# LanceKnight/MolKGNN

Hardware: AMD Instinct MI355X
Metric: molecules/sec fwd+bwd, 3-layer MolKGNN on AID 1798 (higher is better)
Workload: dtype f32; 1 GPU; AID 1798 full set shape (61832 molecules, ~25 atoms / ~53 directed edges each), 3 layers, hidden_dim 32, kernels 10/20/30/50 per degree, batch 4096 molecules per GPU (102584 atoms), 4 resident batches cycled, fwd+bwd+AdamW, one hipGraph per batch; variant=auto, batch_size_per_gpu=4096, parallelism=dp1

## Files before the change

include/molkgnn_hip.h:

```cpp
#ifndef MOLKGNN_HIP_H
#define MOLKGNN_HIP_H

#include <stddef.h>
#include <stdint.h>

#ifdef __cplusplus
extern "C" {
#endif

#define MKGNN_MAX_DEGREE 4
#define MKGNN_ABI_VERSION 8

#define MKGNN_LOSS_BCE_MEAN 0
#define MKGNN_LOSS_SQERR_MEAN 1
#define MKGNN_LOSS_SQERR_SUM 2

typedef struct mkgnn_kernel_bank {
    int32_t num_kernels;
    int32_t reserved;
    const float* x_center;
    const float* x_support;
    const float* edge_attr_support;
    const float* p_support;
    const float* support_attr_sc_weight;
// ... 142 lines not shown
    const int32_t* in_rowptr; const int32_t* in_col;
    const int32_t* out_rowptr; const int32_t* out_col;
    const int32_t* mol_ptr; const int32_t* atom_mol;
    int64_t n_atoms, n_mols, n_loss_mols;
    mkgnn_readout_params readout;
    const float* head_weight;
    const float* head_bias;
    const float* target;
    float dropout_p;
    int64_t* rng_state; int64_t* rng_used;
    float* emb; int64_t emb_stride;
    float* pred; float* loss;
    float* grad_sim; int64_t grad_sim_stride;
    float *grad_lin1_weight, *grad_lin1_bias, *grad_lin2_weight, *grad_lin2_bias, *grad_head_weight, *grad_head_bias;
    int32_t defer_reduce;
    int32_t loss_kind;
} mkgnn_tail_args;
int mkgnn_tail_supported(int32_t K, int32_t H, int32_t G, const int32_t num_kernels[MKGNN_MAX_DEGREE]);
size_t mkgnn_tail_workspace_bytes(int32_t K, int32_t H, int32_t G, int64_t n_atoms, int64_t n_mols);
int mkgnn_tail_fused(const mkgnn_tail_args* args, void* workspace, size_t workspace_bytes, void* stream);
int mkgnn_tail_fused_readout_dropout(const mkgnn_tail_args* args, float readout_dropout_p, void* workspace, size_t workspace_bytes,
                                     void* stream);
int mkgnn_readout_dropout_mask(const int64_t* rng_pair, int64_t n_rows, int32_t H, float p, float* keep, int64_t keep_stride,
                               void* stream);
int mkgnn_tail_flush(void* stream);
int mkgnn_tail_defer_projection(int32_t on);
int mkgnn_debug_tail_projection_launches(int64_t out[3]);
size_t mkgnn_tail_score_workspace_bytes(int32_t K, int32_t H, int32_t G, int64_t n_atoms, int64_t n_mols);
int mkgnn_tail_score(const mkgnn_tail_args* args, void* workspace, size_t workspace_bytes, void* stream);
#define MKGNN_TAIL_MC_MAX_SAMPLES 64
typedef struct mkgnn_tail_mc_out {
    float* samples; int64_t samples_stride;
    float* mean; float* std; float* acq;
    float alpha, beta;
} mkgnn_tail_mc_out;
size_t mkgnn_tail_score_mc_workspace_bytes(int32_t K, int32_t H, int32_t G, int64_t n_atoms, int64_t n_mols);
int mkgnn_tail_score_mc(const mkgnn_tail_args* args, float readout_dropout_p, int32_t n_samples, const int64_t* rng_pair,
                        const mkgnn_tail_mc_out* out, void* workspace, size_t workspace_bytes, void* stream);

#define MKGNN_ATOM_CONTRIB_MAX_TASKS 32
typedef struct mkgnn_atom_contrib_args {
    const float* sim; int64_t sim_stride;
    int32_t num_kernels[MKGNN_MAX_DEGREE];
    const mkgnn_degree_bucket* buckets;
    const int32_t* in_rowptr; const int32_t* in_col;
    int64_t n_atoms;
    mkgnn_readout_params readout;
    const float* head_weight; int64_t head_stride; int32_t T;
    float* contrib; int64_t contrib_stride;
} mkgnn_atom_contrib_args;
size_t mkgnn_atom_contributions_workspace_bytes(int32_t K, int32_t H, int32_t G, int64_t n_atoms);
int mkgnn_atom_contributions(const mkgnn_atom_contrib_args* args, void* workspace, size_t workspace_bytes, void* stream);

#define MKGNN_BN_SPLIT_ROWS 2
size_t mkgnn_batchnorm_workspace_bytes(int32_t C);
int mkgnn_batchnorm_forward(const float* x, int64_t x_stride, int64_t n_rows, int32_t C,
                            const float* weight, const float* bias,
                            float* running_mean, float* running_var, float momentum, float eps,
                            int32_t training, float* out, int64_t out_stride,
                            float* save_mean, float* save_invstd, float* inv_norm, int64_t* num_batches_tracked,
                            const int64_t* n_valid_rows, void* workspace, size_t workspace_bytes, void* stream);
typedef struct mkgnn_bn_stats {
    const float* x; int64_t x_stride; int64_t n_rows; int32_t C;
    float* running_mean; float* running_var;
    float momentum;
    int64_t* num_batches_tracked;
    const int64_t* row_key; const int64_t* key_limit;
} mkgnn_bn_stats;
size_t mkgnn_batchnorm_stats_workspace_bytes(int32_t C);
int mkgnn_batchnorm_update_stats(const mkgnn_bn_stats* stats, void* workspace, size_t workspace_bytes, void* stream);
int mkgnn_batchnorm_forward_with_stats(const float* x, int64_t x_stride, int64_t n_rows, int32_t C,
                            const float* weight, const float* bias,
                            float* running_mean, float* running_var, float momentum, float eps,
                            int32_t training, float* out, int64_t out_stride,
                            float* save_mean, float* save_invstd, float* inv_norm, int64_t* num_batches_tracked,
                            const int64_t* n_valid_rows, void* workspace, size_t workspace_bytes,
                            const mkgnn_bn_stats* companion, void* companion_workspace, size_t companion_workspace_bytes,
                            void* stream);
int mkgnn_batchnorm_backward(const float* grad_out, int64_t grad_out_stride, const float* x, int64_t x_stride,
                             int64_t n_rows, int32_t C, const float* weight,
                             const float* save_mean, const float* save_invstd, int32_t training,
                             float* grad_x, int64_t grad_x_stride, float* grad_weight, float* grad_bias,
                             const int64_t* n_valid_rows, void* workspace, size_t workspace_bytes, void* stream);
int mkgnn_debug_set_bn_merge(int32_t on);

size_t mkgnn_rf_workspace_bytes(int64_t n_atoms);
int mkgnn_rf_count(const int64_t* edge_index, int64_t n_atoms, int64_t n_edges,
                   void* workspace, size_t workspace_bytes, int64_t* counts, void* stream);
int mkgnn_rf_fill(const int64_t* edge_index, const float* p, const float* edge_attr,
                  int64_t n_atoms, int64_t n_edges, int32_t E, const void* workspace,
                  const mkgnn_degree_bucket out[MKGNN_MAX_DEGREE], void* stream);

size_t mkgnn_plan_workspace_bytes(int64_t n_atoms, int64_t n_edges, int64_t n_rows);

size_t mkgnn_index_workspace_bytes(int64_t n_atoms, int64_t n_edges, int64_t n_rows);
int mkgnn_index_build(const int64_t* edge_index, const float* p, const float* edge_attr, int64_t n_atoms, int64_t n_edges,
                      int32_t E, const mkgnn_degree_bucket out[MKGNN_MAX_DEGREE],
                      int32_t* scatter_rowptr, int32_t* scatter_rows, int32_t* in_rowptr, int32_t* in_col,
                      int32_t* in_col_packed, int32_t* out_rowptr, int32_t* out_col, int8_t* deg8, int64_t* counts,
                      void* workspace, size_t workspace_bytes, void* rf_ready_event, void* stream);

int mkgnn_expand_batch(const int32_t* bond_ij, const uint8_t* bond_attr, int64_t n_bonds, int32_t E,
                       const int32_t* mol_ptr, int64_t n_molecules, int64_t n_atoms,
                       int64_t* edge_index, float* edge_attr, int64_t* batch, int32_t* atom_molecule, void* stream);
int mkgnn_plan_build(const mkgnn_degree_bucket buckets[MKGNN_MAX_DEGREE], int64_t n_atoms, const int64_t* edge_index,
                     int64_t n_edges, int32_t* scatter_rowptr, int32_t* scatter_rows, int32_t* in_rowptr, int32_t* in_col,
                     int32_t* in_col_packed, int32_t* out_rowptr, int32_t* out_col, int8_t* deg8, void* workspace,
                     size_t workspace_bytes, void* stream);

int mkgnn_plan_present_blocks(const mkgnn_degree_bucket buckets[MKGNN_MAX_DEGREE], int64_t n_atoms, const int32_t* in_rowptr,
                              const int32_t* in_col_packed, int8_t* present8, int8_t* contrib_present8, void* stream);
int mkgnn_backward_grad_blocks(const int8_t* present8, const int32_t num_kernels[MKGNN_MAX_DEGREE]);
int64_t mkgnn_debug_grad_blocks_launches(void);
int mkgnn_debug_poison_backward(int32_t enable);
int mkgnn_debug_conv_dispatch(const mkgnn_kernel_bank banks[MKGNN_MAX_DEGREE], const mkgnn_degree_bucket buckets[MKGNN_MAX_DEGREE],
                              const float* x, int64_t x_stride, int64_t out_stride, int64_t n_atoms, int32_t F, int32_t E,
                              int32_t fwd_variant, int32_t bwd_variant, int32_t want_grad_x, const float* grad_x,
                              int64_t grad_x_stride, int32_t out[11]);

size_t mkgnn_bce_head_workspace_bytes(int64_t n_rows, int32_t H);
int mkgnn_bce_head_forward(const float* emb, int64_t emb_stride, int64_t n_rows, int32_t H,
                           const float* weight, const float* bias, const float* target,
                           float* pred, float* loss, void* workspace, size_t workspace_bytes, void* stream);
int mkgnn_bce_head_backward(const float* emb, int64_t emb_stride, int64_t n_rows, int32_t H,
                            const float* weight, const float* target, const float* pred, const float* grad_loss,
                            float* grad_emb, int64_t grad_emb_stride, float* grad_weight, float* grad_bias,
                            void* workspace, size_t workspace_bytes, void* stream);

int mkgnn_bce_head_dropout_forward(const float* emb, int64_t emb_stride, int64_t n_rows, int32_t H,
                                   const float* weight, const float* bias, const float* target, float dropout_p,
                                   int64_t* rng_state, int64_t* rng_used, float* pred, float* loss,
                                   void* workspace, size_t workspace_bytes, void* stream);
int mkgnn_bce_head_dropout_backward(const float* emb, int64_t emb_stride, int64_t n_rows, int32_t H,
                                    const float* weight, const float* target, const float* pred,
                                    const float* grad_loss, float dropout_p, const int64_t* rng_used,
                                    float* grad_emb, int64_t grad_emb_stride, float* grad_weight, float* grad_bias,
                                    void* workspace, size_t workspace_bytes, void* stream);

int mkgnn_bce_head_fused(const float* emb, int64_t emb_stride, int64_t n_rows, int32_t H,
                         const float* weight, const float* bias, const float* target, float dropout_p,
                         int64_t* rng_state, int64_t* rng_used, float* pred, float* loss,
                         float* grad_emb, int64_t grad_emb_stride, float* grad_weight, float* grad_bias,
                         void* workspace, size_t workspace_bytes, void* stream);

int mkgnn_head_loss_forward(int32_t loss_kind, const float* emb, int64_t emb_stride, int64_t n_rows, int32_t H,
                            const float* weight, const float* bias, const float* target,
                            float* pred, float* loss, void* workspace, size_t workspace_bytes, void* stream);
int mkgnn_head_loss_backward(int32_t loss_kind, const float* emb, int64_t emb_stride, int64_t n_rows, int32_t H,
                             const float* weight, const float* target, const float* pred, const float* grad_loss,
                             float* grad_emb, int64_t grad_emb_stride, float* grad_weight, float* grad_bias,
                             void* workspace, size_t workspace_bytes, void* stream);
int mkgnn_head_loss_dropout_forward(int32_t loss_kind, const float* emb, int64_t emb_stride, int64_t n_rows, int32_t H,
                                    const float* weight, const float* bias, const float* target, float dropout_p,
                                    int64_t* rng_state, int64_t* rng_used, float* pred, float* loss,
                                    void* workspace, size_t workspace_bytes, void* stream);
int mkgnn_head_loss_dropout_backward(int32_t loss_kind, const float* emb, int64_t emb_stride, int64_t n_rows, int32_t H,
                                     const float* weight, const float* target, const float* pred,
                                     const float* grad_loss, float dropout_p, const int64_t* rng_used,
                                     float* grad_emb, int64_t grad_emb_stride, float* grad_weight, float* grad_bias,
                                     void* workspace, size_t workspace_bytes, void* stream);
int mkgnn_head_loss_fused(int32_t loss_kind, const float* emb, int64_t emb_stride, int64_t n_rows, int32_t H,
                          const float* weight, const float* bias, const float* target, float dropout_p,
                          int64_t* rng_state, int64_t* rng_used, float* pred, float* loss,
                          float* grad_emb, int64_t grad_emb_stride, float* grad_weight, float* grad_bias,
                          void* workspace, size_t workspace_bytes, void* stream);

#define MKGNN_TASK_HEAD_MAX_TASKS 32
size_t mkgnn_task_head_workspace_bytes(int64_t n_rows, int32_t H, int32_t T);
int mkgnn_task_head_forward(int32_t loss_kind, const float* emb, int64_t emb_stride, int64_t n_rows, int32_t H, int32_t T,
                            const float* weight, const float* bias, const float* target, const int32_t* task,
                            const int32_t* row_ids, int64_t n_task, float dropout_p, int64_t* rng_state, int64_t* rng_used,
                            float* pred, float* loss, void* workspace, size_t workspace_bytes, void* stream);
int mkgnn_task_head_backward(int32_t loss_kind, const float* emb, int64_t emb_stride, int64_t n_rows, int32_t H, int32_t T,
                             const float* weight, const float* target, const int32_t* task, const int32_t* row_ids,
                             int64_t n_task, const float* pred, const float* grad_loss, float dropout_p,
                             const int64_t* rng_used, float* grad_emb, int64_t grad_emb_stride, float* grad_weight,
                             float* grad_bias, void* workspace, size_t workspace_bytes, void* stream);
int mkgnn_task_head_fused(int32_t loss_kind, const float* emb, int64_t emb_stride, int64_t n_rows, int32_t H, int32_t T,
                          const float* weight, const float* bias, const float* target, const int32_t* task,
                          const int32_t* row_ids, int64_t n_task, float dropout_p, int64_t* rng_state, int64_t* rng_used,
                          float* pred, float* loss, float* grad_emb, int64_t grad_emb_stride, float* grad_weight,
                          float* grad_bias, void* workspace, size_t workspace_bytes, void* stream);

typedef struct mkgnn_loss_weights {
    const float*   sample_weight;
    const int32_t* weight_ids;
    int64_t        n_sample_weight;
    const float*   pos_weight;
} mkgnn_loss_weights;
int mkgnn_task_head_weighted_forward(int32_t loss_kind, const float* emb, int64_t emb_stride, int64_t n_rows, int32_t H, int32_t T,
                                     const float* weight, const float* bias, const float* target, const int32_t* task,
                                     const int32_t* row_ids, int64_t n_task, float dropout_p, int64_t* rng_state,
                                     int64_t* rng_used, float* pred, float* loss, const mkgnn_loss_weights* weights,
                                     void* workspace, size_t workspace_bytes, void* stream);
int mkgnn_task_head_weighted_backward(int32_t loss_kind, const float* emb, int64_t emb_stride, int64_t n_rows, int32_t H, int32_t T,
// ... 254 lines not shown
```

molkgnn_amd/_lib.py:

```python
from __future__ import annotations

import ctypes as C
import os
from typing import Optional, Sequence

import torch

_HERE = os.path.dirname(os.path.abspath(__file__))
LIB_PATH = os.environ.get("MKGNN_LIB") or os.path.join(_HERE, "libmolkgnn_hip.so")
MAX_DEGREE = 4
ABI_VERSION = 8
LOSS_BCE_MEAN, LOSS_SQERR_MEAN, LOSS_SQERR_SUM = 0, 1, 2
TASK_HEAD_MAX_TASKS, TASK_HEAD_MAX_H = 32, 64
EMBED_COSINE_MAX_QUERIES, EMBED_COSINE_MAX_H = 32, 64
MAX_COSINE_MAX_REFS, MAX_COSINE_MAX_H = 1 << 20, 64
MAX_COSINE_ROWS, MAX_COSINE_TILE, MAX_COSINE_MAX_PARTS, MAX_COSINE_TARGET_BLOCKS = 128, 32, 256, 2048
SELECT_ROWS_PASS = 1024
DIVERSE_MAX_ROWS, DIVERSE_MAX_H = 1 << 20, 64
DIVERSE_COVER_ROWS, DIVERSE_COVER_TILE = 128, 32
MAXMIN_MAX_ROWS, MAXMIN_MAX_PICKS, MAXMIN_MAX_H = 1 << 20, 4096, 64
MAXMIN_TILE, MAXMIN_ROWS = 1024, 256
EXEMPLARS_MAX_K, EXEMPLARS_MAX_COLUMNS = 64, 256
EXEMPLARS_TILE, EXEMPLARS_CHUNK = 128, 64
KNN_MAX_K, KNN_MAX_QUERIES, KNN_MAX_ROWS, KNN_MAX_H = 64, 1 << 20, 1 << 20, 64
# ... 144 lines not shown
Int64x6 = C.c_int64 * 6
Banks4 = KernelBank * MAX_DEGREE
BankGrads4 = KernelBankGrad * MAX_DEGREE
Buckets4 = DegreeBucket * MAX_DEGREE
Saved4 = Saved * MAX_DEGREE
Int32x4 = C.c_int32 * MAX_DEGREE
Int64x4 = C.c_int64 * MAX_DEGREE

MOLECULE_MAX_LAYERS = 4
MOLECULE_MAX_ATOMS = 64
MOLECULE_MAX_MOLS = 16
MOLECULE_HEAD, MOLECULE_BACKWARD, MOLECULE_GRAD_EMB, MOLECULE_SQERR, MOLECULE_SUM = 1, 2, 4, 8, 16
MOLECULE_READOUT_DROPOUT = 32


class MoleculeLayer(C.Structure):
    _fields_ = [("bank", Banks4), ("grad", BankGrads4), ("saved", Saved4), ("F", C.c_int32), ("reserved", C.c_int32),
                ("sim_out", C.c_void_p), ("sim_stride", C.c_int64)]


class BnStats(C.Structure):
    _fields_ = [("x", C.c_void_p), ("x_stride", C.c_int64), ("n_rows", C.c_int64), ("C", C.c_int32),
                ("running_mean", C.c_void_p), ("running_var", C.c_void_p), ("momentum", C.c_float),
                ("num_batches_tracked", C.c_void_p), ("row_key", C.c_void_p), ("key_limit", C.c_void_p)]


class MoleculeNet(C.Structure):
    _fields_ = [("num_layers", C.c_int32), ("E", C.c_int32), ("layer", MoleculeLayer * MOLECULE_MAX_LAYERS),
                ("bn_weight", C.c_void_p), ("bn_bias", C.c_void_p), ("bn_running_mean", C.c_void_p),
                ("bn_running_var", C.c_void_p), ("bn_num_batches_tracked", C.c_void_p),
                ("bn_eps", C.c_float), ("bn_momentum", C.c_float), ("bn_training", C.c_int32), ("reserved", C.c_int32),
                ("grad_bn_weight", C.c_void_p), ("grad_bn_bias", C.c_void_p),
                ("readout", ReadoutParams),
                ("grad_lin1_weight", C.c_void_p), ("grad_lin1_bias", C.c_void_p), ("grad_lin2_weight", C.c_void_p),
                ("grad_lin2_bias", C.c_void_p),
                ("ffn_weight", C.c_void_p), ("ffn_bias", C.c_void_p), ("grad_ffn_weight", C.c_void_p),
                ("grad_ffn_bias", C.c_void_p), ("head_dropout", C.c_float), ("readout_dropout", C.c_float),
                ("rng_state", C.c_void_p), ("rng_used", C.c_void_p), ("edge_stats", C.POINTER(BnStats))]


class MoleculeBatch(C.Structure):
    _fields_ = [("n_atoms", C.c_int64), ("n_mols", C.c_int64), ("n_chunks", C.c_int64), ("max_chunk_atoms", C.c_int64),
                ("chunk_mol_ptr", C.c_void_p), ("mol_atom_ptr", C.c_void_p), ("atom_degree", C.c_void_p),
                ("atom_rank", C.c_void_p), ("buckets", Buckets4), ("x", C.c_void_p), ("x_stride", C.c_int64)]


class LossWeights(C.Structure):
    _fields_ = [("sample_weight", C.c_void_p), ("weight_ids", C.c_void_p), ("n_sample_weight", C.c_int64),
                ("pos_weight", C.c_void_p)]


EXPORTS = ("mkgnn_abi_version", "mkgnn_last_error", "mkgnn_row_inv_norm", "mkgnn_unit_rows8", "mkgnn_workspace_bytes",
           "mkgnn_kernelsetconv_forward", "mkgnn_kernelsetconv_backward", "mkgnn_segment_sum_rows",
           "mkgnn_readout_hidden_stride", "mkgnn_readout_workspace_bytes", "mkgnn_readout_forward",
           "mkgnn_readout_backward", "mkgnn_batchnorm_workspace_bytes", "mkgnn_batchnorm_forward",
           "mkgnn_batchnorm_backward", "mkgnn_bce_head_workspace_bytes", "mkgnn_bce_head_forward",
           "mkgnn_bce_head_backward", "mkgnn_rf_workspace_bytes", "mkgnn_rf_count", "mkgnn_rf_fill", "mkgnn_adamw_step", "mkgnn_adamw_state_floats",
           "mkgnn_adamw_clip_workspace_bytes", "mkgnn_adamw_step_clipped",
           "mkgnn_adamw_average_floats", "mkgnn_adamw_step_averaged", "mkgnn_flat_swap",
           "mkgnn_bce_head_dropout_forward", "mkgnn_bce_head_dropout_backward", "mkgnn_segment_sum_block_rows",
           "mkgnn_plan_workspace_bytes", "mkgnn_plan_build", "mkgnn_plan_present_blocks", "mkgnn_backward_grad_blocks",
           "mkgnn_debug_grad_blocks_launches", "mkgnn_debug_poison_backward", "mkgnn_backward_join", "mkgnn_backward_streams", "mkgnn_bank_prepare", "mkgnn_bank_prepare_deferred", "mkgnn_bank_prepare_flush", "mkgnn_bank_prepare_withdraw", "mkgnn_touch_hint", "mkgnn_expand_batch", "mkgnn_bce_head_fused", "mkgnn_collate_compact", "mkgnn_collate_compact_bytes",
           "mkgnn_readout_blocks_supported", "mkgnn_readout_blocks_forward", "mkgnn_readout_blocks_backward",
           "mkgnn_readout_blocks_workspace_bytes", "mkgnn_molecule_supported", "mkgnn_molecule_workspace_bytes",
           "mkgnn_molecule_step", "mkgnn_batchnorm_stats_workspace_bytes", "mkgnn_batchnorm_update_stats",
           "mkgnn_batchnorm_forward_with_stats", "mkgnn_index_workspace_bytes", "mkgnn_index_build",
           "mkgnn_rows_split_supported", "mkgnn_rows_presplit", "mkgnn_tail_supported", "mkgnn_tail_workspace_bytes", "mkgnn_tail_fused", "mkgnn_tail_flush", "mkgnn_flat_copy",
           "mkgnn_tail_fused_readout_dropout", "mkgnn_readout_dropout_mask", "mkgnn_tail_score", "mkgnn_tail_score_workspace_bytes",
           "mkgnn_head_loss_forward", "mkgnn_head_loss_backward", "mkgnn_head_loss_dropout_forward",
           "mkgnn_head_loss_dropout_backward", "mkgnn_head_loss_fused", "mkgnn_gather_compact",
           "mkgnn_gather_compact_workspace_bytes", "mkgnn_gather_compact_packed", "mkgnn_topk_update", "mkgnn_topk_workspace_bytes",
           "mkgnn_task_head_workspace_bytes", "mkgnn_task_head_forward", "mkgnn_task_head_backward", "mkgnn_task_head_fused",
           "mkgnn_task_head_weighted_forward", "mkgnn_task_head_weighted_backward", "mkgnn_task_head_weighted_fused",
           "mkgnn_tail_fused_weighted",
           "mkgnn_task_scores", "mkgnn_topk_tasks_workspace_bytes", "mkgnn_topk_update_tasks", "mkgnn_embed_cosine",
           "mkgnn_atom_contributions", "mkgnn_atom_contributions_workspace_bytes", "mkgnn_embed_max_cosine",
           "mkgnn_embed_max_cosine_workspace_bytes", "mkgnn_select_rows", "mkgnn_tail_defer_projection",
           "mkgnn_debug_tail_projection_launches", "mkgnn_diverse_pick", "mkgnn_diverse_pick_workspace_bytes",
           "mkgnn_kernel_exemplars_update", "mkgnn_kernel_exemplars_workspace_bytes", "mkgnn_embed_knn_update",
           "mkgnn_embed_knn_workspace_bytes", "mkgnn_embed_count_within", "mkgnn_embed_count_within_workspace_bytes",
           "mkgnn_embed_neighbours_within", "mkgnn_embed_neighbours_within_workspace_bytes", "mkgnn_graph_components",
           "mkgnn_graph_components_workspace_bytes", "mkgnn_maxmin_pick", "mkgnn_maxmin_pick_workspace_bytes",
           "mkgnn_tail_score_mc", "mkgnn_tail_score_mc_workspace_bytes", "mkgnn_debug_set_bn_merge", "mkgnn_debug_conv_dispatch",
           "mkgnn_bootstrap_roc", "mkgnn_bootstrap_roc_workspace_bytes")

_lib: Optional[C.CDLL] = None
TORCH_LIB_PATH = os.path.join(os.path.dirname(LIB_PATH), "libmolkgnn_torch.so")
_torch_ops_loaded = False


def load_torch_ops():
    global _torch_ops_loaded
    import torch
    if not _torch_ops_loaded:
        load()
        if not os.path.exists(TORCH_LIB_PATH):
            raise MolKGNNLibraryError(f"{TORCH_LIB_PATH} is missing: build it with `make -C molkgnn_amd/csrc torch`")
        torch.ops.load_library(TORCH_LIB_PATH)
        if int(torch.ops.molkgnn.abi_version()) != ABI_VERSION:
            raise MolKGNNLibraryError("libmolkgnn_torch.so was built against another ABI version")
        _torch_ops_loaded = True
    return torch.ops.molkgnn


class MolKGNNLibraryError(RuntimeError):
    pass


def load() -> C.CDLL:
    global _lib
    if _lib is not None:
        return _lib
    if not os.path.exists(LIB_PATH):
        raise MolKGNNLibraryError(
            f"{LIB_PATH} is missing: build it with `make -C molkgnn_amd/csrc` "
            "(python -c 'import __graft_entry__ as g; g.build()'). There is no fallback path.")
    lib = C.CDLL(LIB_PATH)
    for name in EXPORTS:
        if not hasattr(lib, name):
            raise MolKGNNLibraryError(f"{LIB_PATH} does not export {name}")
    lib.mkgnn_abi_version.restype = C.c_int
    lib.mkgnn_last_error.restype = C.c_char_p
    lib.mkgnn_row_inv_norm.restype = C.c_int
    lib.mkgnn_row_inv_norm.argtypes = [C.c_void_p, C.c_int64, C.c_int64, C.c_int32, C.c_void_p, C.c_void_p]
    lib.mkgnn_unit_rows8.restype = C.c_int
    lib.mkgnn_unit_rows8.argtypes = [C.c_void_p, C.c_int64, C.c_int32, C.c_void_p, C.c_void_p]
    lib.mkgnn_workspace_bytes.restype = C.c_size_t
    lib.mkgnn_workspace_bytes.argtypes = [Int32x4, C.c_int32, C.c_int32, C.c_int64, C.c_int64]
    lib.mkgnn_kernelsetconv_forward.restype = C.c_int
    lib.mkgnn_kernelsetconv_forward.argtypes = [
        Banks4, Buckets4, C.c_void_p, C.c_int64, C.c_void_p, C.c_int64, C.c_int32, C.c_int32, C.c_int32,
        C.c_void_p, C.c_int64, Saved4, C.c_void_p, C.c_size_t, C.c_int32, C.c_void_p]
    lib.mkgnn_kernelsetconv_backward.restype = C.c_int
    lib.mkgnn_kernelsetconv_backward.argtypes = [
        Banks4, Buckets4, C.c_void_p, C.c_int64, C.c_void_p, C.c_int64, C.c_int32, C.c_int32, C.c_int32,
        C.c_void_p, C.c_int64, Saved4, C.c_void_p, C.c_void_p, C.c_void_p, C.c_int64, BankGrads4,
        C.c_void_p, C.c_size_t, C.c_int32, C.c_int32, C.c_void_p]
    lib.mkgnn_backward_streams.restype = C.c_int
    lib.mkgnn_backward_streams.argtypes = [Banks4, Buckets4, C.c_void_p, C.c_int64, C.c_int64, C.c_int32, C.c_int32]
    lib.mkgnn_debug_conv_dispatch.restype = C.c_int
    lib.mkgnn_debug_conv_dispatch.argtypes = [Banks4, Buckets4, C.c_void_p, C.c_int64, C.c_int64, C.c_int64, C.c_int32, C.c_int32,
                                              C.c_int32, C.c_int32, C.c_int32, C.c_void_p, C.c_int64, C.POINTER(C.c_int32 * 11)]
    lib.mkgnn_tail_supported.restype = C.c_int
    lib.mkgnn_tail_supported.argtypes = [C.c_int32, C.c_int32, C.c_int32, Int32x4]
    lib.mkgnn_tail_workspace_bytes.restype = C.c_size_t
    lib.mkgnn_tail_workspace_bytes.argtypes = [C.c_int32, C.c_int32, C.c_int32, C.c_int64, C.c_int64]
    lib.mkgnn_tail_fused.restype = C.c_int
    lib.mkgnn_tail_fused.argtypes = [C.POINTER(TailArgs), C.c_void_p, C.c_size_t, C.c_void_p]
    lib.mkgnn_tail_score_workspace_bytes.restype = C.c_size_t
    lib.mkgnn_tail_score_workspace_bytes.argtypes = [C.c_int32, C.c_int32, C.c_int32, C.c_int64, C.c_int64]
    lib.mkgnn_tail_score.restype = C.c_int
    lib.mkgnn_tail_score.argtypes = [C.POINTER(TailArgs), C.c_void_p, C.c_size_t, C.c_void_p]
    lib.mkgnn_tail_score_mc_workspace_bytes.restype = C.c_size_t
    lib.mkgnn_tail_score_mc_workspace_bytes.argtypes = [C.c_int32, C.c_int32, C.c_int32, C.c_int64, C.c_int64]
    lib.mkgnn_tail_score_mc.restype = C.c_int
    lib.mkgnn_tail_score_mc.argtypes = [C.POINTER(TailArgs), C.c_float, C.c_int32, C.c_void_p, C.POINTER(TailMcOut), C.c_void_p,
                                        C.c_size_t, C.c_void_p]
    lib.mkgnn_atom_contributions_workspace_bytes.restype = C.c_size_t
    lib.mkgnn_atom_contributions_workspace_bytes.argtypes = [C.c_int32, C.c_int32, C.c_int32, C.c_int64]
    lib.mkgnn_atom_contributions.restype = C.c_int
    lib.mkgnn_atom_contributions.argtypes = [C.POINTER(AtomContribArgs), C.c_void_p, C.c_size_t, C.c_void_p]
    lib.mkgnn_tail_fused_readout_dropout.restype = C.c_int
    lib.mkgnn_tail_fused_readout_dropout.argtypes = [C.POINTER(TailArgs), C.c_float, C.c_void_p, C.c_size_t, C.c_void_p]
    lib.mkgnn_tail_fused_weighted.restype = C.c_int
    lib.mkgnn_tail_fused_weighted.argtypes = [C.POINTER(TailArgs), C.c_float, C.POINTER(LossWeights), C.c_void_p, C.c_size_t,
                                              C.c_void_p]
    lib.mkgnn_readout_dropout_mask.restype = C.c_int
# ... 97 lines not shown
    for name, args in (("mkgnn_head_loss_forward", lib.mkgnn_bce_head_forward.argtypes),
                       ("mkgnn_head_loss_backward", lib.mkgnn_bce_head_backward.argtypes),
                       ("mkgnn_head_loss_dropout_forward", lib.mkgnn_bce_head_dropout_forward.argtypes),
                       ("mkgnn_head_loss_dropout_backward", lib.mkgnn_bce_head_dropout_backward.argtypes),
                       ("mkgnn_head_loss_fused", lib.mkgnn_bce_head_fused.argtypes)):
        getattr(lib, name).restype = C.c_int
        getattr(lib, name).argtypes = [I32] + list(args)
    lib.mkgnn_bce_head_workspace_bytes.restype = C.c_size_t
    lib.mkgnn_bce_head_workspace_bytes.argtypes = [I64, I32]
    lib.mkgnn_task_head_workspace_bytes.restype = C.c_size_t
    lib.mkgnn_task_head_workspace_bytes.argtypes = [I64, I32, I32]
    lib.mkgnn_task_head_forward.restype = C.c_int
    lib.mkgnn_task_head_forward.argtypes = [I32, P, I64, I64, I32, I32, P, P, P, P, P, I64, C.c_float, P, P, P, P, P, C.c_size_t, P]
    lib.mkgnn_task_head_backward.restype = C.c_int
    lib.mkgnn_task_head_backward.argtypes = [I32, P, I64, I64, I32, I32, P, P, P, P, I64, P, P, C.c_float, P, P, I64, P, P, P,
                                             C.c_size_t, P]
    lib.mkgnn_task_head_fused.restype = C.c_int
    lib.mkgnn_task_head_fused.argtypes = [I32, P, I64, I64, I32, I32, P, P, P, P, P, I64, C.c_float, P, P, P, P, P, I64, P, P, P,
                                          C.c_size_t, P]
    for name in ("forward", "backward", "fused"):
        args = list(getattr(lib, "mkgnn_task_head_" + name).argtypes)
        getattr(lib, "mkgnn_task_head_weighted_" + name).restype = C.c_int
        getattr(lib, "mkgnn_task_head_weighted_" + name).argtypes = args[:-3] + [C.POINTER(LossWeights)] + args[-3:]
    lib.mkgnn_task_scores.restype = C.c_int
    lib.mkgnn_task_scores.argtypes = [P, I64, I64, I32, I32, P, P, P, I64, I64, P]
    lib.mkgnn_embed_cosine.restype = C.c_int
    lib.mkgnn_embed_cosine.argtypes = [P, I64, I64, I32, P, I64, I32, P, I64, I64, P]
    lib.mkgnn_embed_max_cosine_workspace_bytes.restype = C.c_size_t
    lib.mkgnn_embed_max_cosine_workspace_bytes.argtypes = [I64, I32]
    lib.mkgnn_embed_max_cosine.restype = C.c_int
    lib.mkgnn_embed_max_cosine.argtypes = [P, I64, I64, I32, P, I64, I32, P, P, P, C.c_size_t, P]
    lib.mkgnn_embed_count_within_workspace_bytes.restype = C.c_size_t
    lib.mkgnn_embed_count_within_workspace_bytes.argtypes = [I64, I32]
    lib.mkgnn_embed_count_within.restype = C.c_int
    lib.mkgnn_embed_count_within.argtypes = [P, I64, I64, I32, P, I64, I32, F32, P, P, C.c_size_t, P]
    lib.mkgnn_embed_neighbours_within_workspace_bytes.restype = C.c_size_t
    lib.mkgnn_embed_neighbours_within_workspace_bytes.argtypes = [I64, I32]
    lib.mkgnn_embed_neighbours_within.restype = C.c_int
    lib.mkgnn_embed_neighbours_within.argtypes = [P, I64, I64, I32, P, I64, I32, F32, P, I64, P, P, P, P, C.c_size_t, P]
    lib.mkgnn_graph_components_workspace_bytes.restype = C.c_size_t
    lib.mkgnn_graph_components_workspace_bytes.argtypes = [I32]
    lib.mkgnn_graph_components.restype = C.c_int
    lib.mkgnn_graph_components.argtypes = [P, P, I32, P, P, I32, P, C.c_size_t, P]
    lib.mkgnn_select_rows.restype = C.c_int
    lib.mkgnn_select_rows.argtypes = [P, P, P, I32, P, P, P, P, P, P]
    lib.mkgnn_diverse_pick_workspace_bytes.restype = C.c_size_t
    lib.mkgnn_diverse_pick_workspace_bytes.argtypes = [I64]
    lib.mkgnn_diverse_pick.restype = C.c_int
    lib.mkgnn_diverse_pick.argtypes = [P, I64, I64, I32, C.c_float, I32, P, P, P, P, P, C.c_size_t, P]
    lib.mkgnn_maxmin_pick_workspace_bytes.restype = C.c_size_t
    lib.mkgnn_maxmin_pick_workspace_bytes.argtypes = [I64]
    lib.mkgnn_maxmin_pick.restype = C.c_int
    lib.mkgnn_maxmin_pick.argtypes = [P, I64, I64, I32, P, C.c_float, I32, P, P, P, P, P, P, C.c_size_t, P]
    lib.mkgnn_bootstrap_roc_workspace_bytes.restype = C.c_size_t
    lib.mkgnn_bootstrap_roc_workspace_bytes.argtypes = [I64, I32]
    lib.mkgnn_bootstrap_roc.restype = C.c_int
    lib.mkgnn_bootstrap_roc.argtypes = [P, P, P, I64, I64, I32, C.c_uint64, C.c_uint64, C.c_double, C.c_double, P, P, P, P, P,
                                        C.c_size_t, P]
    lib.mkgnn_kernel_exemplars_workspace_bytes.restype = C.c_size_t
    lib.mkgnn_kernel_exemplars_workspace_bytes.argtypes = [C.POINTER(Int64x4), C.POINTER(Int32x4), I32, I32]
    lib.mkgnn_kernel_exemplars_update.restype = C.c_int
    lib.mkgnn_kernel_exemplars_update.argtypes = [P, I64, I64, C.POINTER(Buckets4), C.POINTER(Int32x4), C.POINTER(Int32x4), P, P, P,
                                                  I32, P, P, P, I32, I32, P, P, P, P, P, C.c_size_t, P]
    lib.mkgnn_embed_knn_workspace_bytes.restype = C.c_size_t
    lib.mkgnn_embed_knn_workspace_bytes.argtypes = [I64, I32, I32]
    lib.mkgnn_embed_knn_update.restype = C.c_int
    lib.mkgnn_embed_knn_update.argtypes = [P, I64, I64, I32, P, P, P, P, I64, I32, I32, P, P, P, P, C.c_size_t, P]
    lib.mkgnn_rf_workspace_bytes.restype = C.c_size_t
    lib.mkgnn_rf_workspace_bytes.argtypes = [I64]
    lib.mkgnn_rf_count.restype = C.c_int
    lib.mkgnn_rf_count.argtypes = [P, I64, I64, P, C.c_size_t, P, P]
    lib.mkgnn_rf_fill.restype = C.c_int
    lib.mkgnn_rf_fill.argtypes = [P, P, P, I64, I64, I32, P, Buckets4, P]
    lib.mkgnn_segment_sum_block_rows.restype = C.c_int
    lib.mkgnn_segment_sum_block_rows.argtypes = [P, I64, P, P, P, I64, Int32x4, I32, P, I64, P, P]
    lib.mkgnn_plan_workspace_bytes.restype = C.c_size_t
    lib.mkgnn_plan_workspace_bytes.argtypes = [I64, I64, I64]
    lib.mkgnn_plan_build.restype = C.c_int
    lib.mkgnn_plan_build.argtypes = [Buckets4, I64, P, I64, P, P, P, P, P, P, P, P, P, C.c_size_t, P]
    lib.mkgnn_plan_present_blocks.restype = C.c_int
    lib.mkgnn_plan_present_blocks.argtypes = [Buckets4, I64, P, P, P, P, P]
    lib.mkgnn_backward_grad_blocks.restype = C.c_int
    lib.mkgnn_backward_grad_blocks.argtypes = [P, P]
    lib.mkgnn_debug_grad_blocks_launches.restype = C.c_int64
    lib.mkgnn_debug_grad_blocks_launches.argtypes = []
    lib.mkgnn_debug_poison_backward.restype = C.c_int
    lib.mkgnn_debug_poison_backward.argtypes = [I32]
    lib.mkgnn_index_workspace_bytes.restype = C.c_size_t
    lib.mkgnn_index_workspace_bytes.argtypes = [I64, I64, I64]
    lib.mkgnn_index_build.restype = C.c_int
    lib.mkgnn_index_build.argtypes = [P, P, P, I64, I64, I32, Buckets4, P, P, P, P, P, P, P, P, P, P, C.c_size_t, P, P]
    lib.mkgnn_adamw_step.restype = C.c_int
    lib.mkgnn_adamw_state_floats.restype = C.c_int64
    lib.mkgnn_adamw_state_floats.argtypes = [I64]
    lib.mkgnn_adamw_step.argtypes = [P, I32, P, I32, P]
    lib.mkgnn_adamw_clip_workspace_bytes.restype = C.c_size_t
    lib.mkgnn_adamw_clip_workspace_bytes.argtypes = [P, I32]
    lib.mkgnn_adamw_step_clipped.restype = C.c_int
    lib.mkgnn_adamw_step_clipped.argtypes = [P, I32, P, I32, C.c_float, I32, P, C.c_size_t, P, P]
    lib.mkgnn_adamw_average_floats.restype = C.c_int64
    lib.mkgnn_adamw_average_floats.argtypes = [I64]
    lib.mkgnn_adamw_step_averaged.restype = C.c_int
    lib.mkgnn_adamw_step_averaged.argtypes = [P, I32, P, I32, C.POINTER(AdamWAverage), C.c_float, I32, P, C.c_size_t, P, P]
    lib.mkgnn_flat_swap.restype = C.c_int
    lib.mkgnn_flat_swap.argtypes = [P, I32, P]
    lib.mkgnn_molecule_supported.restype = C.c_int
    lib.mkgnn_molecule_supported.argtypes = [C.POINTER(MoleculeNet), I32]
    lib.mkgnn_molecule_workspace_bytes.restype = C.c_size_t
    lib.mkgnn_molecule_workspace_bytes.argtypes = [C.POINTER(MoleculeNet), I32, I64, I64]
    lib.mkgnn_molecule_step.restype = C.c_int
    lib.mkgnn_molecule_step.argtypes = [C.POINTER(MoleculeNet), C.POINTER(MoleculeBatch), I32, P, P, P, P, P, P, C.c_size_t, P]
    if lib.mkgnn_abi_version() != ABI_VERSION:
        raise MolKGNNLibraryError(f"ABI version {lib.mkgnn_abi_version()} != {ABI_VERSION}: rebuild the library")
    _lib = lib
    return lib


def check(rc: int, what: str) -> None:
    if rc != 0:
        msg = load().mkgnn_last_error()
        raise MolKGNNLibraryError(f"{what}: {msg.decode() if msg else 'error'}")


def ptr(t: Optional[torch.Tensor]) -> Optional[int]:
    return None if t is None or t.numel() == 0 else t.data_ptr()


def stream_ptr(device: torch.device) -> int:
    return torch.cuda.current_stream(device).cuda_stream


def require_gpu_tensor(t: torch.Tensor, name: str) -> None:
    if not t.is_cuda:
        raise MolKGNNLibraryError(
            f"{name} is on {t.device}: the kernel convolution runs on an MI355X only (no CPU fallback)")
```

molkgnn_amd/csrc/kgnn_batchnorm.hip:

```cpp
#include <hip/hip_runtime.h>
#include <atomic>
#include <cstdint>
#include <cstdlib>
#include "kgnn_common.h"

#include "kgnn_launch.h"
#include "kgnn_prepare.h"
#include "kgnn_split.h"
#include "../../include/molkgnn_hip.h"

namespace mkgnn {

typedef mkgnn_f32x4 f32x4;

#ifndef MKGNN_BN_BLOCKS
#define MKGNN_BN_BLOCKS 256
#endif
#ifndef MKGNN_BN_AB
#define MKGNN_BN_AB 0
#endif
constexpr int BN_MAIN_BLOCKS = MKGNN_BN_BLOCKS;
constexpr int BN_SIDE_BLOCKS = 1024;
struct BnSide {
    const float* x; int64_t xs; int64_t n; int C, CL, nblk;
    int flat;
    float *running_mean, *running_var; float momentum;
    int64_t* nbt;
    const int64_t* key; const int64_t* key_limit;
    float* part;
    int merge;
};

struct BnArgs {
    const float* x; int64_t xs; int64_t n; int C;
    const float *weight, *bias;
    float *running_mean, *running_var;
    float momentum, eps; int training;
    float* out; int64_t os;
    float *save_mean, *save_invstd;
    float* part1; float* part2;
    float* part3;
    const float* gout; int64_t gos;
    float* gx; int64_t gxs;
    float *gweight, *gbias;
    float* inv_out;
    int split_out;
    int touch_first;
    TouchArgs touch;
    int64_t* nbt;
    const int64_t* nvalid;
    int merge;
    BnSide side;
};

__device__ __forceinline__ int bn_nblk() { return (int)gridDim.x < BN_MAIN_BLOCKS ? (int)gridDim.x : BN_MAIN_BLOCKS; }

__device__ __forceinline__ int64_t bn_valid(const BnArgs& a) {
    if (!a.nvalid) return a.n;
    const int64_t v = *a.nvalid;
    return v < 1 ? 1 : (v < a.n ? v : a.n);
}

__device__ __forceinline__ void bn_rows(const BnArgs& a, int64_t& lo, int64_t& hi) {
    const int64_t per = (a.n + bn_nblk() - 1) / bn_nblk();
    lo = per * blockIdx.x;
    hi = lo + per < a.n ? lo + per : a.n;
    if (lo > hi) lo = hi;
}

constexpr int BN_U = 16;
constexpr int BN_UA = 8;

__device__ __forceinline__ float bn_shfl_xor(float v, int o) { return __shfl_xor(v, o, 64); }
__device__ __forceinline__ f32x4 bn_shfl_xor(f32x4 v, int o) {
    return f32x4{__shfl_xor(v[0], o, 64), __shfl_xor(v[1], o, 64), __shfl_xor(v[2], o, 64), __shfl_xor(v[3], o, 64)};
}
__device__ __forceinline__ void bn_zero(float& v) { v = 0.f; }
__device__ __forceinline__ void bn_zero(f32x4& v) { v = f32x4{0.f, 0.f, 0.f, 0.f}; }

template <typename V> __device__ __forceinline__ V bn_reduce_rows(V v, int LW, V* shv) {
    const int t = threadIdx.x;
    for (int o = 32; o >= LW; o >>= 1) v = v + bn_shfl_xor(v, o);
    __syncthreads();
    int parts;
    if (LW <= 64) {
        if ((t & 63) < LW) shv[(t >> 6) * LW + (t & 63)] = v;
        parts = 4;
    } else {
        shv[t] = v;
        parts = 256 / LW;
    }
    __syncthreads();
    V r;
    bn_zero(r);
    if (t < LW)
        for (int k = 0; k < parts; ++k) r = r + shv[k * LW + t];
    return r;
}

__device__ __forceinline__ void bn_share(int64_t nv, int nblk, int b, int64_t& lo, int64_t& hi) {
    const int64_t per = (nv + nblk - 1) / nblk;
    lo = per * b;
    hi = lo + per < nv ? lo + per : nv;
    if (lo > hi) lo = hi;
}

template <int MODE, int U>
__device__ __forceinline__ void bn_pass_vec(const float* x, int64_t xs, const float* g, int64_t gs, int64_t lo, int64_t hi, int rsub, int RS,
                                            int col, f32x4 mu, f32x4 is, f32x4& s0, f32x4& s1) {
    for (int64_t r0 = lo + rsub; r0 < hi; r0 += (int64_t)U * RS) {
        f32x4 v[U], gg[U];
#pragma unroll
        for (int u = 0; u < U; ++u) {
            const int64_t rr = r0 + (int64_t)u * RS < hi ? r0 + (int64_t)u * RS : hi - 1;
            v[u] = *(const f32x4*)(x + rr * xs + col);
            if (MODE == 2) gg[u] = *(const f32x4*)(g + rr * gs + col);
        }
#pragma unroll
        for (int u = 0; u < U; ++u) {
            if (r0 + (int64_t)u * RS < hi) {
#pragma unroll
                for (int e = 0; e < 4; ++e) {
                    if (MODE == 0) s0[e] += v[u][e];
                    if (MODE == 1) { const float d = v[u][e] - mu[e]; s0[e] = fmaf(d, d, s0[e]); s1[e] += d; }
                    if (MODE == 2) { s0[e] += gg[u][e]; s1[e] = fmaf(gg[u][e], (v[u][e] - mu[e]) * is[e], s1[e]); }
                }
            }
        }
    }
}
template <int MODE>
__device__ __forceinline__ void bn_pass_col(const float* x, int64_t xs, const float* g, int64_t gs, int64_t lo, int64_t hi, int rsub, int RS,
                                            int c, float mu, float is, float& s0, float& s1) {
    for (int64_t r0 = lo + rsub; r0 < hi; r0 += 8 * RS) {
        float v[8], gg[8];
#pragma unroll
        for (int u = 0; u < 8; ++u) {
            const int64_t rr = r0 + u * RS < hi ? r0 + u * RS : hi - 1;
            v[u] = x[rr * xs + c];
            if (MODE == 2) gg[u] = g[rr * gs + c];
        }
#pragma unroll
        for (int u = 0; u < 8; ++u) {
            if (r0 + u * RS < hi) {
                if (MODE == 0) s0 += v[u];
                if (MODE == 1) { const float d = v[u] - mu; s0 = fmaf(d, d, s0); s1 += d; }
                if (MODE == 2) { s0 += gg[u]; s1 = fmaf(gg[u], (v[u] - mu) * is, s1); }
            }
        }
    }
}

static inline bool bn_vec_rows(const void* p, int64_t stride, int C) { return p && C % 4 == 0 && stride % 4 == 0 && ((uintptr_t)p & 15) == 0; }

template <bool VEC>
__device__ __forceinline__ void bn_block_stats(const BnArgs& a, int CL, float* sh) {
    __shared__ float bmean[256];
    const int t = threadIdx.x;
    int64_t lo, hi;
    bn_share(bn_valid(a), bn_nblk(), blockIdx.x, lo, hi);
    const float cnt = (float)(hi - lo);
    float* const p1 = a.part1 + (int64_t)blockIdx.x * a.C;
    float* const p2 = a.part2 + (int64_t)blockIdx.x * a.C;
    float* const p3 = a.part3 + (int64_t)blockIdx.x * a.C;
    if constexpr (VEC) {
        const int LW = CL >= 4 ? CL / 4 : 1, g = t % LW, rsub = t / LW, RS = 256 / LW, col = 4 * g;
        const bool act = col < a.C;
        const int cb = act ? col : 0;
        const f32x4 z = {0.f, 0.f, 0.f, 0.f};
        f32x4 s0 = z, s1 = z;
        bn_pass_vec<0, BN_U>(a.x, a.xs, nullptr, 0, lo, hi, rsub, RS, cb, z, z, s0, s1);
        const f32x4 tot = bn_reduce_rows(s0, LW, (f32x4*)sh);
        if (t < LW && act) {
#pragma unroll
            for (int e = 0; e < 4; ++e) { p1[col + e] = tot[e]; bmean[col + e] = cnt > 0.f ? tot[e] / cnt : 0.f; }
        }
        __syncthreads();
        const f32x4 mu = {bmean[cb], bmean[cb + 1], bmean[cb + 2], bmean[cb + 3]};
        s0 = z;
        if (MKGNN_BN_AB != 3) bn_pass_vec<1, BN_U>(a.x, a.xs, nullptr, 0, lo, hi, rsub, RS, cb, mu, z, s0, s1);
        const f32x4 m2 = bn_reduce_rows(s0, LW, (f32x4*)sh);
        const f32x4 m1 = bn_reduce_rows(s1, LW, (f32x4*)sh);
        if (t < LW && act) {
#pragma unroll
            for (int e = 0; e < 4; ++e) { p2[col + e] = m2[e]; p3[col + e] = m1[e]; }
        }
    } else {
        const int c = t & (CL - 1), rsub = t / CL, RS = 256 / CL;
// ... 733 lines not shown
    const bool split_rows = (training & MKGNN_BN_SPLIT_ROWS) != 0;
    training &= 1;
    if (split_rows && !inv_norm) return api_fail("mkgnn_batchnorm_forward: MKGNN_BN_SPLIT_ROWS needs inv_norm");
    if (companion && !training) return api_fail("mkgnn_batchnorm_forward: a statistics companion needs training mode (nothing moves in eval mode)");
    if (!x || !out || x_stride < C || out_stride < C) return api_fail("mkgnn_batchnorm_forward: bad x/out");
    if (training && (!save_mean || !save_invstd)) return api_fail("mkgnn_batchnorm_forward: save_mean/save_invstd is null");
    if (!training && (!running_mean || !running_var)) return api_fail("mkgnn_batchnorm_forward: eval mode needs running statistics");
    if (training && (!ws || ws_bytes < mkgnn_batchnorm_workspace_bytes(C))) return api_fail("mkgnn_batchnorm_forward: workspace too small");
    hipStream_t st = (hipStream_t)stream;
    BnArgs a{};
    a.x = x; a.xs = x_stride; a.n = n_rows; a.C = C; a.weight = weight; a.bias = bias;
    a.running_mean = running_mean; a.running_var = running_var; a.momentum = momentum; a.eps = eps; a.training = training;
    a.out = out; a.os = out_stride; a.save_mean = save_mean; a.save_invstd = save_invstd;
    if (inv_norm && (C > 32 || C % 4 || x_stride % 4 || out_stride % 4 || ((uintptr_t)x & 15) || ((uintptr_t)out & 15)))
        return api_fail("mkgnn_batchnorm_forward: inv_norm needs C <= 32, a multiple of 4, and 16-byte aligned rows of x and out (C=%d)", C);
    a.inv_out = inv_norm; a.split_out = split_rows ? 1 : 0; a.nbt = num_batches_tracked; a.nvalid = n_valid_rows; a.merge = bn_merge_on();
    a.part1 = (float*)ws; a.part2 = a.part1 ? a.part1 + (size_t)BN_BLOCKS * C : nullptr;
    a.part3 = a.part1 ? a.part1 + (size_t)2 * BN_BLOCKS * C : nullptr;
    static_assert(BN_BLOCKS == BN_MAIN_BLOCKS, "the companion's blocks sit behind the batch norm's own");
    bool side_single = false;
    if (companion) {
        if (int rc = bn_side_setup("mkgnn_batchnorm_forward", companion, companion_ws, companion_ws_bytes, a.side)) return rc;
        if ((int64_t)companion->n_rows * a.side.CL <= 64 * 1024) { a.side.nblk = 1; side_single = true; }
    }
    const bool one_launch = switches().bn_one_launch;
    if (training && one_launch) {
        if (bn_vec_rows(x, x_stride, C)) bn_forward_fused_kernel<true><<<BN_BLOCKS + a.side.nblk, 256, 0, st>>>(a, CL);
        else bn_forward_fused_kernel<false><<<BN_BLOCKS + a.side.nblk, 256, 0, st>>>(a, CL);
    } else {
        if (training) {
            a.touch.count = 0;
            a.touch_first = BN_BLOCKS + a.side.nblk;
            const int extra = take_touch_hint(a.touch) ? TOUCH_BLOCKS : 0;
            PrepManyArgs pm;
            if (take_pending_prepare(pm)) {
                pm.touch.count = 0;
                const int prep_first = a.touch_first + extra;
                if (bn_vec_rows(x, x_stride, C)) bn_stats_prep_kernel<true><<<prep_first + pm.prep_blocks, 256, 0, st>>>(a, CL, pm, prep_first);
                else bn_stats_prep_kernel<false><<<prep_first + pm.prep_blocks, 256, 0, st>>>(a, CL, pm, prep_first);
            } else if (bn_vec_rows(x, x_stride, C)) bn_stats_kernel<true><<<BN_BLOCKS + a.side.nblk + extra, 256, 0, st>>>(a, CL);
            else bn_stats_kernel<false><<<BN_BLOCKS + a.side.nblk + extra, 256, 0, st>>>(a, CL);
            a.touch.count = 0;
        }
        bn_apply_kernel<<<BN_BLOCKS + ((a.side.nblk && !side_single) ? 1 : 0), 256, 0, st>>>(a, CL);
    }
    hipError_t e = hipGetLastError();
    return e == hipSuccess ? 0 : api_hip_fail("mkgnn_batchnorm_forward", e);
}

int mkgnn_batchnorm_backward(const float* grad_out, int64_t grad_out_stride, const float* x, int64_t x_stride,
                             int64_t n_rows, int32_t C, const float* weight, const float* save_mean,
                             const float* save_invstd, int32_t training, float* grad_x, int64_t grad_x_stride, float* grad_weight, float* grad_bias,
                             const int64_t* n_valid_rows, void* ws, size_t ws_bytes, void* stream) {
    int CL;
    if (int rc = bn_common("mkgnn_batchnorm_backward", n_rows, C, CL)) return rc;
    if (!grad_out || !x || grad_out_stride < C || x_stride < C) return api_fail("mkgnn_batchnorm_backward: bad grad_out/x");
    if (!save_mean || !save_invstd) return api_fail("mkgnn_batchnorm_backward: saved statistics are null");
    if (grad_x && grad_x_stride < C) return api_fail("mkgnn_batchnorm_backward: bad grad_x stride");
    if (!ws || ws_bytes < mkgnn_batchnorm_workspace_bytes(C)) return api_fail("mkgnn_batchnorm_backward: workspace too small");
    hipStream_t st = (hipStream_t)stream;
    BnArgs a{};
    a.x = x; a.xs = x_stride; a.n = n_rows; a.C = C; a.weight = weight;
    a.training = training;
    a.save_mean = (float*)save_mean; a.save_invstd = (float*)save_invstd;
    a.part1 = (float*)ws; a.part2 = a.part1 + (size_t)BN_BLOCKS * C;
    a.gout = grad_out; a.gos = grad_out_stride; a.gx = grad_x; a.gxs = grad_x_stride;
    a.gweight = grad_weight; a.gbias = grad_bias; a.nvalid = n_valid_rows; a.merge = bn_merge_on();
    const bool one_launch = switches().bn_one_launch;
    const bool vec = bn_vec_rows(x, x_stride, C) && bn_vec_rows(grad_out, grad_out_stride, C) && (!grad_x || bn_vec_rows(grad_x, grad_x_stride, C));
    if (one_launch && grad_x) {
        if (vec) bn_backward_fused_kernel<true><<<BN_BLOCKS, 256, 0, st>>>(a, CL);
        else bn_backward_fused_kernel<false><<<BN_BLOCKS, 256, 0, st>>>(a, CL);
    } else if (vec) {
        bn_bwd_partial_kernel<true><<<BN_BLOCKS, 256, 0, st>>>(a, CL);
        bn_bwd_final_kernel<true><<<grad_x ? BN_BLOCKS : 1, 256, 0, st>>>(a, CL, BN_BLOCKS);
    } else {
        bn_bwd_partial_kernel<false><<<BN_BLOCKS, 256, 0, st>>>(a, CL);
        bn_bwd_final_kernel<false><<<grad_x ? BN_BLOCKS : 1, 256, 0, st>>>(a, CL, BN_BLOCKS);
    }
    hipError_t e = hipGetLastError();
    return e == hipSuccess ? 0 : api_hip_fail("mkgnn_batchnorm_backward", e);
}

}
```

molkgnn_amd/csrc/kgnn_capi.hip:

```cpp
#include <stdarg.h>
#include <stdio.h>
#include <string.h>

#include <mutex>

#include "kgnn_launch.h"
#include "kgnn_split.h"

using namespace mkgnn;

static thread_local char g_err[512] = "";

namespace mkgnn {
int api_fail(const char* fmt, ...) {
    va_list ap;
    va_start(ap, fmt);
    vsnprintf(g_err, sizeof(g_err), fmt, ap);
    va_end(ap);
    return 1;
}
int api_hip_fail(const char* what, hipError_t e) { return api_fail("%s: %s", what, hipGetErrorString(e)); }
int spans_disjoint(const char* who, const Span* writes, int n_writes, const Span* reads, int n_reads, const char* reads_text,
                   const char* writes_text) {
    auto overlap_start = [](const Span& x, const Span& y) -> const char* {
        const char *xp = (const char*)x.p, *yp = (const char*)y.p;
        return x.n && y.n && xp < yp + y.n && yp < xp + x.n ? (xp > yp ? xp : yp) : nullptr;
    };
    const char *first = nullptr, *text = nullptr;
    for (int i = 0; i < n_writes; ++i) {
        for (int j = 0; j < n_reads; ++j) {
            const char* at = overlap_start(writes[i], reads[j]);
            if (at && (!first || at < first)) { first = at; text = reads_text; }
        }
        for (int j = i + 1; j < n_writes; ++j) {
            const char* at = overlap_start(writes[i], writes[j]);
            if (at && (!first || at < first)) { first = at; text = writes_text; }
        }
    }
    return first ? api_fail("%s: %s", who, text) : 0;
}
}

struct DegreeStreams {
    hipStream_t aux[3];
    hipEvent_t fork;
    hipEvent_t join[3];
    bool ready;
    bool deferred;
    std::once_flag once;
};
static DegreeStreams g_streams[16];

static DegreeStreams* degree_streams() {
    if (switches().serial) return nullptr;
    int dev = 0;
    if (hipGetDevice(&dev) != hipSuccess || dev < 0 || dev >= 16) return nullptr;
    DegreeStreams& p = g_streams[dev];
    std::call_once(p.once, [&p]() {
        bool ok = true;
        int least = 0, greatest = 0;
        const char env_prio = switches().helper_priority;
        const bool ranged = env_prio && hipDeviceGetStreamPriorityRange(&least, &greatest) == hipSuccess;
        const int prio = (ranged && env_prio == 'l') ? least : ((ranged && env_prio == 'h') ? greatest : 0);
        for (int i = 0; i < 3 && ok; ++i) {
            ok = ((ranged && prio != 0) ? hipStreamCreateWithPriority(&p.aux[i], hipStreamNonBlocking, prio)
                                        : hipStreamCreateWithFlags(&p.aux[i], hipStreamNonBlocking)) == hipSuccess &&
                 hipEventCreateWithFlags(&p.join[i], hipEventDisableTiming) == hipSuccess;
        }
        ok = ok && hipEventCreateWithFlags(&p.fork, hipEventDisableTiming) == hipSuccess;
        p.ready = ok;
    });
    return p.ready ? &p : nullptr;
}

struct ForkJoin {
    DegreeStreams* p;
    hipStream_t main;
    bool used[3];
    bool two_way = false;
    hipError_t begin(hipStream_t st, bool enable) {
        hipStreamCaptureStatus cap = hipStreamCaptureStatusNone;
        const bool fork_in_graph = switches().fork_in_graph;
        const bool capturing = hipStreamIsCapturing(st, &cap) == hipSuccess && cap != hipStreamCaptureStatusNone;
        if (enable && capturing && switches().fork_mode && !fork_in_graph) two_way = true;
        else if (enable && !fork_in_graph && capturing) enable = false;
        main = st; p = enable ? degree_streams() : nullptr;
        used[0] = used[1] = used[2] = false;
        if (!p) return hipSuccess;
        return two_way ? hipSuccess : hipEventRecord(p->fork, main);
// ... 254 lines not shown
    if (n_rows < 0 || E < 1 || E > 8) return api_fail("mkgnn_unit_rows8: %lld rows of width %d (1..8)", (long long)n_rows, E);
    if (n_rows && (!in || !out)) return api_fail("mkgnn_unit_rows8: null pointer");
    hipError_t e = launch_unit_rows8(in, n_rows, E, out, (hipStream_t)stream);
    return e == hipSuccess ? 0 : api_hip_fail("mkgnn_unit_rows8", e);
}

size_t mkgnn_workspace_bytes(const int32_t num_kernels[MKGNN_MAX_DEGREE], int32_t F, int32_t E, int64_t n_atoms,
                             int64_t n_edges) {
    return make_layout(num_kernels, F, E, n_atoms, n_edges).total;
}

static int check_common(const char* who, const mkgnn_kernel_bank banks[4], const mkgnn_degree_bucket buckets[4],
                        const float* x, int64_t x_stride, const float* inv_norm, int64_t n_atoms, int32_t F, int32_t E,
                        int32_t need_coordinates, int64_t* n_edges_out) {
    if (!banks || !buckets) return api_fail("%s: banks/buckets is null", who);
    if (F <= 0 || F > 256) return api_fail("%s: node attribute width F=%d outside 1..256", who, F);
    if (E <= 0 || E > 64) return api_fail("%s: edge attribute width E=%d outside 1..64", who, E);
    if (n_atoms < 0 || x_stride < F) return api_fail("%s: bad x shape", who);
    if (n_atoms && (!x || !inv_norm)) return api_fail("%s: x/inv_norm is null", who);
    int64_t n_edges = 0, n_focal = 0;
    for (int i = 0; i < 4; ++i) {
        const mkgnn_kernel_bank& b = banks[i];
        const mkgnn_degree_bucket& k = buckets[i];
        if (b.num_kernels < 0 || b.num_kernels > 4096) return api_fail("%s: degree %d has %d kernels", who, i + 1, b.num_kernels);
        if (k.count < 0) return api_fail("%s: degree %d bucket count %lld", who, i + 1, (long long)k.count);
        if (k.count > 0) {
            if (!k.selected_index || !k.nei_index || !k.nei_edge_attr)
                return api_fail("%s: degree %d bucket has null index/edge tensors", who, i + 1);
            if (i == 3 && need_coordinates && (!k.p_focal || !k.nei_p || !b.p_support))
                return api_fail("%s: degree-4 coordinates are required in the last layer (chirality)", who);
        }
        if (b.num_kernels > 0 && (!b.x_center || !b.x_support || !b.edge_attr_support || !b.support_attr_sc_weight ||
                                  !b.center_attr_sc_weight || !b.edge_attr_support_sc_weight))
            return api_fail("%s: degree %d bank has null parameters", who, i + 1);
        n_edges += k.count * (i + 1);
        n_focal += k.count;
    }
    if (n_focal > n_atoms) return api_fail("%s: buckets hold %lld atoms, batch has %lld", who, (long long)n_focal, (long long)n_atoms);
    *n_edges_out = n_edges;
    return 0;
}

static thread_local TouchArgs g_touch_hint;
extern "C++" {
namespace mkgnn {
bool take_touch_hint(TouchArgs& out) {
    if (g_touch_hint.count <= 0) return false;
    out = g_touch_hint;
    g_touch_hint.count = 0;
    return true;
}
}
}

static thread_local GradBlocks g_grad_blocks_hint;
static std::atomic<int> g_poison_bwd{0};
extern "C++" {
namespace mkgnn {
std::atomic<long long> g_grad_blocks_launches;
bool take_grad_blocks_hint(GradBlocks& out) {
    out = g_grad_blocks_hint;
    g_grad_blocks_hint = GradBlocks{};
    return out.present8 != nullptr;
}
}
}

int mkgnn_backward_grad_blocks(const int8_t* present8, const int32_t num_kernels[MKGNN_MAX_DEGREE]) {
    g_grad_blocks_hint = GradBlocks{};
    if (!present8) return 0;
    if (!num_kernels) return api_fail("mkgnn_backward_grad_blocks: null pointer");
    GradBlocks gb{present8, 0, 0};
    int off = 0;
    for (int d = 1; d <= 4; ++d) {
        const int L = num_kernels[d - 1];
        if (L < 1 || off + L > 255) return 0;
        gb.blk_off |= (uint64_t)off << (8 * d);
        gb.blk_len |= (uint64_t)L << (8 * d);
        off += L;
    }
    g_grad_blocks_hint = gb;
    return 0;
}

int64_t mkgnn_debug_grad_blocks_launches(void) { return g_grad_blocks_launches.load(); }
int mkgnn_debug_poison_backward(int32_t enable) { g_poison_bwd.store(enable ? 1 : 0); return 0; }

int mkgnn_touch_hint(const void* const* arrays, const size_t* bytes, int32_t count) {
    if (count <= 0 || !arrays || !bytes) {
        const int had = g_touch_hint.count > 0 ? 1 : 0;
        g_touch_hint.count = 0;
        return had;
    }
    TouchArgs ta{};
    for (int k = 0; k < count && ta.count < TOUCH_MAX; ++k) {
        if (!arrays[k] || bytes[k] < 32) continue;
        const uintptr_t lo = ((uintptr_t)arrays[k] + 15) & ~(uintptr_t)15, hi = ((uintptr_t)arrays[k] + bytes[k]) & ~(uintptr_t)15;
        if (hi <= lo) continue;
        const size_t n = hi - lo;
        ta.ptr[ta.count] = (const char*)lo;
        ta.bytes[ta.count] = (uint32_t)(n > 0xfffffff0u ? 0xfffffff0u : n);
        ++ta.count;
    }
    g_touch_hint = ta;
    return 0;
}

struct PendingPrepare { PrepManyArgs m; bool armed; };
static PendingPrepare g_pending_prepare[16];
static std::mutex g_pending_prepare_mutex;
static PendingPrepare* pending_prepare_slot() {
    int dev = 0;
    if (hipGetDevice(&dev) != hipSuccess || dev < 0 || dev >= 16) dev = 0;
    return &g_pending_prepare[dev];
}
extern "C++" {
namespace mkgnn {
bool take_pending_prepare(PrepManyArgs& out) {
    std::lock_guard<std::mutex> lock(g_pending_prepare_mutex);
    PendingPrepare* p = pending_prepare_slot();
    if (!p->armed) return false;
    out = p->m;
    p->armed = false;
    return true;
}
}
}

static int bank_prepare_impl(const char* who, int32_t count, const mkgnn_kernel_bank* banks, const int32_t* F, int32_t E,
                             void* const* workspaces, const size_t* workspace_bytes, bool defer, void* stream);

int mkgnn_bank_prepare_deferred(int32_t count, const mkgnn_kernel_bank* banks, const int32_t* F, int32_t E, void* const* workspaces,
                                const size_t* workspace_bytes) {
    return bank_prepare_impl("mkgnn_bank_prepare_deferred", count, banks, F, E, workspaces, workspace_bytes, true, nullptr);
}

int mkgnn_bank_prepare_flush(void* stream) {
    PrepManyArgs m;
    if (!take_pending_prepare(m)) return 0;
    (void)take_touch_hint(m.touch);
    hipError_t e = launch_bank_prepare_args(m, (hipStream_t)stream);
    return e == hipSuccess ? 0 : api_hip_fail("mkgnn_bank_prepare_flush", e);
}

int mkgnn_bank_prepare_withdraw(void) {
    PrepManyArgs m;
    return take_pending_prepare(m) ? 1 : 0;
}

int mkgnn_bank_prepare(int32_t count, const mkgnn_kernel_bank* banks, const int32_t* F, int32_t E, void* const* workspaces,
                       const size_t* workspace_bytes, void* stream) {
    if (int rc = mkgnn_bank_prepare_flush(stream)) return rc;
    return bank_prepare_impl("mkgnn_bank_prepare", count, banks, F, E, workspaces, workspace_bytes, false, stream);
}

static int bank_prepare_impl(const char* who, int32_t count, const mkgnn_kernel_bank* banks, const int32_t* F, int32_t E,
                             void* const* workspaces, const size_t* workspace_bytes, bool defer, void* stream) {
    if (count < 0 || count > PREP_MANY_MAX) return api_fail("%s: %d calls (0..%d per launch)", who, count, PREP_MANY_MAX);
    TouchArgs ta{};
    if (!defer) (void)take_touch_hint(ta);
    if (count == 0 && ta.count == 0) return 0;
    if (count > 0 && (!banks || !F || !workspaces || !workspace_bytes || E <= 0)) return api_fail("%s: bad arguments", who);
    WorkspaceLayout w[PREP_MANY_MAX];
    char* ws[PREP_MANY_MAX];
    int Fs[PREP_MANY_MAX];
    for (int k = 0; k < count; ++k) {
// ... 42 lines not shown
    for (int i = 0; i < 4; ++i) { L[i] = banks[i].num_kernels; K += L[i]; }
    if (out_stride < K || (n_atoms && !out)) return api_fail("%s: bad out (stride %lld, K %d)", who, (long long)out_stride, K);
    WorkspaceLayout w = make_layout(L, F, E, n_atoms, n_edges);
    if (workspace_bytes < w.fwd_end || !workspace)
        return api_fail("%s: workspace of %zu bytes, need %zu", who, workspace_bytes, w.fwd_end);
    const bool block_rows_only = (variant & MKGNN_VARIANT_BLOCK_ROWS) != 0;
    const bool bank_prepared = (variant & MKGNN_VARIANT_BANK_PREPARED) != 0;
    const bool rows_split = (variant & MKGNN_VARIANT_ROWS_SPLIT) != 0;
    variant &= ~(MKGNN_VARIANT_BLOCK_ROWS | MKGNN_VARIANT_BANK_PREPARED | MKGNN_VARIANT_ROWS_SPLIT);
    if (variant < 0 || variant > 3) return api_fail("%s: variant %d", who, variant);
    const ConvShape shape = conv_shape(banks, buckets, F, E, n_atoms, x, x_stride, out_stride);
    const FwdDispatch plan = plan_conv_forward(shape, variant);
    if (rows_split && (variant == 1 || variant == 3 || !rows_split_covered(shape, plan)))
        return api_fail("%s: MKGNN_VARIANT_ROWS_SPLIT needs the streamed kernels with split-fp16 products for every degree "
                        "(mkgnn_rows_split_supported(..) tells)", who);
    if (const int g = plan.overflow_groups)
        return api_fail("%s: the banks need %d column groups, the %s launch holds %d", who, g, plan.overflow_launch, FUSED_MAX_GROUPS);
    if (const int d = plan.refused_degree)
        return api_fail("%s: MFMA variant does not cover degree %d with F=%d E=%d L=%d stride=%lld", who, d, F, E, L[d - 1], (long long)x_stride);
    hipStream_t st = (hipStream_t)stream; char* ws = (char*)workspace;
    hipError_t e = bank_prepared ? hipSuccess : launch_bank_prepare(banks, w, ws, F, E, st);
    if (e != hipSuccess) return api_hip_fail("bank_prepare", e);
    if (n_atoms > 0 && K > 0 && !block_rows_only) {
        const int64_t K4 = (K + 3) / 4 * 4;
        if (K4 == out_stride) e = hipMemsetAsync(out, 0, (size_t)n_atoms * out_stride * 4, st);
        else e = hipMemset2DAsync(out, (size_t)out_stride * 4, 0, (size_t)(K4 <= out_stride ? K4 : K) * 4, (size_t)n_atoms, st);
        if (e != hipSuccess) return api_hip_fail("output memset", e);
    }
    FusedFwdArgs fa; memset(&fa, 0, sizeof(fa));
    fa.x = x; fa.xs = x_stride; fa.inv = inv_norm; fa.out = out; fa.os = out_stride;
    fa.K = K; fa.F = F; fa.E = E; fa.last = is_last_layer ? 1 : 0; fa.n_atoms = n_atoms;
    fa.bf16 = variant == 3 ? 1 : 0;
    fa.x_split = rows_split ? 1 : 0;
    bool use_stream[4], use_bank[4], any_fused = false;
    int off = 0;
    for (int i = 0; i < 4; ++i) {
        const int d = i + 1; FwdArgs a;
        a.x = x; a.xs = x_stride; a.inv = inv_norm;
        a.sel = buckets[i].selected_index; a.nei = buckets[i].nei_index; a.e_nei = buckets[i].nei_edge_attr;
        a.p_focal = buckets[i].p_focal; a.p_nei = buckets[i].nei_p;
        a.n = buckets[i].count; a.F = F; a.E = E; a.L = L[i]; a.last = is_last_layer ? 1 : 0;
        a.cen = (const float*)(ws + w.bank[i].cen); a.sup = (const float*)(ws + w.bank[i].sup);
        a.edg = (const float*)(ws + w.bank[i].edg); a.chir = (const int8_t*)(ws + w.bank[i].chir);
        a.mix = (const float*)(ws + w.bank[i].mix);
        a.padded = (const float*)(ws + w.bank[i].padded); a.edge_padded = (const float*)(ws + w.bank[i].edge_padded);
        a.n_atoms = n_atoms;
        a.out = out; a.os = out_stride; a.off = off; a.K = K;
        a.pair = saved ? saved[i].pair_state : nullptr;
        a.chir_out = (saved && d == 4 && is_last_layer) ? saved[i].chirality : nullptr;
        off += L[i];
        use_stream[i] = plan.deg[i] == FWD_STREAMED; use_bank[i] = plan.deg[i] == FWD_LDS_BANK;
        if (use_stream[i] || use_bank[i]) {
            FusedDeg& g = fa.deg[i];
            g.sel = a.sel; g.nei = a.nei; g.e_nei = a.e_nei; g.e_unit = buckets[i].nei_edge_unit; g.p_focal = a.p_focal; g.p_nei = a.p_nei;
            g.padded = a.padded; g.edge_padded = a.edge_padded; g.chir = a.chir; g.mix = a.mix;
            g.eqflag = (const int8_t*)(ws + w.eqflag);
            g.signflag = (const int8_t*)(ws + w.signflag);
            g.pair = a.pair; g.chir_out = a.chir_out;
            g.n = a.n; g.L = a.L; g.off = a.off;
            any_fused = true;
        } else if (plan.deg[i] == FWD_GENERIC) {
            e = launch_forward_generic(d, a, st);
            if (e != hipSuccess) return api_hip_fail("kernelconv forward launch", e);
        }
    }
    if (any_fused) {
        e = launch_forward_fused(fa, use_stream, use_bank, st);
        if (e != hipSuccess) return api_hip_fail("fused kernelconv forward launch", e);
    }
    return 0;
}

int mkgnn_kernelsetconv_backward(const mkgnn_kernel_bank banks[MKGNN_MAX_DEGREE],
                                 const mkgnn_degree_bucket buckets[MKGNN_MAX_DEGREE], const float* x, int64_t x_stride,
                                 const float* inv_norm, int64_t n_atoms, int32_t F, int32_t E, int32_t is_last_layer,
                                 const float* grad_out, int64_t grad_out_stride,
                                 const mkgnn_saved saved[MKGNN_MAX_DEGREE], const int32_t* scatter_rowptr,
                                 const int32_t* scatter_rows, float* grad_x, int64_t grad_x_stride,
                                 const mkgnn_kernel_bank_grad grads[MKGNN_MAX_DEGREE], void* workspace,
                                 size_t workspace_bytes, int32_t workspace_from_forward, int32_t variant, void* stream) {
    const char* who = "mkgnn_kernelsetconv_backward";
    GradBlocks gb;
    const bool gb_hint = take_grad_blocks_hint(gb);
    const bool defer_bank = (variant & MKGNN_BACKWARD_DEFER_BANK) != 0;
    const bool through_nei = (variant & MKGNN_BACKWARD_THROUGH_NEIGHBOURS) != 0;
    const bool rows_split = (variant & MKGNN_BACKWARD_ROWS_SPLIT) != 0;
    variant &= ~(MKGNN_BACKWARD_DEFER_BANK | MKGNN_BACKWARD_THROUGH_NEIGHBOURS | MKGNN_BACKWARD_ROWS_SPLIT);
    if (variant < 0 || variant > 2) return api_fail("%s: variant %d (0 = automatic, 1 = generic kernels, 2 = fast kernels)", who, variant);
    int64_t n_edges = 0;
    if (int rc = check_common(who, banks, buckets, x, x_stride, inv_norm, n_atoms, F, E, 0, &n_edges)) return rc;
    if (!saved || !grads) return api_fail("%s: saved/grads is null", who);
    int32_t L[4], K = 0;
    for (int i = 0; i < 4; ++i) { L[i] = banks[i].num_kernels; K += L[i]; }
    if (grad_out_stride < K || (n_atoms && !grad_out)) return api_fail("%s: bad grad_out", who);
    if (grad_x && grad_x_stride < F) return api_fail("%s: bad grad_x stride", who);
    if (grad_x && n_atoms && n_edges > 0 && (!scatter_rowptr || !scatter_rows)) return api_fail("%s: scatter CSR is null", who);
    WorkspaceLayout w = make_layout(L, F, E, n_atoms, n_edges);
    if (workspace_bytes < w.total || !workspace) return api_fail("%s: workspace of %zu bytes, need %zu", who, workspace_bytes, w.total);
    for (int i = 0; i < 4; ++i) {
        if (buckets[i].count > 0 && L[i] > 0 && !saved[i].pair_state) return api_fail("%s: degree %d has no saved forward state", who, i + 1);
        if (i == 3 && is_last_layer && buckets[i].count > 0 && !saved[i].chirality)
            return api_fail("%s: degree-4 chirality signs were not saved", who);
    }
    const BwdDispatch plan = plan_conv_backward(conv_shape(banks, buckets, F, E, n_atoms, x, x_stride, 0, grad_x, grad_x_stride), variant);
    if (const int d = plan.refused_degree)
        return api_fail("%s: the fast kernels do not cover degree %d with F=%d E=%d L=%d stride=%lld", who, d, F, E, L[d - 1], (long long)x_stride);
    if (through_nei && !plan.through_nei_ok)
        return api_fail("%s: MKGNN_BACKWARD_THROUGH_NEIGHBOURS needs the streamed kernels for every degree "
                        "(mkgnn_backward_streams(..) tells)", who);
    if (rows_split && !plan.rows_split_ok)
        return api_fail("%s: MKGNN_BACKWARD_ROWS_SPLIT needs the streamed kernels with split-fp16 products for every degree "
                        "(mkgnn_rows_split_supported(..) tells)", who);
    const bool fuse_bank = plan.bank_fused, rows_streamed = plan.rows_streamed, streamed = plan.bank_streamed;
    bool gb_gather = gb_hint && switches().grad_blocks && variant != 1 && grad_x && n_edges > 0 && F <= 255 &&
                     backward_gather_aligned_supported((const float*)((char*)workspace + w.contrib), (F + 3) / 4 * 4, scatter_rows, x, x_stride,
                                                       n_atoms, F, grad_x, grad_x_stride);
    if (gb_gather) {
        int width = 0;
        for (int d = 1; d <= 4; ++d) width += (int)((gb.blk_len >> (8 * d)) & 0xFF);
        gb_gather = width == F;
    }
    hipStream_t st = (hipStream_t)stream; char* ws = (char*)workspace;
    BwdArgs bank_a[4];
    BankReduceArgs reduce[4];
    bool bank_use[4];
    const float* e_unit4[4]; float* coefq4[4];
    int off = 0; int64_t base = 0;
    size_t coef_off = w.coefq_off[0];
    for (int i = 0; i < 4; ++i) {
        BwdArgs& a = bank_a[i];
        a.x = x; a.xs = x_stride; a.inv = inv_norm;
        a.sel = buckets[i].selected_index; a.nei = buckets[i].nei_index; a.e_nei = buckets[i].nei_edge_attr;
        a.n = buckets[i].count; a.F = F; a.E = E; a.L = L[i];
        a.cen = (const float*)(ws + w.bank[i].cen); a.sup = (const float*)(ws + w.bank[i].sup);
        a.edg = (const float*)(ws + w.bank[i].edg); a.mix = (const float*)(ws + w.bank[i].mix);
        a.gout = grad_out; a.gs = grad_out_stride; a.off = off;
        a.pair = saved[i].pair_state;
        a.chir = (i == 3 && is_last_layer) ? saved[i].chirality : nullptr;
        a.contrib = (float*)(ws + w.contrib); a.contrib_base = base; a.CS = (F + 3) / 4 * 4;
        a.slab = (float*)(ws + w.slab_off[i]);
        a.padded = (const float*)(ws + w.bank[i].padded);
        a.nchunk = (int)(a.n < BWD_BANK_BLOCKS ? (a.n > 0 ? a.n : 1) : BWD_BANK_BLOCKS);
        a.theta_slab = (float*)(ws + w.theta_off[i]);
        BankReduceArgs& r = reduce[i];
        r.slab = a.slab; r.F = F; r.E = E; r.L = L[i];
        r.cen = a.cen; r.sup = a.sup; r.edg = a.edg;
        r.icen = (const float*)(ws + w.bank[i].icen); r.isup = (const float*)(ws + w.bank[i].isup);
        r.iedg = (const float*)(ws + w.bank[i].iedg);
        r.g = grads[i];
        off += L[i]; base += buckets[i].count * (i + 2);
        bank_use[i] = fuse_bank && plan.deg[i] >= BWD_MFMA_LDS;
        e_unit4[i] = buckets[i].nei_edge_unit; coefq4[i] = nullptr;
        if (!bank_use[i]) continue;
        coefq4[i] = (float*)(ws + coef_off);
        coef_off += (size_t)((buckets[i].count + 15) / 16) * ((L[i] + 15) / 16) * 512 * 4;
    }
    const bool any_bank = bank_use[0] || bank_use[1] || bank_use[2] || bank_use[3];
    hipError_t e = hipSuccess;
    if (g_poison_bwd.load() && grad_x && n_atoms) {
        int64_t rows_all = 0;
        for (int i = 0; i < 4; ++i) rows_all += buckets[i].count * (i + 2);
        e = hipMemsetAsync(ws + w.contrib, 0xFF, (size_t)rows_all * ((F + 3) / 4 * 4) * sizeof(float), st);
        if (e == hipSuccess)
            e = hipMemset2DAsync(grad_x, (size_t)grad_x_stride * sizeof(float), 0xFF, (size_t)F * sizeof(float), (size_t)n_atoms, st);
        if (e != hipSuccess) return api_hip_fail("poison", e);
    }
    if (!workspace_from_forward) {
        e = launch_bank_prepare(banks, w, ws, F, E, st);
        if (e != hipSuccess) return api_hip_fail("bank_prepare", e);
    }
    int slot_of[4];
    degree_slots(banks, buckets, slot_of);
    ForkJoin fj;
    e = fj.begin(st, !g_time_bwd.load());
    if (e != hipSuccess) return api_hip_fail("stream fork", e);
    TailProjection tp;
    bool project = false;
    if (pending_tail_projection(&tp)) {
        project = grad_out == tp.dsim && grad_out_stride == tp.dss && streamed && rows_streamed && !through_nei && defer_bank && fj.p != nullptr &&
                  any_bank && K == tp.K;
        for (int i = 0; i < 4 && project; ++i) {
            const bool same = L[i] == tp.L[i] && bank_a[i].off == tp.off[i] && buckets[i].count == tp.cnt[i] &&
                              (tp.cnt[i] == 0 || buckets[i].selected_index == tp.sel[i]);
            const bool wanted = tp.cnt[i] > 0 && tp.L[i] > 0;
            project = same && (!wanted || bank_use[i]) && bank_stream_projection_supported(tp.H, tp.HP, L[i]);
        }
        if (!project) {
            e = launch_pending_tail_projection(st, true);
            if (e != hipSuccess) return api_hip_fail("deferred tail projection launch", e);
            e = fj.fork_here();
            if (e != hipSuccess) return api_hip_fail("stream fork", e);
        }
    }
    bool bank_on_main = false;
    for (int i = 0; i < 4; ++i) {
        const int d = i + 1;
        const BwdArgs& a = bank_a[i];
        hipStream_t dst = fj.stream(fj.two_way ? 0 : slot_of[i], &e);
        if (e != hipSuccess) return api_hip_fail("stream fork", e);
        int nchunk = a.n > 0 ? a.nchunk : 0;
        int ntheta = -1;
        if (plan.deg[i] == BWD_ZERO_FILL) {
            e = hipMemsetAsync(a.contrib + (size_t)a.contrib_base * a.CS, 0, (size_t)a.n * (d + 1) * a.CS * sizeof(float), dst);
// ... 13 lines not shown
                }
            }
            if (rows_mfma && !rows_streamed && (grad_x || !fuse_bank)) {
                e = launch_backward_rows_mfma(d, a, &ntheta, st_rows);
                if (e != hipSuccess) return api_hip_fail("kernelconv backward launch", e);
            }
            if (!fuse_bank) e = launch_backward_lds(d, a, &nchunk, &ntheta, !rows_mfma, st_bank);
        }
        if (e != hipSuccess) return api_hip_fail("kernelconv backward launch", e);
        BankReduceArgs& r = reduce[i];
        r.nchunk = nchunk;
        if (ntheta >= 0) { r.theta_src = a.theta_slab; r.theta_stride = 4; r.theta_count = ntheta; }
        else {
            r.theta_src = a.slab + (size_t)L[i] * F + (size_t)L[i] * d * F + (size_t)L[i] * d * E;
            r.theta_stride = bank_floats(d, L[i], F, E); r.theta_count = nchunk;
        }
    }
    BankStreamLaunch bsl;
    int nchunk4[4] = {0, 0, 0, 0}, ntheta4[4] = {0, 0, 0, 0};
    if (streamed) {
        plan_backward_bank_stream(bank_a, bank_use, e_unit4, coefq4, nchunk4, ntheta4, through_nei, &bsl);
        bsl.x_split = rows_split ? 1 : 0;
        if (project) { bsl.a.proj_dz = tp.dz; bsl.a.proj_w1 = tp.w1; bsl.a.proj_H = tp.H; bsl.a.proj_HP = tp.HP; bsl.a.proj_K = tp.K; }
        if (project && switches().tail_project_in_prepass >= 2) {
            e = fj.refork(1);
            if (e != hipSuccess) return api_hip_fail("stream fork", e);
            e = launch_pending_tail_projection(fj.p->aux[0], false);
            if (e != hipSuccess) return api_hip_fail("deferred tail projection launch", e);
        }
        { BwdTimer t(st, 0); e = launch_coef_prepare(bsl, st); }
        if (e != hipSuccess) return api_hip_fail("coefficient pre-pass launch", e);
        e = fj.refork(1);
        if (e != hipSuccess) return api_hip_fail("stream fork", e);
    }
    if (rows_streamed && any_bank && grad_x) {
        BwdTimer t(st, 1);
        e = launch_backward_rows_stream(bank_a, bank_use, streamed ? coefq4 : nullptr, st);
        if (e != hipSuccess) return api_hip_fail("streamed rows launch", e);
    }
    if (any_bank) {
        hipStream_t st_bank = fj.stream(1, &e);
        if (e != hipSuccess) return api_hip_fail("stream fork", e);
        if (project) {
            e = launch_pending_tail_projection(st_bank, false);
            if (e != hipSuccess) return api_hip_fail("deferred tail projection launch", e);
        }
        if (st_bank != st) {
            e = launch_pending_tail_reduce(st_bank);
            if (e != hipSuccess) return api_hip_fail("deferred tail reduction launch", e);
        }
        {
            BwdTimer t(st_bank, 2);
            if (streamed) e = launch_backward_bank_stream(bsl, st_bank);
            else e = launch_backward_bank_fused(bank_a, bank_use, nchunk4, ntheta4, st_bank);
        }
        if (e != hipSuccess) return api_hip_fail("fused bank gradient launch", e);
        for (int i = 0; i < 4; ++i)
            if (bank_use[i]) {
                reduce[i].nchunk = nchunk4[i];
                reduce[i].theta_src = bank_a[i].theta_slab; reduce[i].theta_stride = 4; reduce[i].theta_count = ntheta4[i];
            }
    }
    const bool split = fj.two_way && !bank_on_main && fj.used[0];
    if (!split) {
        e = fj.end();
        if (e != hipSuccess) return api_hip_fail("stream join", e);
    }
    hipStream_t st_reduce = st;
    if (split) {
        st_reduce = fj.stream(1, &e);
        if (e != hipSuccess) return api_hip_fail("stream fork", e);
    }
    { BwdTimer t(st_reduce, 3); e = launch_bank_reduce_all(reduce, st_reduce); }
    if (e != hipSuccess) return api_hip_fail("bank gradient reduce launch", e);
    if (grad_x && n_edges == 0) {
        if (n_atoms) e = hipMemset2DAsync(grad_x, (size_t)grad_x_stride * sizeof(float), 0, (size_t)F * sizeof(float), (size_t)n_atoms, st);
        if (e != hipSuccess) return api_hip_fail("zero input gradient", e);
    } else if (grad_x) {
        BwdTimer t(st, 4);
        if (gb_gather) {
            e = launch_backward_gather_grad_blocks((const float*)(ws + w.contrib), (F + 3) / 4 * 4, scatter_rowptr, scatter_rows, x, x_stride,
                                                   inv_norm, n_atoms, F, grad_x, grad_x_stride, st, rows_split, gb);
            if (e == hipSuccess) g_grad_blocks_launches.fetch_add(1);
        } else
        e = launch_backward_gather((const float*)(ws + w.contrib), (F + 3) / 4 * 4, base, scatter_rowptr, scatter_rows, x,
                                   x_stride, inv_norm, n_atoms, F, grad_x, grad_x_stride, variant != 1, st, rows_split);
        if (e != hipSuccess) return api_hip_fail("backward gather launch", e);
    }
    if (split && defer_bank && fj.used[0] && !fj.used[1] && !fj.used[2]) {
        fj.p->deferred = true;
    } else if (split) {
        e = fj.end();
        if (e != hipSuccess) return api_hip_fail("stream join", e);
    }
    return 0;
}

int mkgnn_backward_streams(const mkgnn_kernel_bank banks[MKGNN_MAX_DEGREE], const mkgnn_degree_bucket buckets[MKGNN_MAX_DEGREE],
                           const float* x, int64_t x_stride, int64_t n_atoms, int32_t F, int32_t E) {
    if (!banks || !buckets) return 0;
    return plan_conv_backward(conv_shape(banks, buckets, F, E, n_atoms, x, x_stride, 0), 0).covers ? 1 : 0;
}

int mkgnn_rows_split_supported(const mkgnn_kernel_bank banks[MKGNN_MAX_DEGREE], const mkgnn_degree_bucket buckets[MKGNN_MAX_DEGREE],
                               int64_t x_stride, int64_t out_stride, int64_t n_atoms, int32_t F, int32_t E) {
    if (!banks || !buckets || F < 1 || E < 1) return 0;
    const ConvShape s = conv_shape(banks, buckets, F, E, n_atoms, nullptr, x_stride, out_stride);
    return rows_split_covered(s, plan_conv_forward(s, 0)) ? 1 : 0;
}

int mkgnn_debug_conv_dispatch(const mkgnn_kernel_bank banks[MKGNN_MAX_DEGREE], const mkgnn_degree_bucket buckets[MKGNN_MAX_DEGREE],
                              const float* x, int64_t x_stride, int64_t out_stride, int64_t n_atoms, int32_t F, int32_t E,
                              int32_t fwd_variant, int32_t bwd_variant, int32_t want_grad_x, const float* grad_x, int64_t grad_x_stride,
                              int32_t out[11]) {
    const char* who = "mkgnn_debug_conv_dispatch";
    if (!banks || !buckets || !out) return api_fail("%s: null pointer", who);
    fwd_variant &= ~(MKGNN_VARIANT_BLOCK_ROWS | MKGNN_VARIANT_BANK_PREPARED | MKGNN_VARIANT_ROWS_SPLIT);
    bwd_variant &= ~(MKGNN_BACKWARD_DEFER_BANK | MKGNN_BACKWARD_THROUGH_NEIGHBOURS | MKGNN_BACKWARD_ROWS_SPLIT);
    if (fwd_variant < 0 || fwd_variant > 3 || bwd_variant < 0 || bwd_variant > 2)
        return api_fail("%s: variants %d / %d", who, fwd_variant, bwd_variant);
    const FwdDispatch fwd = plan_conv_forward(conv_shape(banks, buckets, F, E, n_atoms, x, x_stride, out_stride), fwd_variant);
    const BwdDispatch bwd = plan_conv_backward(conv_shape(banks, buckets, F, E, n_atoms, x, x_stride, 0, want_grad_x ? grad_x : nullptr,
                                                          grad_x_stride), bwd_variant);
    for (int i = 0; i < 4; ++i) { out[i] = fwd.deg[i]; out[4 + i] = bwd.deg[i]; }
    out[8] = bwd.bank_fused; out[9] = bwd.rows_streamed; out[10] = bwd.bank_streamed;
    return 0;
}

int mkgnn_backward_join(void* stream) {
    DegreeStreams* p = degree_streams();
    if (!p || !p->deferred) return 0;
    p->deferred = false;
    hipError_t e = hipEventRecord(p->join[0], p->aux[0]);
    if (e == hipSuccess) e = hipStreamWaitEvent((hipStream_t)stream, p->join[0], 0);
    return e == hipSuccess ? 0 : api_hip_fail("mkgnn_backward_join", e);
}

int mkgnn_segment_sum_rows(const float* in, int64_t in_stride, const int32_t* rowptr, const int32_t* col, int64_t n_rows,
                           int32_t width, float* out, int64_t out_stride, float* inv_norm, void* stream) {
    if (n_rows < 0 || width <= 0 || width > 16384 || in_stride < width || out_stride < width)
        return api_fail("mkgnn_segment_sum_rows: bad shape");
    if (n_rows && (!in || !rowptr || !out)) return api_fail("mkgnn_segment_sum_rows: null pointer");
    hipError_t e = launch_segment_sum(in, in_stride, rowptr, col, n_rows, width, out, out_stride, inv_norm, (hipStream_t)stream);
    return e == hipSuccess ? 0 : api_hip_fail("mkgnn_segment_sum_rows", e);
}

int mkgnn_segment_sum_block_rows(const float* in, int64_t in_stride, const int32_t* rowptr, const int32_t* col,
                                 const int8_t* degree, int64_t n_rows, const int32_t num_kernels[MKGNN_MAX_DEGREE],
                                 int32_t mode, float* out, int64_t out_stride, float* inv_norm, void* stream) {
    const char* who = "mkgnn_segment_sum_block_rows";
    if (mode < 1 || mode > 3) return api_fail("%s: mode %d (1 = block-row sources, 2 = block-row destinations, 3 = 1 with pre-split output)", who, mode);
    if (mode == 3 && !inv_norm) return api_fail("%s: mode 3 (pre-split rows) needs inv_norm", who);
    if (!num_kernels) return api_fail("%s: num_kernels is null", who);
    int width = 0;
    for (int i = 0; i < MKGNN_MAX_DEGREE; ++i) {
        if (num_kernels[i] < 0 || num_kernels[i] > 255) return api_fail("%s: num_kernels[%d] = %d outside 0..255", who, i, num_kernels[i]);
        width += num_kernels[i];
    }
    if (n_rows < 0 || width <= 0 || in_stride < width || out_stride < width) return api_fail("%s: bad shape", who);
    if (n_rows == 0) return 0;
    if (!in || !rowptr || !col || !out || (mode == 2 && !degree)) return api_fail("%s: null pointer", who);
    if (!segment_sum_blocks_supported(in, in_stride, n_rows, width, out, out_stride))
        return api_fail("%s: needs 16-byte aligned rows (strides multiples of 4 floats), at most 255 columns and fewer than 2^28 rows", who);
    hipError_t e = launch_segment_sum_blocks(in, in_stride, rowptr, col, degree, n_rows, width, num_kernels, mode, out, out_stride,
                                             inv_norm, (hipStream_t)stream);
    return e == hipSuccess ? 0 : api_hip_fail(who, e);
// ... 4 lines not shown
```

molkgnn_amd/csrc/kgnn_csr.hip:

```cpp
#include <hip/hip_runtime.h>
#include <cstdint>
#include <cstdlib>
#include "kgnn_common.h"
#include "kgnn_launch.h"
#include "kgnn_split.h"

#include <atomic>
#include <type_traits>

namespace mkgnn {

typedef mkgnn_f32x4 f32x4;

struct CsrArgs {
    const float* src; int64_t ss;
    const int32_t* rowptr; const int32_t* idx;
    int64_t n; int width;
    float* out; int64_t os;
    float* inv_out;
    const float* x; int64_t xs; const float* inv;
    const int8_t* deg8;
    uint64_t blk_off, blk_len;
    int fixed4;
    int split_out;
    int x_split;
    const int8_t* present8;
};

template <int LPR>
__device__ __forceinline__ float group_sum(float v) {
#pragma unroll
    for (int o = LPR / 2; o > 0; o >>= 1) v += __shfl_xor(v, o, 64);
    return v;
}

__device__ __forceinline__ f32x4 keep_if(f32x4 v, bool keep) {
    const uint32_t m = keep ? 0xFFFFFFFFu : 0u;
#pragma unroll
    for (int c = 0; c < 4; ++c) v[c] = __uint_as_float(__float_as_uint(v[c]) & m);
    return v;
}

__device__ __forceinline__ f32x4 mask_cols(f32x4 v, int col, int width) {
#pragma unroll
    for (int c = 0; c < 4; ++c) v[c] = (col + c < width) ? v[c] : 0.f;
    return v;
}

template <int LPR, bool GATHER, int BLK = 0, int CPL = 1, bool PM = false>
__global__ void __launch_bounds__(256) csr_rows_kernel(CsrArgs a) {
    static_assert(!(GATHER && BLK), "block rows: segment sums only");
    static_assert(!PM || GATHER, "present blocks: the gather only");
    static_assert(CPL == 1 || CPL == 2, "one or two chunks per lane");
    constexpr int RPW = 64 / LPR, SEG = 4;
    static_assert(LPR >= SEG, "one index per lane of a row group");
    const int lane = threadIdx.x & 63;
    const int sub = lane / LPR, l = lane % LPR;
    int col[CPL], colc[CPL];
    bool active[CPL];
#pragma unroll
    for (int q = 0; q < CPL; ++q) {
        col[q] = 4 * (l + q * LPR);
        active[q] = col[q] < a.width;
        colc[q] = active[q] ? col[q] : 0;
    }
    const int n = (int)a.n;
    const int wave0 = (int)((blockIdx.x * blockDim.x + threadIdx.x) >> 6);
    const int nwaves = (int)((gridDim.x * blockDim.x) >> 6);
    const int ngroups = (n + RPW - 1) / RPW;
    int last = a.rowptr[n] - 1;
    const int32_t* idxp = last >= 0 ? a.idx : a.rowptr;
    last = last >= 0 ? last : 0;

    auto segment = [&](int g, int& lo, int& hi, int& dg) -> int {
        const int j = g * RPW + sub;
        const int jc = (j < n && g < ngroups) ? j : n - 1;
        lo = a.rowptr[(uint32_t)jc];
        hi = a.rowptr[(uint32_t)jc + 1];
        if constexpr (BLK == 2) dg = a.deg8[(uint32_t)jc];
        if constexpr (PM) dg = a.present8[(uint32_t)jc];
        if (j >= n || g >= ngroups) hi = lo;
        return jc;
    };
    auto block_of = [&](int d, int& b0, int& b1) {
        b0 = (int)((a.blk_off >> (8 * (d & 7))) & 0xFF);
        b1 = b0 + (int)((a.blk_len >> (8 * (d & 7))) & 0xFF);
    };
    uint32_t keep_tab[CPL], col_tab[CPL];
#pragma unroll
    for (int q = 0; q < CPL; ++q) keep_tab[q] = col_tab[q] = 0;
    if constexpr (BLK == 1) {
#pragma unroll
        for (int d = 1; d <= 4; ++d) {
            int b0, b1;
            block_of(d, b0, b1);
            const int lo4 = b0 & ~3, hi4 = (b1 - 1) & ~3;
#pragma unroll
            for (int q = 0; q < CPL; ++q) {
                const int lo = min(max(b0 - col[q], 0), 4), hi = min(max(b1 - col[q], 0), 4);
                const uint32_t m = hi > lo ? (1u << hi) - (1u << lo) : 0u;
                int cc = colc[q] < lo4 ? lo4 : (colc[q] > hi4 ? hi4 : colc[q]);
                if (b1 <= b0) cc = 0;
                keep_tab[q] |= m << (4 * d);
                col_tab[q] |= (uint32_t)(cc >> 2) << (6 * d);
            }
        }
    }
    uint32_t pm_blocks[CPL], pm_first = 0;
    int pm_c[CPL];
    bool pm_keep[CPL];
#pragma unroll
    for (int q = 0; q < CPL; ++q) { pm_blocks[q] = 0; pm_c[q] = colc[q]; pm_keep[q] = true; }
    if constexpr (PM) {
#pragma unroll
        for (int q = 0; q < CPL; ++q) pm_blocks[q] = active[q] ? grad_blocks_of_chunk(a.blk_off, a.blk_len, col[q]) : 0u;
#pragma unroll
        for (int d = 1; d <= 4; ++d) {
            int b0, b1;
            block_of(d, b0, b1);
            pm_first |= (uint32_t)(b0 >> 2) << (8 * (d - 1));
        }
    }
    auto present_of = [&](int mask8) {
        if constexpr (PM) {
            const uint32_t m = (uint32_t)mask8 & 15u;
            const uint32_t first = (pm_first >> ((8 * (uint32_t)__builtin_ctz(m | 16u)) & 31u)) & 0xFFu;
#pragma unroll
            for (int q = 0; q < CPL; ++q) {
                pm_keep[q] = m == 0 || (m & pm_blocks[q]) != 0;
                pm_c[q] = pm_keep[q] ? colc[q] : (int)(first << 2);
            }
        }
    };
    auto row_load = [&](int rid_raw, int dst_b0, int dst_b1, f32x4 (&v)[CPL]) {
        int row = rid_raw, c[CPL];
#pragma unroll
        for (int q = 0; q < CPL; ++q) c[q] = PM ? pm_c[q] : colc[q];
        if constexpr (BLK == 1) {
            const uint32_t d6 = 6 * ((uint32_t)rid_raw >> 28);
            row = rid_raw & 0x0FFFFFFF;
#pragma unroll
            for (int q = 0; q < CPL; ++q) c[q] = (int)((col_tab[q] >> d6) & 63) << 2;
        } else if constexpr (BLK == 2) {
            const int lo4 = dst_b0 & ~3, hi4 = (dst_b1 - 1) & ~3;
#pragma unroll
            for (int q = 0; q < CPL; ++q) {
                c[q] = c[q] < lo4 ? lo4 : (c[q] > hi4 ? hi4 : c[q]);
                if (dst_b1 <= dst_b0) c[q] = 0;
            }
        }
        const float* base = a.src + (uint64_t)(uint32_t)row * (uint32_t)a.ss;
#pragma unroll
        for (int q = 0; q < CPL; ++q) {
#ifdef MKGNN_CSR_NT_LOAD
            if constexpr (GATHER) { v[q] = __builtin_nontemporal_load((const f32x4*)(base + (uint32_t)c[q])); continue; }
#endif
            v[q] = *(const f32x4*)(base + (uint32_t)c[q]);
        }
    };
    auto row_keep = [&](const f32x4 (&v)[CPL], int rid_raw, bool valid, f32x4 (&acc)[CPL], bool first) {
        if constexpr (BLK == 1) {
            const uint32_t d4 = valid ? 4 * ((uint32_t)rid_raw >> 28) : 0;
#pragma unroll
            for (int q = 0; q < CPL; ++q) {
                const int m = (int)(keep_tab[q] >> d4);
                f32x4 w = v[q];
#pragma unroll
                for (int c = 0; c < 4; ++c)
                    w[c] = __uint_as_float(__float_as_uint(w[c]) & (uint32_t)__builtin_amdgcn_sbfe(m, c, 1));
                acc[q] = first ? w : acc[q] + w;
            }
        } else {
#pragma unroll
            for (int q = 0; q < CPL; ++q) {
                const f32x4 w = keep_if(v[q], PM ? (valid && pm_keep[q]) : valid);
                acc[q] = first ? w : acc[q] + w;
            }
        }
    };
    auto idx_issue = [&](int lo, int hi, int k0) -> int {
        const int u_mine = l & (SEG - 1);
        int k = k0 + u_mine < hi ? k0 + u_mine : lo;
        k = k < last ? k : last;
        return idxp[(uint32_t)k];
    };
    auto idx_bcast = [&](int mine, int (&rid)[SEG]) {
#pragma unroll
        for (int u = 0; u < SEG; ++u) rid[u] = __shfl(mine, sub * LPR + u, 64);
    };

    int lo_c, hi_c, lo_n, hi_n, dg_c = 0, dg_n = 0;
    int g = wave0;
    int j_c = segment(g, lo_c, hi_c, dg_c);
    int mine_c = idx_issue(lo_c, hi_c, lo_c);
    int j_n = segment(g + nwaves, lo_n, hi_n, dg_n);
    int mine_n, lo_nn, hi_nn, dg_nn, j_nn;
    auto body = [&](auto kc) {
        constexpr int K = decltype(kc)::value;
        dg_nn = 0;
        int d0 = 0, d1 = 0;
        if constexpr (BLK == 2) block_of(dg_c, d0, d1);
        present_of(dg_c);
        int rid_c[SEG];
        idx_bcast(mine_c, rid_c);
        f32x4 v[SEG][CPL];
#pragma unroll
        for (int u = 0; u < K; ++u) row_load(rid_c[u], d0, d1, v[u]);
        f32x4 xv[CPL];
        float iv = 0.f;
        if constexpr (GATHER) {
            const float* xrow = a.x + (uint64_t)(uint32_t)j_c * (uint32_t)a.xs;
#pragma unroll
            for (int q = 0; q < CPL; ++q) xv[q] = *(const f32x4*)(xrow + (PM ? pm_c[q] : colc[q]));
            iv = a.inv[j_c];
        }
        mine_n = idx_issue(lo_n, hi_n, lo_n);
        j_nn = segment(g + 2 * nwaves, lo_nn, hi_nn, dg_nn);
        f32x4 acc[CPL];
        row_keep(v[0], rid_c[0], lo_c < hi_c, acc, true);
#pragma unroll
        for (int u = 1; u < K; ++u) row_keep(v[u], rid_c[u], lo_c + u < hi_c, acc, false);
        if (K == SEG && __any(hi_c - lo_c > SEG)) {
            for (int k0 = lo_c + SEG; __any(k0 < hi_c); k0 += SEG) {
                int rid[SEG];
                idx_bcast(idx_issue(lo_c, hi_c, k0), rid);
                f32x4 w[SEG][CPL];
#pragma unroll
                for (int u = 0; u < SEG; ++u) row_load(rid[u], d0, d1, w[u]);
#pragma unroll
                for (int u = 0; u < SEG; ++u) row_keep(w[u], rid[u], k0 + u < hi_c, acc, false);
            }
        }
#pragma unroll
        for (int q = 0; q < CPL; ++q) acc[q] = mask_cols(acc[q], active[q] ? col[q] : a.width, a.width);
        const bool row_ok = g * RPW + sub < n;
        if constexpr (GATHER) {
            const float xscale = a.x_split ? split_row_inv(iv) : iv;
            f32x4 xh[CPL];
            float dotp = 0.f;
#pragma unroll
            for (int q = 0; q < CPL; ++q) {
                if (a.x_split) { xv[q] = split_row_value(xv[q]); }
                xh[q] = mask_cols(xv[q], active[q] ? col[q] : a.width, a.width) * xscale;
                if constexpr (PM) xh[q] = keep_if(xh[q], pm_keep[q]);
                float dq = acc[q][0] * xh[q][0];
                dq = fmaf(acc[q][1], xh[q][1], dq); dq = fmaf(acc[q][2], xh[q][2], dq); dq = fmaf(acc[q][3], xh[q][3], dq);
                dotp = q == 0 ? dq : dotp + dq;
            }
            dotp = group_sum<LPR>(dotp);
            const bool clamped = iv >= (1.f / MKGNN_EPS);
            float* dst = a.out + (uint64_t)(uint32_t)j_c * (uint32_t)a.os;
#pragma unroll
            for (int q = 0; q < CPL; ++q) {
                f32x4 r;
#pragma unroll
                for (int c = 0; c < 4; ++c) r[c] = clamped ? acc[q][c] * iv : (acc[q][c] - dotp * xh[q][c]) * iv;
                if (row_ok && active[q] && (!PM || pm_keep[q])) *(f32x4*)(dst + col[q]) = r;
            }
        } else if constexpr (BLK == 2) {
            float* drow = a.out + (uint64_t)(uint32_t)j_c * (uint32_t)a.os;
#pragma unroll
            for (int q = 0; q < CPL; ++q) {
                if (row_ok && active[q] && col[q] + 3 >= d0 && col[q] < d1) {
                    float* dst = drow + col[q];
                    if (col[q] >= d0 && col[q] + 3 < d1) *(f32x4*)dst = acc[q];
                    else {
#pragma unroll
                        for (int c = 0; c < 4; ++c)
                            if (col[q] + c >= d0 && col[q] + c < d1) dst[c] = acc[q][c];
                    }
                }
            }
        } else {
            f32x4 stored[CPL];
#pragma unroll
            for (int q = 0; q < CPL; ++q) stored[q] = acc[q];
            if (a.inv_out) {
                float ss = 0.f;
#pragma unroll
                for (int q = 0; q < CPL; ++q) {
                    float sq = acc[q][0] * acc[q][0];
                    sq = fmaf(acc[q][1], acc[q][1], sq); sq = fmaf(acc[q][2], acc[q][2], sq); sq = fmaf(acc[q][3], acc[q][3], sq);
                    ss = q == 0 ? sq : ss + sq;
                }
                ss = group_sum<LPR>(ss);
                const float inv = 1.f / fmaxf(sqrtf(ss), MKGNN_EPS);
                if (row_ok && l == 0) a.inv_out[j_c] = inv;
                if (a.split_out) {
#pragma unroll
                    for (int q = 0; q < CPL; ++q) stored[q] = split_row_store(acc[q], inv);
                }
            }
            float* dst = a.out + (uint64_t)(uint32_t)j_c * (uint32_t)a.os;
#pragma unroll
            for (int q = 0; q < CPL; ++q)
                if (row_ok && active[q]) *(f32x4*)(dst + col[q]) = stored[q];
        }
    };
    for (; g < ngroups; g += nwaves) {
        const int len = hi_c - lo_c;
        const int need = a.fixed4 ? SEG : 1 + (int)__any(len >= 2) + (int)__any(len >= 3) + (int)__any(len >= 4);
        switch (need) {
            case 1: body(std::integral_constant<int, 1>{}); break;
            case 2: body(std::integral_constant<int, 2>{}); break;
            case 3: body(std::integral_constant<int, 3>{}); break;
            default: body(std::integral_constant<int, SEG>{}); break;
        }
        lo_c = lo_n; hi_c = hi_n; j_c = j_n; dg_c = dg_n; mine_c = mine_n;
        lo_n = lo_nn; hi_n = hi_nn; j_n = j_nn; dg_n = dg_nn;
    }
}

template <int LPR>
__global__ void __launch_bounds__(256) row_inv_norm_aligned_kernel(const float* __restrict__ x, int64_t xs, int64_t n, int width,
                                                                   float* __restrict__ inv) {
    constexpr int RPW = 64 / LPR;
    const int lane = threadIdx.x & 63;
    const int sub = lane / LPR, l = lane % LPR, col = 4 * l;
    const bool active = col < width;
    const int64_t wave0 = ((int64_t)blockIdx.x * blockDim.x + threadIdx.x) >> 6;
    const int64_t nwaves = ((int64_t)gridDim.x * blockDim.x) >> 6;
    const int64_t ngroups = (n + RPW - 1) / RPW;
    for (int64_t g = wave0; g < ngroups; g += 2 * nwaves) {
        f32x4 v[2];
        int64_t j[2];
#pragma unroll
        for (int u = 0; u < 2; ++u) {
            j[u] = (g + u * nwaves) * RPW + sub;
            const int64_t jc = j[u] < n ? j[u] : n - 1;
            v[u] = *(const f32x4*)(x + jc * xs + (active ? col : 0));
        }
#pragma unroll
        for (int u = 0; u < 2; ++u) {
            const f32x4 m = mask_cols(v[u], active ? col : width, width);
            float ss = m[0] * m[0];
            ss = fmaf(m[1], m[1], ss); ss = fmaf(m[2], m[2], ss); ss = fmaf(m[3], m[3], ss);
            ss = group_sum<LPR>(ss);
            if (j[u] < n && l == 0) inv[j[u]] = 1.f / fmaxf(sqrtf(ss), MKGNN_EPS);
        }
    }
}

template <int LPR>
__global__ void __launch_bounds__(256) row_presplit_kernel(const float* __restrict__ x, int64_t xs, int64_t n, int width,
                                                           float* __restrict__ inv, float* __restrict__ out, int64_t os) {
    constexpr int RPW = 64 / LPR;
    const int lane = threadIdx.x & 63;
    const int sub = lane / LPR, l = lane % LPR, col = 4 * l;
    const bool active = col < width;
    const int64_t wave0 = ((int64_t)blockIdx.x * blockDim.x + threadIdx.x) >> 6;
    const int64_t nwaves = ((int64_t)gridDim.x * blockDim.x) >> 6;
    const int64_t ngroups = (n + RPW - 1) / RPW;
    for (int64_t g = wave0; g < ngroups; g += nwaves) {
        const int64_t j = g * RPW + sub;
        const int64_t jc = j < n ? j : n - 1;
        const f32x4 m = mask_cols(*(const f32x4*)(x + jc * xs + (active ? col : 0)), active ? col : width, width);
        float ss = m[0] * m[0];
        ss = fmaf(m[1], m[1], ss); ss = fmaf(m[2], m[2], ss); ss = fmaf(m[3], m[3], ss);
        ss = group_sum<LPR>(ss);
        const float iv = 1.f / fmaxf(sqrtf(ss), MKGNN_EPS);
        if (j < n && l == 0) inv[j] = iv;
        if (j < n && active) *(f32x4*)(out + j * os + col) = split_row_store(m, iv);
    }
}

static inline int csr_grid(int64_t n, int rpw) {
    int64_t groups = (n + rpw - 1) / rpw;
    int64_t blocks = (groups + 3) / 4;
    if (blocks < 1) blocks = 1;
    const int64_t cap = switches().csr_blocks;
    if (blocks > cap) blocks = cap;
    return (int)blocks;
}

static inline int lanes_per_row(int width) { return width <= 32 ? 8 : width <= 64 ? 16 : width <= 128 ? 32 : 64; }

bool aligned_rows(const void* p, int64_t stride, int width) {
    return ((uintptr_t)p & 15) == 0 && stride % 4 == 0 && stride >= (width + 3) / 4 * 4;
}

bool try_rows_presplit(const float* x, int64_t xs, int64_t n, int width, float* inv, float* out, int64_t os, hipStream_t st, hipError_t* err) {
    if (n == 0 || width > 256 || !aligned_rows(x, xs, width) || !aligned_rows(out, os, width)) return false;
    const int lpr = lanes_per_row(width);
    const int64_t groups = (n + 64 / lpr - 1) / (64 / lpr);
    int64_t blocks = (groups + 3) / 4;
    if (blocks < 1) blocks = 1;
    if (blocks > 256 * 16) blocks = 256 * 16;
    switch (lpr) {
        case 8: row_presplit_kernel<8><<<(int)blocks, 256, 0, st>>>(x, xs, n, width, inv, out, os); break;
        case 16: row_presplit_kernel<16><<<(int)blocks, 256, 0, st>>>(x, xs, n, width, inv, out, os); break;
        case 32: row_presplit_kernel<32><<<(int)blocks, 256, 0, st>>>(x, xs, n, width, inv, out, os); break;
        default: row_presplit_kernel<64><<<(int)blocks, 256, 0, st>>>(x, xs, n, width, inv, out, os); break;
// ... 32 lines not shown
    a.fixed4 = switches().csr_fixed4;
    const int lpr = lanes_per_row(a.width);
    if (csr_chunks<GATHER, BLK>() == 2) {
        switch (lpr) {
            case 8: csr_rows_kernel<4, GATHER, BLK, 2, PM><<<csr_grid(a.n, 16), 256, 0, st>>>(a); break;
            case 16: csr_rows_kernel<8, GATHER, BLK, 2, PM><<<csr_grid(a.n, 8), 256, 0, st>>>(a); break;
            case 32: csr_rows_kernel<16, GATHER, BLK, 2, PM><<<csr_grid(a.n, 4), 256, 0, st>>>(a); break;
            default: csr_rows_kernel<32, GATHER, BLK, 2, PM><<<csr_grid(a.n, 2), 256, 0, st>>>(a); break;
        }
    } else {
        switch (lpr) {
            case 8: csr_rows_kernel<8, GATHER, BLK, 1, PM><<<csr_grid(a.n, 8), 256, 0, st>>>(a); break;
            case 16: csr_rows_kernel<16, GATHER, BLK, 1, PM><<<csr_grid(a.n, 4), 256, 0, st>>>(a); break;
            case 32: csr_rows_kernel<32, GATHER, BLK, 1, PM><<<csr_grid(a.n, 2), 256, 0, st>>>(a); break;
            default: csr_rows_kernel<64, GATHER, BLK, 1, PM><<<csr_grid(a.n, 1), 256, 0, st>>>(a); break;
        }
    }
    return hipGetLastError();
}

template <bool GATHER>
static hipError_t launch_csr(const CsrArgs& a, hipStream_t st) { return launch_csr_rows<GATHER, 0>(a, st); }

template <int BLK>
static hipError_t launch_csr_blocks(const CsrArgs& a, hipStream_t st) { return launch_csr_rows<false, BLK>(a, st); }

bool segment_sum_blocks_supported(const float* in, int64_t is, int64_t n, int width, const float* out, int64_t os) {
    return n > 0 && n < (1 << 28) && width <= 255 && aligned_rows(in, is, width) && aligned_rows(out, os, width);
}

hipError_t launch_segment_sum_blocks(const float* in, int64_t is, const int32_t* rowptr, const int32_t* col, const int8_t* deg8,
                                     int64_t n, int width, const int32_t L[4], int mode, float* out, int64_t os,
                                     float* inv_norm, hipStream_t st) {
    CsrArgs a{};
    a.src = in; a.ss = is; a.rowptr = rowptr; a.idx = col; a.n = n; a.width = width; a.out = out; a.os = os;
    a.inv_out = (mode == 1 || mode == 3) ? inv_norm : nullptr;
    a.split_out = mode == 3 ? 1 : 0;
    a.deg8 = deg8;
    int off = 0;
    for (int d = 1; d <= 4; ++d) {
        a.blk_off |= (uint64_t)off << (8 * d);
        a.blk_len |= (uint64_t)L[d - 1] << (8 * d);
        off += L[d - 1];
    }
    return mode != 2 ? launch_csr_blocks<1>(a, st) : launch_csr_blocks<2>(a, st);
}

bool try_segment_sum_aligned(const float* in, int64_t is, const int32_t* rowptr, const int32_t* col, int64_t n, int width,
                             float* out, int64_t os, float* inv_norm, hipStream_t st, hipError_t* err) {
    if (n == 0 || n >= (1 << 30) || !col || width > 256 || !aligned_rows(in, is, width) || !aligned_rows(out, os, width)) return false;
    CsrArgs a{};
    a.src = in; a.ss = is; a.rowptr = rowptr; a.idx = col; a.n = n; a.width = width; a.out = out; a.os = os;
    a.inv_out = inv_norm;
    *err = launch_csr<false>(a, st);
    return true;
}

bool backward_gather_aligned_supported(const float* contrib, int64_t cs, const int32_t* rows, const float* x, int64_t xs, int64_t n, int F,
                                       const float* gx, int64_t gxs) {
    return n > 0 && n < (1 << 30) && rows && F <= 256 && aligned_rows(contrib, cs, F) && aligned_rows(x, xs, F) && aligned_rows(gx, gxs, F);
}

bool try_backward_gather_aligned(const float* contrib, int64_t cs, const int32_t* rowptr, const int32_t* rows, const float* x,
                                 int64_t xs, const float* inv, int64_t n, int F, float* gx, int64_t gxs, hipStream_t st,
                                 hipError_t* err, bool x_split) {
    if (!backward_gather_aligned_supported(contrib, cs, rows, x, xs, n, F, gx, gxs)) return false;
    CsrArgs a{};
    a.src = contrib; a.ss = cs; a.rowptr = rowptr; a.idx = rows; a.n = n; a.width = F; a.out = gx; a.os = gxs;
    a.x = x; a.xs = xs; a.inv = inv; a.x_split = x_split ? 1 : 0;
    *err = launch_csr<true>(a, st);
    return true;
}

hipError_t launch_backward_gather_grad_blocks(const float* contrib, int64_t cs, const int32_t* rowptr, const int32_t* rows,
                                              const float* x, int64_t xs, const float* inv, int64_t n, int F, float* gx, int64_t gxs,
                                              hipStream_t st, bool x_split, const GradBlocks& gb) {
    CsrArgs a{};
    a.src = contrib; a.ss = cs; a.rowptr = rowptr; a.idx = rows; a.n = n; a.width = F; a.out = gx; a.os = gxs;
    a.x = x; a.xs = xs; a.inv = inv; a.x_split = x_split ? 1 : 0;
    a.present8 = gb.present8; a.blk_off = gb.blk_off; a.blk_len = gb.blk_len;
    return launch_csr_rows<true, 0, true>(a, st);
}

extern "C" int mkgnn_debug_backward_gather(const float* contrib, int64_t cs, const int32_t* rowptr, const int32_t* rows, const float* x,
                                           int64_t xs, const float* inv, int64_t n, int32_t F, float* gx, int64_t gxs, int32_t x_split,
                                           void* stream) {
    hipError_t e = hipSuccess;
    if (!try_backward_gather_aligned(contrib, cs, rowptr, rows, x, xs, inv, n, F, gx, gxs, (hipStream_t)stream, &e, x_split != 0)) return -1;
    return e == hipSuccess ? 0 : 1;
}

bool try_row_inv_norm_aligned(const float* x, int64_t xs, int64_t n, int width, float* inv, hipStream_t st, hipError_t* err) {
    if (n == 0 || width > 256 || !aligned_rows(x, xs, width)) return false;
    const int lpr = lanes_per_row(width);
    const int64_t groups = (n + 64 / lpr - 1) / (64 / lpr);
    int64_t blocks = (groups + 7) / 8;
    if (blocks < 1) blocks = 1;
    if (blocks > 256 * 16) blocks = 256 * 16;
    switch (lpr) {
        case 8: row_inv_norm_aligned_kernel<8><<<(int)blocks, 256, 0, st>>>(x, xs, n, width, inv); break;
        case 16: row_inv_norm_aligned_kernel<16><<<(int)blocks, 256, 0, st>>>(x, xs, n, width, inv); break;
        case 32: row_inv_norm_aligned_kernel<32><<<(int)blocks, 256, 0, st>>>(x, xs, n, width, inv); break;
        default: row_inv_norm_aligned_kernel<64><<<(int)blocks, 256, 0, st>>>(x, xs, n, width, inv); break;
    }
    *err = hipGetLastError();
    return true;
}

}
```

molkgnn_amd/csrc/kgnn_launch.h:

```cpp
#pragma once
#include "kgnn_common.h"
#include "kgnn_switches.h"

#include <atomic>

namespace mkgnn {

struct PrepArgs {
    mkgnn_kernel_bank bank[MKGNN_MAX_DEGREE];
    float* cen[MKGNN_MAX_DEGREE];
    float* sup[MKGNN_MAX_DEGREE];
    float* edg[MKGNN_MAX_DEGREE];
    float* icen[MKGNN_MAX_DEGREE];
    float* isup[MKGNN_MAX_DEGREE];
    float* iedg[MKGNN_MAX_DEGREE];
    int8_t* chir[MKGNN_MAX_DEGREE];
    float* mix[MKGNN_MAX_DEGREE];
    float* padded[MKGNN_MAX_DEGREE];
    float* edge_padded[MKGNN_MAX_DEGREE];
    int row_start[MKGNN_MAX_DEGREE + 1];
    int F, E;
};

struct FwdArgs {
// ... 156 lines not shown
    const int32_t *rin, *cin, *rout, *cout;
    const int32_t *mol_ptr, *atom_mol;
    int64_t n_atoms, n_mols, n_loss;
    const float *b1, *w2, *b2, *wh, *bh, *y;
    int H, G;
    float drop_p; const int64_t* rng;
    float* emb; int64_t es;
    float* pred;
    float* slab; int slab_stride;
    int mg;
    float rdrop_p;
    const float* sw; const int32_t* wids; int64_t n_sw;
    const float* pw;
};
constexpr int TAIL_MAX_BLOCKS = 768;
constexpr int TAIL_B1 = 0, TAIL_W2 = 32, TAIL_B2 = 32 + 1024, TAIL_WH = TAIL_B2 + 32, TAIL_BH = TAIL_WH + 32, TAIL_LOSS = TAIL_BH + 1,
              TAIL_SLAB = (TAIL_LOSS + 1 + 3) / 4 * 4;
hipError_t launch_pending_tail_reduce(hipStream_t st, bool* launched = nullptr);
struct TailProjection {
    const float* dsim; int64_t dss;
    const float* dz; const float* w1;
    int H, HP, K;
    int off[MKGNN_MAX_DEGREE], L[MKGNN_MAX_DEGREE];
    const int64_t* sel[MKGNN_MAX_DEGREE]; int64_t cnt[MKGNN_MAX_DEGREE];
};
bool pending_tail_projection(TailProjection* out);
hipError_t launch_pending_tail_projection(hipStream_t st, bool full);
extern std::atomic<long long> g_tail_projection_launches[3];
int tail_group_size(int64_t n_loss_mols);
int tail_middle_blocks(int64_t n_loss_mols);
hipError_t launch_tail_middle(const TailMidArgs& a, int nb, int loss_kind, hipStream_t st);
hipError_t launch_tail_score(const TailMidArgs& a, int nb, hipStream_t st);
struct TailMcArgs {
    TailMidArgs m;
    int S;
    float* samples; int64_t ss;
    float *mean, *std, *acq;
    float alpha, beta;
};
hipError_t launch_tail_score_mc(const TailMcArgs& a, int nb, hipStream_t st);

struct AtomContribArgs {
    const float* z;
    const int32_t *rin, *cin; int64_t n;
    const float *b1, *w2, *b2;
    const float* wh; int64_t wh_stride;
    int H, G, T;
    float* out; int64_t os;
};
constexpr int ATOM_CONTRIB_MAX_BLOCKS = 1024;
hipError_t launch_atom_contrib(const AtomContribArgs& a, hipStream_t st);

struct BankStreamLaunch { BankStreamArgs a; int nb, prep_blocks, KC; size_t lds_bytes; int x_split; };
void plan_backward_bank_stream(const BwdArgs a4[4], const bool use[4], const float* const e_unit[4], float* const coefq[4],
                               int nchunk_out[4], int ntheta_out[4], bool through_nei, BankStreamLaunch* out);
hipError_t launch_coef_prepare(const BankStreamLaunch& p, hipStream_t st);
hipError_t launch_backward_bank_stream(const BankStreamLaunch& p, hipStream_t st);
struct GradBlocks { const int8_t* present8; uint64_t blk_off, blk_len; };
bool take_grad_blocks_hint(GradBlocks& out);
extern std::atomic<long long> g_grad_blocks_launches;
#ifdef __HIPCC__
__host__ __device__ __forceinline__ uint32_t grad_blocks_of_chunk(uint64_t blk_off, uint64_t blk_len, int col) {
    uint32_t m = 0;
#pragma unroll
    for (int d = 1; d <= 4; ++d) {
        const int b0 = (int)((blk_off >> (8 * d)) & 0xFF), b1 = b0 + (int)((blk_len >> (8 * d)) & 0xFF);
        if (b1 > b0 && col + 3 >= b0 && col < b1) m |= 1u << (d - 1);
    }
    return m;
}
#endif
bool rows_stream_supported(int d, int F, int E, int L);
hipError_t launch_backward_rows_stream(const BwdArgs a4[4], const bool use[4], float* const coefq[4], hipStream_t st);
bool mfma_backward_supported(int d, int F, int E, int L, int64_t xs, bool x_aligned, int64_t n_atoms);
hipError_t launch_backward_rows_mfma(int d, const BwdArgs& a, int* ntheta_out, hipStream_t st);
hipError_t launch_backward_gather(const float* contrib, int64_t cs, int64_t n_contrib_rows, const int32_t* rowptr,
                                  const int32_t* rows, const float* x, int64_t xs, const float* inv, int64_t n, int F,
                                  float* gx, int64_t gxs, bool allow_fast, hipStream_t st, bool x_split = false);
bool backward_gather_aligned_supported(const float* contrib, int64_t cs, const int32_t* rows, const float* x, int64_t xs, int64_t n, int F,
                                       const float* gx, int64_t gxs);
hipError_t launch_backward_gather_grad_blocks(const float* contrib, int64_t cs, const int32_t* rowptr, const int32_t* rows,
                                              const float* x, int64_t xs, const float* inv, int64_t n, int F, float* gx, int64_t gxs,
                                              hipStream_t st, bool x_split, const GradBlocks& gb);
bool segment_sum_blocks_supported(const float* in, int64_t is, int64_t n, int width, const float* out, int64_t os);
hipError_t launch_segment_sum_blocks(const float* in, int64_t is, const int32_t* rowptr, const int32_t* col, const int8_t* deg8,
                                     int64_t n, int width, const int32_t L[4], int mode, float* out, int64_t os,
                                     float* inv_norm, hipStream_t st);
bool try_segment_sum_aligned(const float* in, int64_t is, const int32_t* rowptr, const int32_t* col, int64_t n, int width,
                             float* out, int64_t os, float* inv_norm, hipStream_t st, hipError_t* err);
bool try_backward_gather_aligned(const float* contrib, int64_t cs, const int32_t* rowptr, const int32_t* rows, const float* x,
                                 int64_t xs, const float* inv, int64_t n, int F, float* gx, int64_t gxs, hipStream_t st,
                                 hipError_t* err, bool x_split = false);
bool try_rows_presplit(const float* x, int64_t xs, int64_t n, int width, float* inv, float* out, int64_t os, hipStream_t st, hipError_t* err);
bool try_row_inv_norm_aligned(const float* x, int64_t xs, int64_t n, int width, float* inv, hipStream_t st, hipError_t* err);
hipError_t launch_segment_sum(const float* in, int64_t is, const int32_t* rowptr, const int32_t* col, int64_t n,
                              int width, float* out, int64_t os, float* inv_norm, hipStream_t st);

struct PerDeviceOnce {
    std::atomic<bool> done[16];
    PerDeviceOnce() { for (auto& d : done) d.store(false); }
    int pending() {
        int dev = 0;
        if (hipGetDevice(&dev) != hipSuccess || dev < 0 || dev >= 16) return 0;
        return done[dev].load(std::memory_order_acquire) ? -1 : dev;
    }
    void set(int dev) { if (dev >= 0 && dev < 16) done[dev].store(true, std::memory_order_release); }
};

struct GridCaps { std::atomic<int> fwd{0}, rows{0}, bank{0}; };
extern GridCaps g_grid_caps;
struct PlanInfo { std::atomic<int> blocks{0}, min_iters{0}, max_iters{0}, launches{0}; };
extern PlanInfo g_last_plan[3];
inline int grid_cap(const std::atomic<int>& cap, int dflt) {
    const int c = cap.load(std::memory_order_relaxed);
    return (c >= 8 && c <= FUSED_MAX_BLOCKS) ? c : dflt;
}
inline void note_plan(int which, int blocks, int ng, const int64_t* tiles_of, const int* count, const int* nstream_of) {
    int lo = 1 << 30, hi = 0;
    for (int g = 0; g < ng; ++g) {
        const int64_t streams = (int64_t)count[g] * nstream_of[g];
        const int it = (int)((tiles_of[g] + streams - 1) / streams);
        if (it < lo) lo = it;
        if (it > hi) hi = it;
    }
    g_last_plan[which].blocks.store(blocks); g_last_plan[which].min_iters.store(ng ? lo : 0); g_last_plan[which].max_iters.store(hi);
}

int api_fail(const char* fmt, ...);
int api_hip_fail(const char* what, hipError_t e);
struct Span { const void* p; size_t n; };
int spans_disjoint(const char* who, const Span* writes, int n_writes, const Span* reads, int n_reads, const char* reads_text,
                   const char* writes_text);

int bwd_split_mode();

}
```

molkgnn_amd/csrc/kgnn_switches.h:

```cpp
#pragma once
#include <stdio.h>
#include <stdlib.h>

#ifndef MKGNN_FWD_PP_DEFAULT
#define MKGNN_FWD_PP_DEFAULT 0
#endif
#ifndef MKGNN_FWD_PAIR_DEFAULT
#define MKGNN_FWD_PAIR_DEFAULT 0
#endif
#ifndef MKGNN_FWD_SPLIT_DEFAULT
#define MKGNN_FWD_SPLIT_DEFAULT 1
#endif
#ifndef MKGNN_BWD_SPLIT_DEFAULT
#define MKGNN_BWD_SPLIT_DEFAULT 1
#endif

namespace mkgnn {

struct Switches {
    bool serial;
    bool fork_in_graph;
    bool no_mfma_bwd;
    bool fork_mode;
    bool bank_fused;
    bool rows_stream;
    bool bank_stream;
    bool fwd_stream;
    bool bf16_stream;
    bool rows_split;
    bool grad_blocks;
    int tail_project_in_prepass;
    bool bn_one_launch;
    bool bn_merge;
    char helper_priority;
    int fwd_pp;
    bool fwd_pp_env;
    int fwd_split;
    int bwd_split;
    int fwd_pair;
    int rows_stream_blocks;
    int bank_stream_blocks;
    int bank_blocks;
    int csr_blocks;
    int csr_fixed4;
    int csr_cpl;
    bool stream_cost_set;
    double stream_cost[4];
};

inline const Switches& switches() {
    static const Switches table = [] {
        auto is_set = [](const char* name) { return getenv(name) != nullptr; };
        auto not_0 = [](const char* name) { const char* e = getenv(name); return !(e && e[0] == '0'); };
        auto number = [](const char* name, int unset) { const char* e = getenv(name); return e ? atoi(e) : unset; };
        Switches s{};
        s.serial = is_set("MKGNN_SERIAL"); s.fork_in_graph = is_set("MKGNN_FORK_IN_GRAPH"); s.no_mfma_bwd = is_set("MKGNN_NO_MFMA_BWD");
        s.fork_mode = not_0("MKGNN_FORK_MODE"); s.bank_fused = not_0("MKGNN_BANK_FUSED"); s.rows_stream = not_0("MKGNN_ROWS_STREAM");
        s.bank_stream = not_0("MKGNN_BANK_STREAM"); s.fwd_stream = not_0("MKGNN_FWD_STREAM"); s.bf16_stream = not_0("MKGNN_BF16_STREAM");
        s.rows_split = not_0("MKGNN_ROWS_SPLIT"); s.grad_blocks = not_0("MKGNN_GRAD_BLOCKS"); s.tail_project_in_prepass = number("MKGNN_TAIL_PROJECT_IN_PREPASS", 2);
        if (const char* e = getenv("MKGNN_BN_ONE_LAUNCH")) s.bn_one_launch = e[0] == '1';
        s.bn_merge = not_0("MKGNN_BN_MERGE");
        if (const char* e = getenv("MKGNN_HELPER_PRIORITY")) s.helper_priority = e[0];
        s.fwd_pp = number("MKGNN_FWD_PP", MKGNN_FWD_PP_DEFAULT); s.fwd_pp_env = number("MKGNN_FWD_PP", 0) != 0;
        s.fwd_split = number("MKGNN_FWD_SPLIT", MKGNN_FWD_SPLIT_DEFAULT); s.bwd_split = number("MKGNN_BWD_SPLIT", MKGNN_BWD_SPLIT_DEFAULT);
        s.fwd_pair = number("MKGNN_FWD_PAIR", MKGNN_FWD_PAIR_DEFAULT); s.bank_blocks = number("MKGNN_BANK_BLOCKS", 0);
        s.rows_stream_blocks = number("MKGNN_ROWS_STREAM_BLOCKS", 0); s.bank_stream_blocks = number("MKGNN_BANK_STREAM_BLOCKS", 0);
        s.csr_blocks = number("MKGNN_CSR_BLOCKS", 256 * 16); s.csr_fixed4 = number("MKGNN_CSR_FIXED4", 0);
        s.csr_cpl = number("MKGNN_CSR_CPL", 0);
        if (const char* e = getenv("MKGNN_STREAM_COST"))
            s.stream_cost_set = sscanf(e, "%lf,%lf,%lf,%lf", &s.stream_cost[0], &s.stream_cost[1], &s.stream_cost[2], &s.stream_cost[3]) == 4;
        return s;
    }();
    return table;
}

}
```

molkgnn_amd/functional.py:

```python
from __future__ import annotations

import threading
from typing import List, Optional, Sequence, Tuple

import os

import torch

from . import _lib
from .plan import BatchPlan

PARAMS_PER_DEGREE = 7
VARIANTS = {"auto": 0, "generic": 1, "mfma": 2, "bf16": 3}
BACKWARD_VARIANTS = {"auto": 0, "generic": 1, "fast": 2}


def _f32c(t: torch.Tensor) -> torch.Tensor:
    if t.dtype != torch.float32:
        raise TypeError(f"expected float32, got {t.dtype}")
    return t if t.is_contiguous() else t.contiguous()


def _row_major(x: torch.Tensor) -> torch.Tensor:
    if x.dim() != 2 or x.dtype != torch.float32:
        raise TypeError(f"expected a 2-D float32 tensor, got {tuple(x.shape)} {x.dtype}")
    if x.shape[0] > 1 and x.stride(1) != 1:
        return x.contiguous()
    if x.shape[0] <= 1 and x.stride(-1) != 1:
        return x.contiguous()
    return x


def _aligned_rows(x: torch.Tensor) -> torch.Tensor:
    x = _row_major(x)
    if x.shape[0] == 0 or (_stride0(x) % 4 == 0 and x.data_ptr() % 16 == 0):
        return x
    n, f = x.shape
    store = torch.zeros((n, f + (-f) % 4), dtype=x.dtype, device=x.device)
    store[:, :f] = x
    return store[:, :f]


def _stride0(x: torch.Tensor) -> int:
    return x.stride(0) if x.shape[0] > 1 else max(x.stride(0), x.shape[1])


def _banks(params: Sequence[torch.Tensor], F: int, E: int):
    banks = _lib.Banks4()
    Ls = []
    keep = []
    for i in range(4):
        xc, xs, es, ps, ts, tc, te = params[i * PARAMS_PER_DEGREE:(i + 1) * PARAMS_PER_DEGREE]
        d = i + 1
        L = int(xc.shape[0])
        if L and (tuple(xs.shape) != (L, d, F) or tuple(xc.shape) != (L, F) or tuple(es.shape) != (L, d, E)):
            raise ValueError(f"degree {d}: kernel shapes {tuple(xc.shape)} {tuple(xs.shape)} {tuple(es.shape)} "
                             f"do not match F={F}, E={E}")
        xc, xs, es, ps = _f32c(xc), _f32c(xs), _f32c(es), _f32c(ps)
        keep += [xc, xs, es, ps]
        b = banks[i]
        b.num_kernels = L
        b.x_center, b.x_support, b.edge_attr_support = _lib.ptr(xc), _lib.ptr(xs), _lib.ptr(es)
        b.p_support = _lib.ptr(ps) if ps.shape[-1] == 3 else None
        b.support_attr_sc_weight, b.center_attr_sc_weight, b.edge_attr_support_sc_weight = \
            ts.data_ptr(), tc.data_ptr(), te.data_ptr()
        Ls.append(L)
    return banks, Ls, keep


def _buckets(plan: BatchPlan, E: int, need_p: bool):
    bk = _lib.Buckets4()
    for i, b in enumerate(plan.buckets):
        k = bk[i]
        k.count = b.count
        if b.count:
            if b.e_nei.numel() != b.count * b.degree * E:
                raise ValueError(f"nei_edge_attr_deg{b.degree} has {b.e_nei.numel()} values, expected "
                                 f"{b.count}x{b.degree}x{E}")
            k.selected_index, k.nei_index, k.nei_edge_attr = b.sel.data_ptr(), b.nei.data_ptr(), b.e_nei.data_ptr()
            k.nei_edge_unit = _lib.ptr(b.e_unit(E))
            if need_p and b.degree == 4:
                if b.p_focal is None or b.p_focal.shape[-1] != 3:
                    raise ValueError("chirality (degree 4, last layer) needs 3-D coordinates")
                k.p_focal, k.nei_p = b.p_focal.data_ptr(), b.nei_p.data_ptr()
    return bk


def workspace_bytes(Ls: Sequence[int], F: int, E: int, n_atoms: int, n_slots: int) -> int:
    return int(_lib.load().mkgnn_workspace_bytes(_lib.Int32x4(*Ls), F, E, n_atoms, n_slots))


def row_inv_norm(x: torch.Tensor) -> torch.Tensor:
    _lib.require_gpu_tensor(x, "x")
    x = _row_major(x)
    inv = torch.empty(x.shape[0], dtype=torch.float32, device=x.device)
    with torch.cuda.device(x.device):
        _lib.check(_lib.load().mkgnn_row_inv_norm(x.data_ptr(), _stride0(x), x.shape[0], x.shape[1],
                                                  inv.data_ptr(), _lib.stream_ptr(x.device)), "mkgnn_row_inv_norm")
    return inv


BANK_PREPARED = 0x200
ROWS_SPLIT = 0x400
_SPLIT_ATTR = "_mkgnn_rows_split"


_PRODUCTS_EPOCH = 0


def debug_set_products(forward: int = -1, backward: int = -1) -> None:
    global _PRODUCTS_EPOCH
    lib = _lib.load()
    _lib.check(lib.mkgnn_debug_set_forward_products(int(forward)), "mkgnn_debug_set_forward_products")
    _lib.check(lib.mkgnn_debug_set_backward_products(int(backward)), "mkgnn_debug_set_backward_products")
    _PRODUCTS_EPOCH += 1


def is_rows_split(x: torch.Tensor) -> bool:
    tag = getattr(x, _SPLIT_ATTR, None)
    return tag is not None and tag == x._version


def mark_rows_split(x: torch.Tensor) -> torch.Tensor:
    setattr(x, _SPLIT_ATTR, x._version)
    return x


_GRAD_BLOCKS_ATTR = "_mkgnn_grad_blocks"
GRAD_BLOCKS = os.environ.get("MKGNN_GRAD_BLOCKS", "1")[:1] != "0"


def mark_grad_blocks(h: torch.Tensor, plan: BatchPlan, blocks) -> torch.Tensor:
    if GRAD_BLOCKS and h.is_cuda and plan.edge_index is not None:
        setattr(h, _GRAD_BLOCKS_ATTR, (h._version, plan, tuple(int(v) for v in blocks)))
    return h


def grad_blocks_of(x: torch.Tensor, plan: BatchPlan):
    tag = getattr(x, _GRAD_BLOCKS_ATTR, None)
    if tag is None or not GRAD_BLOCKS:
        return None
    version, tag_plan, blocks = tag
    if version != x._version or tag_plan is not plan or sum(blocks) != x.shape[1]:
        return None
    if getattr(x, "_backward_hooks", None) or x.retains_grad or torch.is_anomaly_enabled():
        return None
    return blocks


def debug_grad_blocks_launches() -> int:
    return int(_lib.load().mkgnn_debug_grad_blocks_launches())


def debug_poison_backward(on: bool) -> None:
    _lib.check(_lib.load().mkgnn_debug_poison_backward(int(bool(on))), "mkgnn_debug_poison_backward")


def presplit_rows(x: torch.Tensor) -> torch.Tensor:
    _lib.require_gpu_tensor(x, "x")
    x = _aligned_rows(x)
    n, F = x.shape
    F4 = F + (-F) % 4
    out = torch.zeros((n, F4), dtype=torch.float32, device=x.device)[:, :F]
    inv = torch.empty(n, dtype=torch.float32, device=x.device)
    with torch.cuda.device(x.device):
        _lib.check(_lib.load().mkgnn_rows_presplit(x.data_ptr(), _stride0(x), n, F, inv.data_ptr(), out.data_ptr(), F4,
                                                   _lib.stream_ptr(x.device)), "mkgnn_rows_presplit")
    setattr(out, _INV_ATTR, (inv, out._version))
    return mark_rows_split(out)


def rows_split_supported(plan: BatchPlan, params: Sequence[torch.Tensor], F: int, E: int, n_atoms: int) -> bool:
    banks, Ls, keep = _banks([p.detach() for p in params], F, E)
    buckets = _buckets(plan, E, False)
    F4, K4 = F + (-F) % 4, sum(Ls) + (-sum(Ls)) % 4
    return bool(_lib.load().mkgnn_rows_split_supported(banks, buckets, F4, K4, n_atoms, F, E))


class PreparedBank:
    __slots__ = ("ws", "key")

    def __init__(self, ws, key):
        self.ws, self.key = ws, key


def _prepared_key(params, F, E, n_atoms, n_slots):
    return (F, E, n_atoms, n_slots) + tuple((p.data_ptr(), p._version) for p in params)


TOUCH = os.environ.get("MKGNN_TOUCH", "1") != "0"


def plan_touch_list(plan: BatchPlan) -> List[torch.Tensor]:
    out = []
    for bk in plan.buckets:
        if bk.count:
            out += [bk.nei, bk.sel]
            if bk._e_unit is not None:
                out.append(bk._e_unit)
    if plan._csr_in_packed is not None:
        out += [t for t in plan._csr_in_packed if t is not None]
    if plan._present8 is not None:
        out.append(plan._present8)
    return [t for t in out if t.is_cuda and t.numel() * t.element_size() >= 4096][:16]


class touch_hint:

    def __init__(self, tensors):
        self.tensors = [t for t in (tensors or []) if t.is_cuda][:16] if TOUCH else []
        self.taken = False

    def __enter__(self):
        if self.tensors:
            import ctypes as C
            n = len(self.tensors)
            ptrs = (C.c_void_p * n)(*[t.data_ptr() for t in self.tensors])
            nbytes = (C.c_size_t * n)(*[t.numel() * t.element_size() for t in self.tensors])
            _lib.load().mkgnn_touch_hint(C.cast(ptrs, C.c_void_p), C.cast(nbytes, C.c_void_p), n)
        return self

    def __exit__(self, *exc):
        if self.tensors:
            self.taken = _lib.load().mkgnn_touch_hint(None, None, 0) == 0
        return False


def prepare_banks(params_per_call: Sequence[Sequence[torch.Tensor]], Fs: Sequence[int], E: int, n_atoms: int, n_slots: int,
                  side: Optional["torch.cuda.Stream"] = None, defer: bool = False):
    if defer and len(params_per_call) > 4:
# ... 128 lines not shown
    _USE_TORCH_OPS = bool(on)


def _op_lists(plan: BatchPlan, params, E: int, need_p: bool, saved_t, dev):
    none = torch.empty(0, dtype=torch.float32, device=dev)
    ps = []
    for i in range(4):
        xc, xs, es, p3, ts, tc, te = params[i * PARAMS_PER_DEGREE:(i + 1) * PARAMS_PER_DEGREE]
        ps += [_f32c(xc), _f32c(xs), _f32c(es), _f32c(p3), ts.detach(), tc.detach(), te.detach()]
    bk, counts = [], []
    for b in plan.buckets:
        counts.append(int(b.count))
        if not b.count:
            bk += [none] * 6
            continue
        if b.e_nei.numel() != b.count * b.degree * E:
            raise ValueError(f"nei_edge_attr_deg{b.degree} has {b.e_nei.numel()} values, expected {b.count}x{b.degree}x{E}")
        eu = b.e_unit(E)
        withp = need_p and b.degree == 4
        if withp and (b.p_focal is None or b.p_focal.shape[-1] != 3):
            raise ValueError("chirality (degree 4, last layer) needs 3-D coordinates")
        bk += [b.sel, b.nei, b.e_nei, b.p_focal if withp else none, b.nei_p if withp else none, eu if eu is not None else none]
    sv = []
    for pr, ch in saved_t:
        sv += [pr if pr is not None else none, ch if ch is not None else none]
    return ps, bk, counts, sv


def kernelsetconv_details(x, plan: BatchPlan, is_last_layer: bool, params, edge_attr_dim: int, variant: str = "auto",
                          raw: bool = False):
    with torch.no_grad():
        _, out, _, saved_t, _, _, _ = _forward_impl(x, plan, is_last_layer, VARIANTS[variant], 0, edge_attr_dim,
                                                 [p.detach() for p in params], True, _handed_inv_norm(x))
    if raw:
        return out, saved_t

    def unpack(pr, ch):
        if pr is None:
            return None, None, None
        best = pr[..., 3].contiguous().view(torch.int32).to(torch.uint8).t()
        return best, pr[..., :3].permute(2, 1, 0), (None if ch is None else ch.t())
    return out, [unpack(pr, ch) for pr, ch in saved_t]


DEFER_BANK = 0x100
THROUGH_NEIGHBOURS = 0x200


class _Deferred:
    active = False
    held: list = []
    seen: set = set()


class deferred_bank_gradients:

    def __enter__(self):
        if _Deferred.active:
            raise RuntimeError("deferred_bank_gradients regions do not nest")
        _Deferred.active, _Deferred.held, _Deferred.seen = True, [], set()
        return self

    def __exit__(self, *exc):
        _Deferred.active = False
        try:
            if _Deferred.held and torch.cuda.is_available():
                _lib.check(_lib.load().mkgnn_backward_join(_lib.stream_ptr(_Deferred.held[0][0].device)), "mkgnn_backward_join")
        finally:
            _Deferred.held, _Deferred.seen = [], set()
        return False


_CALL = threading.local()


class _KernelSetConvFn(torch.autograd.Function):

    @staticmethod
    def forward(ctx, x, plan: BatchPlan, is_last_layer: bool, variant: int, out_pad: int, E: int, inv, bwd_variant: int,
                propagate, prepared, *params):
        need_grad = any(ctx.needs_input_grad) and getattr(_CALL, "grad_enabled", True)
        ctx.bwd_variant = int(bwd_variant)
        ctx.grad_blocks = grad_blocks_of(x, plan) if (need_grad and bwd_variant != BACKWARD_VARIANTS["generic"]) else None
        x, out_full, inv, saved_t, Ls, ws, x_split = _forward_impl(x, plan, is_last_layer, variant, out_pad, E, params, need_grad,
                                                                   inv, prepared)
        ctx.x_split = x_split
        ctx.plan, ctx.is_last, ctx.E, ctx.Ls = plan, bool(is_last_layer), E, Ls
        ctx.ws = ws if need_grad else None
        ctx.param_versions = [p._version for p in params]
        ctx.saved_t = saved_t
        ctx.save_for_backward(x, inv, *params)
        ctx.propagate = bool(propagate)
        K = sum(Ls)
        sim_sc = out_full[:, :K] if out_full.shape[1] != K else out_full
        if not propagate:
            return sim_sc
        inv_h = torch.empty(x.shape[0], dtype=torch.float32, device=x.device)
        h = _segment_sum_blocks(sim_sc, plan.csr_in_packed, None, tuple(Ls), 3 if propagate == "split" else 1, (-K) % 4, inv_h)
        ctx.mark_non_differentiable(inv_h)
        ctx.set_materialize_grads(False)
        return h, inv_h

    @staticmethod
    def backward(ctx, grad_out, _grad_inv=None):
        lib = _lib.load()
        x, inv, *params = ctx.saved_tensors
        plan, E, Ls = ctx.plan, ctx.E, ctx.Ls
        n, F = x.shape
        dev = x.device
        if grad_out is None:
            return (None,) * (10 + len(params))
        g = _row_major(grad_out if grad_out.dtype == torch.float32 else grad_out.float())
        banks, _, keep = _banks(params, F, E)
        buckets = _buckets(plan, E, False)
        through = 0
        if ctx.propagate:
            with torch.cuda.device(dev):
                streams = ctx.bwd_variant != BACKWARD_VARIANTS["generic"] and \
                    lib.mkgnn_backward_streams(banks, buckets, x.data_ptr(), _stride0(x), n, F, E) == 1
            if streams and not os.environ.get("MKGNN_NO_THROUGH_NEIGHBOURS"):
                through = THROUGH_NEIGHBOURS
            else:
                K = sum(Ls)
                if _stride0(g) % 4 or g.data_ptr() % 16:
                    g = _aligned_rows(g)
                g = _segment_sum_blocks(g, plan.csr_out, plan.deg8, tuple(Ls), 2, (-K) % 4, None)
        saved = _lib.Saved4()
        for i, (pr, ch) in enumerate(ctx.saved_t):
            saved[i].pair_state = _lib.ptr(pr)
            saved[i].chirality = _lib.ptr(ch)
        grads = _lib.BankGrads4()
        gparams: List[Optional[torch.Tensor]] = []
        alive = []
        for i in range(4):
            xc, xs, es, ps, ts, tc, te = params[i * PARAMS_PER_DEGREE:(i + 1) * PARAMS_PER_DEGREE]
            gxc, gxs, ges = torch.empty_like(xc), torch.empty_like(xs), torch.empty_like(es)
            idle = plan.buckets[i].count == 0 or Ls[i] == 0
            gth = torch.zeros(3, dtype=torch.float32, device=dev) if idle else torch.empty(3, dtype=torch.float32, device=dev)
            alive += [gxc, gxs, ges, gth]
            gr = grads[i]
            gr.x_center, gr.x_support, gr.edge_attr_support = _lib.ptr(gxc), _lib.ptr(gxs), _lib.ptr(ges)
            gr.support_attr_sc_weight = gth.data_ptr()
            gr.center_attr_sc_weight = gth.data_ptr() + 4
            gr.edge_attr_support_sc_weight = gth.data_ptr() + 8
            if idle:
                gparams += [None] * PARAMS_PER_DEGREE
            else:
                gparams += [gxc, gxs, ges, None, gth[0].reshape(ts.shape), gth[1].reshape(tc.shape),
                            gth[2].reshape(te.shape)]
        rowptr, rows = plan.scatter
        with torch.cuda.device(dev):
            F4 = F + (-F) % 4
            gx = torch.empty((n, F4), dtype=torch.float32, device=dev)[:, :F] if ctx.needs_input_grad[0] else None
            ws_bytes = workspace_bytes(Ls, F, E, n, plan.n_slots)
            ws, ctx.ws = ctx.ws, None
            reuse = ws is not None and ws.numel() >= ws_bytes and \
                all(p._version == v for p, v in zip(params, ctx.param_versions))
            if not reuse:
                ws = torch.empty(ws_bytes, dtype=torch.uint8, device=dev)
            bwd_variant = ctx.bwd_variant | through | (ROWS_SPLIT if ctx.x_split else 0)
            live = [p for p in params if p.requires_grad]
            defer = _Deferred.active and all(p.grad is None and id(p) not in _Deferred.seen for p in live)
            if defer:
                bwd_variant |= DEFER_BANK
                _Deferred.seen.update(id(p) for p in live)
                _Deferred.held.append((x, inv, g, ws, ctx.saved_t, plan, params, [t for t in alive if t is not None and
                                                                                 all(t is not q for q in gparams)]))
            hinted = ctx.grad_blocks is not None and gx is not None
            present = plan.present8 if hinted else None
            if _USE_TORCH_OPS:
                ps, bkl, counts, sv = _op_lists(plan, params, E, False, ctx.saved_t, dev)
            try:
                if hinted:
                    _lib.check(lib.mkgnn_backward_grad_blocks(present.data_ptr(), _lib.Int32x4(*ctx.grad_blocks)),
                               "mkgnn_backward_grad_blocks")
                if _USE_TORCH_OPS:
                    _lib.load_torch_ops().kernelsetconv_backward(x, inv, ps, bkl, counts, E, bool(ctx.is_last), g, sv, rowptr, rows, gx,
                                                                 list(alive), ws, bool(reuse), bwd_variant)
                else:
                    _lib.check(lib.mkgnn_kernelsetconv_backward(
                        banks, buckets, x.data_ptr(), _stride0(x), inv.data_ptr(), n, F, E, int(ctx.is_last),
                        g.data_ptr(), _stride0(g), saved, rowptr.data_ptr(), rows.data_ptr(),
                        _lib.ptr(gx), F4, grads, ws.data_ptr(), ws_bytes, int(reuse), bwd_variant, _lib.stream_ptr(dev)),
                        "mkgnn_kernelsetconv_backward")
            finally:
                if hinted:
                    lib.mkgnn_backward_grad_blocks(None, None)
        del alive
        return (gx, None, None, None, None, None, None, None, None, None, *gparams)


BLOCK_ROWS = 0x100
_BLOCKS_ATTR = "_mkgnn_block_rows"


def kernelsetconv(x: torch.Tensor, plan: BatchPlan, is_last_layer: bool, params: Sequence[torch.Tensor],
                  edge_attr_dim: int, variant: str = "auto", out_pad: Optional[int] = None,
                  block_rows: bool = False, backward_variant: Optional[str] = None, propagate: bool = False,
                  prepared: Optional[PreparedBank] = None, grad_blocks: bool = False) -> torch.Tensor:
    if block_rows and out_pad not in (None, (-sum(int(p.shape[0]) for p in params[0::7])) % 4):
        raise ValueError("block_rows needs the default padded storage")
    if backward_variant is None:
        backward_variant = "generic" if variant == "generic" else "auto"
    _CALL.grad_enabled = torch.is_grad_enabled()
    if propagate:
        if not block_rows:
            raise ValueError("propagate=True continues on block rows: block_rows=True is required")
        if propagate not in (True, "split"):
            raise ValueError('propagate: False, True, or "split" (h written pre-split for the next kernelsetconv)')
        h, inv_h = _KernelSetConvFn.apply(x, plan, is_last_layer, VARIANTS[variant] | BLOCK_ROWS, out_pad, edge_attr_dim,
                                          _handed_inv_norm(x), BACKWARD_VARIANTS[backward_variant], propagate, prepared, *params)
        setattr(h, _INV_ATTR, (inv_h, h._version))
        if propagate == "split":
            mark_rows_split(h)
        if grad_blocks:
            mark_grad_blocks(h, plan, [int(p.shape[0]) for p in params[0::7]])
        return h
    out = _KernelSetConvFn.apply(x, plan, is_last_layer, VARIANTS[variant] | (BLOCK_ROWS if block_rows else 0), out_pad,
                                 edge_attr_dim, _handed_inv_norm(x), BACKWARD_VARIANTS[backward_variant], False, prepared,
                                 *params)
    if block_rows:
        setattr(out, _BLOCKS_ATTR, tuple(int(p.shape[0]) for p in params[0::7]))
    return out


FORWARD_FAMILIES = ("skip", "generic", "lds_bank", "streamed")
BACKWARD_FAMILIES = ("skip", "zero_fill", "generic", "lds_pair", "mfma_lds", "streamed")


def debug_conv_dispatch(x: torch.Tensor, plan: BatchPlan, params: Sequence[torch.Tensor], E: int, variant: str = "auto",
                        backward_variant: Optional[str] = None):
    if backward_variant is None:
        backward_variant = "generic" if variant == "generic" else "auto"
    x = _row_major(x) if variant == "generic" else _aligned_rows(x)
    n, F = x.shape
    banks, Ls, keep = _banks([p.detach() for p in params], F, E)
    buckets = _buckets(plan, E, False)
    K, F4 = sum(Ls), F + (-F) % 4
    out = (_lib.C.c_int32 * 11)()
    _lib.check(_lib.load().mkgnn_debug_conv_dispatch(banks, buckets, x.data_ptr(), _stride0(x), K + (-K) % 4, n, F, E, VARIANTS[variant],
                                                     BACKWARD_VARIANTS[backward_variant], 1, 16, F4, out), "mkgnn_debug_conv_dispatch")
    return ([FORWARD_FAMILIES[v] for v in out[0:4]], [BACKWARD_FAMILIES[v] for v in out[4:8]], tuple(int(v) for v in out[8:11]))


_INV_ATTR = "_mkgnn_inv_norm"


def _handed_inv_norm(x: torch.Tensor):
    tag = getattr(x, _INV_ATTR, None)
    if tag is None:
        return None
    inv, version = tag
    if version != x._version or inv.shape[0] != x.shape[0] or inv.device != x.device:
        return None
    return inv


class _SegmentSumFn(torch.autograd.Function):

    @staticmethod
    def forward(ctx, v, plan: BatchPlan, out_pad: int, blocks):
        _lib.require_gpu_tensor(v, "sim_sc")
        v = _row_major(v)
        ctx.plan = plan
        ctx.width = v.shape[1]
        ctx.blocks = blocks
        inv = torch.empty(v.shape[0], dtype=torch.float32, device=v.device)
        if blocks is not None:
            out = _segment_sum_blocks(v, plan.csr_in_packed, None, blocks, 1, out_pad, inv)
        else:
# ... 53 lines not shown
```

molkgnn_amd/readout.py:

```python
from __future__ import annotations

import ctypes

import weakref
from typing import Optional, Tuple

import os

import torch

from . import _lib
from .functional import _aligned_rows, _row_major, _stride0

_SEG_CACHE: dict = {}
_SEG_CACHE_MAX = 32


class MoleculeSegments:

    @classmethod
    def from_tensors(cls, mol_ptr: torch.Tensor, atom_mol: torch.Tensor, max_atoms: Optional[int] = None,
                     max_edges: Optional[int] = None) -> "MoleculeSegments":
        if mol_ptr.dtype != torch.int32 or atom_mol.dtype != torch.int32:
            raise TypeError("mol_ptr and atom_mol must be int32")
# ... 147 lines not shown
        return out

    @staticmethod
    def backward(ctx, grad_out):
        lib = _lib.load()
        sim, w1, b1, w2, b2, gate, gsum, pooled = ctx.saved_tensors
        seg, plan, blocks = ctx.seg, ctx.plan, ctx.blocks
        n, K = sim.shape
        H, G = w1.shape[0], w2.shape[0]
        dev = sim.device
        g = _row_major(grad_out if grad_out.dtype == torch.float32 else grad_out.float())
        hs = gate.shape[1]
        dz = torch.empty((n, hs), dtype=torch.float32, device=dev)
        K4 = K + (-K) % 4
        gsim = torch.empty((n, K4), dtype=torch.float32, device=dev)[:, :K] if ctx.needs_input_grad[0] else None
        gw1, gw2 = torch.empty_like(w1), torch.empty_like(w2)
        gb1 = torch.empty_like(b1) if b1 is not None else None
        gb2 = torch.empty_like(b2) if b2 is not None else None
        p = _params(w1, b1, w2, b2)
        bk = _sel_buckets(plan)
        rowptr, col = plan.csr_out
        with torch.cuda.device(dev):
            ws_bytes = int(lib.mkgnn_readout_blocks_workspace_bytes(K, H, G, seg.size))
            ws = torch.empty(ws_bytes, dtype=torch.uint8, device=dev)
            _lib.check(lib.mkgnn_readout_blocks_backward(
                p, sim.data_ptr(), _stride0(sim), _lib.Int32x4(*blocks), bk, n, rowptr.data_ptr(), col.data_ptr(),
                seg.mol_ptr.data_ptr(), seg.atom_mol.data_ptr(), seg.size, gate.data_ptr(), gsum.data_ptr(), pooled.data_ptr(),
                g.data_ptr(), _stride0(g), dz.data_ptr(), _lib.ptr(gsim), K4, gw1.data_ptr(), _lib.ptr(gb1),
                gw2.data_ptr(), _lib.ptr(gb2), ws.data_ptr(), ws_bytes, _lib.stream_ptr(dev)), "mkgnn_readout_blocks_backward")
        return gsim, gw1, gb1, gw2, gb2, None, None, None, None


def readout_blocks_supported(K: int, H: int, G: int, blocks) -> bool:
    return bool(_lib.load().mkgnn_readout_blocks_supported(int(K), int(H), int(G), _lib.Int32x4(*[int(b) for b in blocks])))


def readout_blocks(sim: torch.Tensor, plan, blocks, lin1: torch.nn.Linear, lin2: torch.nn.Linear,
                   dropout: Optional[torch.nn.Dropout], seg: "MoleculeSegments") -> torch.Tensor:
    H = lin1.weight.shape[0]
    p_drop = dropout.p if (dropout is not None and dropout.training) else 0.0
    keep = None
    if p_drop > 0.0:
        keep = torch.empty((sim.shape[0], H), dtype=torch.float32, device=sim.device)
        if p_drop >= 1.0:
            keep.zero_()
        else:
            keep.bernoulli_(1.0 - p_drop).mul_(1.0 / (1.0 - p_drop))
    return _ReadoutBlocksFn.apply(sim, lin1.weight, lin1.bias, lin2.weight, lin2.bias, keep, seg, plan, tuple(blocks))


_TORCH_READOUT_OK = os.environ.get("MKGNN_TORCH_READOUT", "") == "1"


def readout(h: torch.Tensor, lin1: torch.nn.Linear, lin2: torch.nn.Linear, dropout: Optional[torch.nn.Dropout],
            batch: torch.Tensor, size: Optional[int] = None, segments: Optional["MoleculeSegments"] = None) -> torch.Tensor:
    _lib.require_gpu_tensor(h, "node_representation")
    seg = segments if segments is not None else molecule_segments(batch, size)
    H, F = lin1.weight.shape
    G = lin2.weight.shape[0]
    p_drop = dropout.p if (dropout is not None and dropout.training) else 0.0
    if not readout_supported(F, H, G) and not _TORCH_READOUT_OK:
        raise _lib.MolKGNNLibraryError(
            f"readout: lin1 {F} -> {H}, lin2 -> {G} is outside the HIP readout kernels (F <= 128, H <= 64, G <= 64; inside "
            "MolKGNNNet the block-row readout takes up to 255 kernel columns); set MKGNN_TORCH_READOUT=1 to run this shape "
            "through PyTorch operators on the GPU instead")
    if not (seg.sorted and readout_supported(F, H, G) and h.shape[0] > 0 and seg.size > 0):
        z = swish(lin1(h))
        if dropout is not None:
            z = dropout(z)
        z = lin2(z)
        return torch.zeros(seg.size, G, dtype=z.dtype, device=z.device).index_add_(0, batch, z)
    keep = None
    if p_drop > 0.0:
        keep = torch.empty((h.shape[0], H), dtype=torch.float32, device=h.device)
        if p_drop >= 1.0:
            keep.zero_()
        else:
            keep.bernoulli_(1.0 - p_drop).mul_(1.0 / (1.0 - p_drop))
    return _ReadoutFn.apply(h, lin1.weight, lin1.bias, lin2.weight, lin2.bias, keep, seg)


class _BatchNormFn(torch.autograd.Function):
    @staticmethod
    def forward(ctx, x, weight, bias, bn: torch.nn.BatchNorm1d, use_batch_stats: bool, n_valid=None, companion=None, split_out=False):
        lib = _lib.load()
        ctx.n_valid = n_valid
        x = _row_major(x if x.dtype == torch.float32 else x.float())
        n, C = x.shape
        dev = x.device
        out = torch.empty((n, C), dtype=torch.float32, device=dev)
        save_mean = torch.empty(C, dtype=torch.float32, device=dev)
        save_invstd = torch.empty(C, dtype=torch.float32, device=dev)
        update = bn.training and bn.track_running_stats and bn.running_mean is not None
        rm = bn.running_mean if (update or not use_batch_stats) else None
        rv = bn.running_var if (update or not use_batch_stats) else None
        nbt = bn.num_batches_tracked if (update and bn.num_batches_tracked is not None) else None
        if nbt is not None and (nbt.dtype != torch.int64 or nbt.device != dev):
            raise _lib.MolKGNNLibraryError("num_batches_tracked must be an int64 tensor on the input's device")
        inv = torch.empty(n, dtype=torch.float32, device=dev) \
            if (C <= 32 and C % 4 == 0 and _stride0(x) % 4 == 0 and x.data_ptr() % 16 == 0) else None
        with torch.cuda.device(dev):
            ws_bytes = int(lib.mkgnn_batchnorm_workspace_bytes(C))
            ws = torch.empty(ws_bytes, dtype=torch.uint8, device=dev)
            st, keep, cws, cws_bytes = None, None, None, 0
            if companion is not None and use_batch_stats and bn.training:
                st, keep = _bn_stats_struct(*companion)
                cws_bytes = int(lib.mkgnn_batchnorm_stats_workspace_bytes(st.C))
                cws = torch.empty(cws_bytes, dtype=torch.uint8, device=dev)
            _lib.check(lib.mkgnn_batchnorm_forward_with_stats(
                x.data_ptr(), _stride0(x), n, C, _lib.ptr(weight), _lib.ptr(bias), _lib.ptr(rm), _lib.ptr(rv),
                float(bn.momentum if bn.momentum is not None else 0.0), float(bn.eps),
                int(use_batch_stats) | (2 if (split_out and inv is not None) else 0),
                out.data_ptr(), C, save_mean.data_ptr(), save_invstd.data_ptr(), _lib.ptr(inv), _lib.ptr(nbt),
                _lib.ptr(n_valid), ws.data_ptr(), ws_bytes, None if st is None else ctypes.byref(st), _lib.ptr(cws), cws_bytes,
                _lib.stream_ptr(dev)), "mkgnn_batchnorm_forward_with_stats")
            del keep
        ctx.use_batch_stats = use_batch_stats
        ctx.save_for_backward(x, weight, save_mean, save_invstd)
        ctx.wrote_split = bool(split_out and inv is not None)
        if inv is None:
            inv = torch.empty(0, dtype=torch.float32, device=dev)
        ctx.mark_non_differentiable(inv)
        ctx.set_materialize_grads(False)
        return out, inv

    @staticmethod
    def backward(ctx, grad_out, _g_inv=None):
        lib = _lib.load()
        if grad_out is None:
            return None, None, None, None, None, None, None, None
        x, weight, save_mean, save_invstd = ctx.saved_tensors
        n, C = x.shape
        dev = x.device
        g = _row_major(grad_out if grad_out.dtype == torch.float32 else grad_out.float())
        gx = torch.empty((n, C), dtype=torch.float32, device=dev) if ctx.needs_input_grad[0] else None
        gw = torch.empty(C, dtype=torch.float32, device=dev) if (weight is not None and ctx.needs_input_grad[1]) else None
        gb = torch.empty(C, dtype=torch.float32, device=dev) if ctx.needs_input_grad[2] else None
        with torch.cuda.device(dev):
            ws_bytes = int(lib.mkgnn_batchnorm_workspace_bytes(C))
            ws = torch.empty(ws_bytes, dtype=torch.uint8, device=dev)
            _lib.check(lib.mkgnn_batchnorm_backward(
                g.data_ptr(), _stride0(g), x.data_ptr(), _stride0(x), n, C, _lib.ptr(weight), save_mean.data_ptr(),
                save_invstd.data_ptr(), int(ctx.use_batch_stats), _lib.ptr(gx), C, _lib.ptr(gw), _lib.ptr(gb),
                _lib.ptr(ctx.n_valid), ws.data_ptr(), ws_bytes, _lib.stream_ptr(dev)), "mkgnn_batchnorm_backward")
        return gx, gw, gb, None, None, None, None, None


def _stats_supported(x: torch.Tensor, bn: torch.nn.BatchNorm1d) -> bool:
    return (x.is_cuda and x.dim() == 2 and 1 <= x.shape[1] <= 256 and x.shape[0] >= 1 and x.shape[1] == bn.num_features
            and bn.momentum is not None and bn.running_mean is not None and bn.running_mean.is_cuda)


def _bn_stats_struct(x: torch.Tensor, bn: torch.nn.BatchNorm1d, key: Optional[torch.Tensor], key_limit: Optional[torch.Tensor]):
    x = _row_major(x if x.dtype == torch.float32 else x.float())
    if (key is None) != (key_limit is None):
        raise ValueError("key and key_limit come together")
    if key is not None:
        if not (key.is_cuda and key.dtype == torch.int64 and key.is_contiguous() and key.numel() == x.shape[0]):
            raise ValueError("key must be a contiguous int64 GPU tensor with one entry per row")
        if not (key_limit.is_cuda and key_limit.dtype == torch.int64 and key_limit.numel() == 1):
            raise ValueError("key_limit must be a one-element int64 tensor on the GPU")
    nbt = bn.num_batches_tracked
    if nbt is not None and (nbt.dtype != torch.int64 or nbt.device != x.device):
        raise _lib.MolKGNNLibraryError("num_batches_tracked must be an int64 tensor on the input's device")
    st = _lib.BnStats(x.data_ptr(), _stride0(x), x.shape[0], x.shape[1], _lib.ptr(bn.running_mean), _lib.ptr(bn.running_var),
                      float(bn.momentum), _lib.ptr(nbt), _lib.ptr(key), _lib.ptr(key_limit))
    return st, (x, key, key_limit)


def update_running_stats(x: torch.Tensor, bn: torch.nn.BatchNorm1d, key: Optional[torch.Tensor] = None,
                         key_limit: Optional[torch.Tensor] = None) -> None:
    if not (bn.training and bn.track_running_stats and bn.running_mean is not None):
        return
    _lib.require_gpu_tensor(x, "x")
    if not _stats_supported(x, bn):
        if key is not None:
            if torch.cuda.is_current_stream_capturing():
                raise _lib.MolKGNNLibraryError("update_running_stats: a keyed batch outside the HIP kernels' limits (> 256 channels, "
                                               "momentum None, statistics off the GPU) cannot run inside a hipGraph capture")
            x = x[key < key_limit]
        bn(x)
        return
    lib = _lib.load()
    dev = x.device
    st, keep = _bn_stats_struct(x, bn, key, key_limit)
    with torch.cuda.device(dev):
        ws_bytes = int(lib.mkgnn_batchnorm_stats_workspace_bytes(st.C))
        ws = torch.empty(ws_bytes, dtype=torch.uint8, device=dev)
        _lib.check(lib.mkgnn_batchnorm_update_stats(ctypes.byref(st), ws.data_ptr(), ws_bytes, _lib.stream_ptr(dev)),
                   "mkgnn_batchnorm_update_stats")
    del keep


def batch_norm(x: torch.Tensor, bn: torch.nn.BatchNorm1d, n_valid: Optional[torch.Tensor] = None,
               companion=None, split_out: bool = False) -> torch.Tensor:
    _lib.require_gpu_tensor(x, "x")
    if n_valid is not None and not (n_valid.is_cuda and n_valid.dtype == torch.int64 and n_valid.numel() == 1):
        raise ValueError("n_valid must be a one-element int64 tensor on the GPU")
    if x.dim() != 2 or x.shape[1] != bn.num_features:
        raise ValueError(f"expected a [N, {bn.num_features}] input, got {tuple(x.shape)}")
    use_batch_stats = bn.training or bn.running_mean is None
    if companion is not None:
        x2, bn2 = companion[0], companion[1]
        if not (bn2.training and bn2.track_running_stats and bn2.running_mean is not None):
            companion = None
        elif not (_stats_supported(x2, bn2) and bn.training and use_batch_stats):
            update_running_stats(*companion)
            companion = None
    if x.shape[1] > 256 or x.shape[0] == 0 or (bn.training and bn.track_running_stats and bn.momentum is None):
        if n_valid is not None:
            raise ValueError("n_valid needs the HIP batch norm (<= 256 channels, momentum set)")
        if companion is not None:
            update_running_stats(*companion)
        return bn(x)
    if use_batch_stats and bn.training and x.shape[0] == 1:
        raise ValueError(f"Expected more than 1 value per channel when training, got input size {tuple(x.shape)}")
    out, inv = _BatchNormFn.apply(x, bn.weight, bn.bias, bn, use_batch_stats, n_valid, companion, split_out)
    if inv.numel():
        from .functional import _INV_ATTR, mark_rows_split
        setattr(out, _INV_ATTR, (inv, out._version))
        if split_out:
            mark_rows_split(out)
    return out


_HEAD_WS: dict = {}


def _head_workspace(dev, nbytes: int) -> torch.Tensor:
    held = _HEAD_WS.setdefault(str(dev), [])
    if not held or held[-1].numel() < nbytes:
        held.append(torch.empty(max(nbytes, 1 << 16), dtype=torch.uint8, device=dev))
    return held[-1]


_HEAD_RNG: dict = {}
_SPLIT_HEAD = os.environ.get("MKGNN_SPLIT_HEAD") == "1"


def head_rng_state(dev) -> torch.Tensor:
    st = _HEAD_RNG.get(str(dev))
    if st is None:
        seed = int(torch.randint(0, 2 ** 62, (1,), dtype=torch.int64).item())
        st = torch.tensor([seed, 0], dtype=torch.int64, device=dev)
        _HEAD_RNG[str(dev)] = st
    return st


def reset_head_rng(dev=None, seed=None) -> None:
    for k in ([str(dev)] if dev is not None else list(_HEAD_RNG)):
        _HEAD_RNG.pop(k, None)
        if seed is not None:
            _HEAD_RNG[k] = torch.tensor([int(seed), 0], dtype=torch.int64, device=torch.device(k))


_UNIT_SEEDS: list = []


def register_unit_gradient(one: torch.Tensor) -> None:
    if not any(t is one for t, _ in _UNIT_SEEDS):
        _UNIT_SEEDS.append((one, one._version))


def _is_unit_seed(grad: torch.Tensor) -> bool:
    for t, version in _UNIT_SEEDS:
        if t._version == version and t.device == grad.device and (grad is t or (
                grad.data_ptr() == t.data_ptr() and grad.numel() == 1 and grad.dtype == t.dtype)):
            return True
    return False


LOSS_KINDS = {"bce": _lib.LOSS_BCE_MEAN, "mse": _lib.LOSS_SQERR_MEAN, "mse_sum": _lib.LOSS_SQERR_SUM}


def loss_kind(loss: str) -> int:
    if loss not in LOSS_KINDS:
        raise ValueError(f"unknown loss {loss!r}: one of {sorted(LOSS_KINDS)}")
    return LOSS_KINDS[loss]


def _head_call(lib, name: str, kind: Optional[int], *args) -> None:
    if kind is None:
        _lib.check(getattr(lib, "mkgnn_bce_head_" + name)(*args), "mkgnn_bce_head_" + name)
    else:
        _lib.check(getattr(lib, "mkgnn_head_loss_" + name)(int(kind), *args), "mkgnn_head_loss_" + name)


class _BceHeadFn(torch.autograd.Function):
    @staticmethod
    def forward(ctx, emb, weight, bias, target, p_drop, n_rows, kind=None):
        lib = _lib.load()
        ctx.kind = kind
        emb = _row_major(emb if emb.dtype == torch.float32 else emb.float())
        ctx.rows_total = emb.shape[0]
        B, H = int(n_rows), emb.shape[1]
        dev = emb.device
        w = weight.reshape(-1).contiguous()
        y = target.reshape(-1).float().contiguous()
        pred = torch.empty(B, dtype=torch.float32, device=dev)
        loss = torch.empty((), dtype=torch.float32, device=dev)
        rng = head_rng_state(dev) if p_drop > 0.0 else None
        used = torch.empty(2, dtype=torch.int64, device=dev) if p_drop > 0.0 else None
        ctx.unit = None
        if any(ctx.needs_input_grad[:3]) and not _SPLIT_HEAD:
            gemb = None
# ... 1638 lines not shown
```

Before: 6.356 million molecules/s.

## Fuse batchnorm backward column sums into the conv backward gather kernel

When the first layer's input comes from a batchnorm whose input needs no gradient, the conv backward gather now accumulates the per-column sums BN needs for grad_weight and grad_bias. It does this directly from the gradient rows it computes and writes per-block partials, so grad_x is never materialised. The BN backward then only runs a small final reduction over those partials. This removes the grad_x write and the separate full read pass of BN backward, at the cost of ticket plumbing, thread-local hints and a per-call workspace allocation.

Result: slower. 6.260 million molecules/s (-1.5%).

```diff
diff --git a/include/molkgnn_hip.h b/include/molkgnn_hip.h
--- a/include/molkgnn_hip.h
+++ b/include/molkgnn_hip.h
@@ -248,6 +248,8 @@
                              const float* save_mean, const float* save_invstd, int32_t training,
                              float* grad_x, int64_t grad_x_stride, float* grad_weight, float* grad_bias,
                              const int64_t* n_valid_rows, void* workspace, size_t workspace_bytes, void* stream);
+int mkgnn_batchnorm_backward_from_partials(int32_t C, float* grad_weight, float* grad_bias, const void* workspace,
+                                           size_t workspace_bytes, void* stream);
 int mkgnn_debug_set_bn_merge(int32_t on);
 
 size_t mkgnn_rf_workspace_bytes(int64_t n_atoms);
@@ -277,6 +279,10 @@
 int mkgnn_plan_present_blocks(const mkgnn_degree_bucket buckets[MKGNN_MAX_DEGREE], int64_t n_atoms, const int32_t* in_rowptr,
                               const int32_t* in_col_packed, int8_t* present8, int8_t* contrib_present8, void* stream);
 int mkgnn_backward_grad_blocks(const int8_t* present8, const int32_t num_kernels[MKGNN_MAX_DEGREE]);
+int mkgnn_backward_bn_sums(const float* x_raw, int64_t x_raw_stride, const float* save_mean, const float* save_invstd,
+                           const int64_t* n_valid_rows, void* workspace, size_t workspace_bytes);
+int mkgnn_backward_bn_sums_taken(void);
+int64_t mkgnn_debug_bn_sums_launches(void);
 int64_t mkgnn_debug_grad_blocks_launches(void);
 int mkgnn_debug_poison_backward(int32_t enable);
 int mkgnn_debug_conv_dispatch(const mkgnn_kernel_bank banks[MKGNN_MAX_DEGREE], const mkgnn_degree_bucket buckets[MKGNN_MAX_DEGREE],
diff --git a/molkgnn_amd/_lib.py b/molkgnn_amd/_lib.py
--- a/molkgnn_amd/_lib.py
+++ b/molkgnn_amd/_lib.py
@@ -250,7 +250,8 @@
            "mkgnn_embed_neighbours_within", "mkgnn_embed_neighbours_within_workspace_bytes", "mkgnn_graph_components",
            "mkgnn_graph_components_workspace_bytes", "mkgnn_maxmin_pick", "mkgnn_maxmin_pick_workspace_bytes",
            "mkgnn_tail_score_mc", "mkgnn_tail_score_mc_workspace_bytes", "mkgnn_debug_set_bn_merge", "mkgnn_debug_conv_dispatch",
-           "mkgnn_bootstrap_roc", "mkgnn_bootstrap_roc_workspace_bytes")
+           "mkgnn_bootstrap_roc", "mkgnn_bootstrap_roc_workspace_bytes", "mkgnn_backward_bn_sums", "mkgnn_backward_bn_sums_taken",
+           "mkgnn_debug_bn_sums_launches", "mkgnn_batchnorm_backward_from_partials")
 
 _lib: Optional[C.CDLL] = None
 TORCH_LIB_PATH = os.path.join(os.path.dirname(LIB_PATH), "libmolkgnn_torch.so")
@@ -514,6 +515,14 @@
     lib.mkgnn_plan_present_blocks.argtypes = [Buckets4, I64, P, P, P, P, P]
     lib.mkgnn_backward_grad_blocks.restype = C.c_int
     lib.mkgnn_backward_grad_blocks.argtypes = [P, P]
+    lib.mkgnn_backward_bn_sums.restype = C.c_int
+    lib.mkgnn_backward_bn_sums.argtypes = [P, I64, P, P, P, P, C.c_size_t]
+    lib.mkgnn_backward_bn_sums_taken.restype = C.c_int
+    lib.mkgnn_backward_bn_sums_taken.argtypes = []
+    lib.mkgnn_debug_bn_sums_launches.restype = C.c_int64
+    lib.mkgnn_debug_bn_sums_launches.argtypes = []
+    lib.mkgnn_batchnorm_backward_from_partials.restype = C.c_int
+    lib.mkgnn_batchnorm_backward_from_partials.argtypes = [I32, P, P, P, C.c_size_t, P]
     lib.mkgnn_debug_grad_blocks_launches.restype = C.c_int64
     lib.mkgnn_debug_grad_blocks_launches.argtypes = []
     lib.mkgnn_debug_poison_backward.restype = C.c_int
diff --git a/molkgnn_amd/csrc/kgnn_batchnorm.hip b/molkgnn_amd/csrc/kgnn_batchnorm.hip
--- a/molkgnn_amd/csrc/kgnn_batchnorm.hip
+++ b/molkgnn_amd/csrc/kgnn_batchnorm.hip
@@ -5,6 +5,7 @@
 #include "kgnn_common.h"
 
 #include "kgnn_launch.h"
+#include "kgnn_bn_reduce.h"
 #include "kgnn_prepare.h"
 #include "kgnn_split.h"
 #include "../../include/molkgnn_hip.h"
@@ -13,13 +14,9 @@
 
 typedef mkgnn_f32x4 f32x4;
 
-#ifndef MKGNN_BN_BLOCKS
-#define MKGNN_BN_BLOCKS 256
-#endif
 #ifndef MKGNN_BN_AB
 #define MKGNN_BN_AB 0
 #endif
-constexpr int BN_MAIN_BLOCKS = MKGNN_BN_BLOCKS;
 constexpr int BN_SIDE_BLOCKS = 1024;
 struct BnSide {
     const float* x; int64_t xs; int64_t n; int C, CL, nblk;
@@ -70,40 +67,6 @@
 
 constexpr int BN_U = 16;
 constexpr int BN_UA = 8;
-
-__device__ __forceinline__ float bn_shfl_xor(float v, int o) { return __shfl_xor(v, o, 64); }
-__device__ __forceinline__ f32x4 bn_shfl_xor(f32x4 v, int o) {
-    return f32x4{__shfl_xor(v[0], o, 64), __shfl_xor(v[1], o, 64), __shfl_xor(v[2], o, 64), __shfl_xor(v[3], o, 64)};
-}
-__device__ __forceinline__ void bn_zero(float& v) { v = 0.f; }
-__device__ __forceinline__ void bn_zero(f32x4& v) { v = f32x4{0.f, 0.f, 0.f, 0.f}; }
-
-template <typename V> __device__ __forceinline__ V bn_reduce_rows(V v, int LW, V* shv) {
-    const int t = threadIdx.x;
-    for (int o = 32; o >= LW; o >>= 1) v = v + bn_shfl_xor(v, o);
-    __syncthreads();
-    int parts;
-    if (LW <= 64) {
-        if ((t & 63) < LW) shv[(t >> 6) * LW + (t & 63)] = v;
-        parts = 4;
-    } else {
-        shv[t] = v;
-        parts = 256 / LW;
-    }
-    __syncthreads();
-    V r;
-    bn_zero(r);
-    if (t < LW)
-        for (int k = 0; k < parts; ++k) r = r + shv[k * LW + t];
-    return r;
-}
-
-__device__ __forceinline__ void bn_share(int64_t nv, int nblk, int b, int64_t& lo, int64_t& hi) {
-    const int64_t per = (nv + nblk - 1) / nblk;
-    lo = per * b;
-    hi = lo + per < nv ? lo + per : nv;
-    if (lo > hi) lo = hi;
-}
 
 template <int MODE, int U>
 __device__ __forceinline__ void bn_pass_vec(const float* x, int64_t xs, const float* g, int64_t gs, int64_t lo, int64_t hi, int rsub, int RS,
@@ -1003,4 +966,18 @@
     return e == hipSuccess ? 0 : api_hip_fail("mkgnn_batchnorm_backward", e);
 }
 
-}
+int mkgnn_batchnorm_backward_from_partials(int32_t C, float* grad_weight, float* grad_bias, const void* ws, size_t ws_bytes, void* stream) {
+    const char* who = "mkgnn_batchnorm_backward_from_partials";
+    int CL;
+    if (int rc = bn_common(who, 1, C, CL)) return rc;
+    if (!ws || ws_bytes < mkgnn_batchnorm_workspace_bytes(C)) return api_fail("%s: workspace too small", who);
+    BnArgs a{};
+    a.C = C;
+    a.part1 = (float*)ws; a.part2 = a.part1 + (size_t)BN_BLOCKS * C;
+    a.gweight = grad_weight; a.gbias = grad_bias; a.merge = bn_merge_on();
+    bn_bwd_final_kernel<true><<<1, 256, 0, (hipStream_t)stream>>>(a, CL, BN_BLOCKS);
+    hipError_t e = hipGetLastError();
+    return e == hipSuccess ? 0 : api_hip_fail(who, e);
+}
+
+}
diff --git a/molkgnn_amd/csrc/kgnn_bn_reduce.h b/molkgnn_amd/csrc/kgnn_bn_reduce.h
--- /dev/null
+++ b/molkgnn_amd/csrc/kgnn_bn_reduce.h
@@ -0,0 +1,57 @@
+#pragma once
+#include <hip/hip_runtime.h>
+#include <cstdint>
+#include "kgnn_common.h"
+
+#ifndef MKGNN_BN_BLOCKS
+#define MKGNN_BN_BLOCKS 256
+#endif
+
+namespace mkgnn {
+
+constexpr int BN_MAIN_BLOCKS = MKGNN_BN_BLOCKS;
+
+struct BnSums {
+    const float* x_raw; int64_t xrs;
+    const float *save_mean, *save_invstd;
+    const int64_t* nvalid;
+    float *part1, *part2;
+};
+
+#ifdef __HIPCC__
+__device__ __forceinline__ float bn_shfl_xor(float v, int o) { return __shfl_xor(v, o, 64); }
+__device__ __forceinline__ mkgnn_f32x4 bn_shfl_xor(mkgnn_f32x4 v, int o) {
+    return mkgnn_f32x4{__shfl_xor(v[0], o, 64), __shfl_xor(v[1], o, 64), __shfl_xor(v[2], o, 64), __shfl_xor(v[3], o, 64)};
+}
+__device__ __forceinline__ void bn_zero(float& v) { v = 0.f; }
+__device__ __forceinline__ void bn_zero(mkgnn_f32x4& v) { v = mkgnn_f32x4{0.f, 0.f, 0.f, 0.f}; }
+
+template <typename V> __device__ __forceinline__ V bn_reduce_rows(V v, int LW, V* shv) {
+    const int t = threadIdx.x;
+    for (int o = 32; o >= LW; o >>= 1) v = v + bn_shfl_xor(v, o);
+    __syncthreads();
+    int parts;
+    if (LW <= 64) {
+        if ((t & 63) < LW) shv[(t >> 6) * LW + (t & 63)] = v;
+        parts = 4;
+    } else {
+        shv[t] = v;
+        parts = 256 / LW;
+    }
+    __syncthreads();
+    V r;
+    bn_zero(r);
+    if (t < LW)
+        for (int k = 0; k < parts; ++k) r = r + shv[k * LW + t];
+    return r;
+}
+
+__device__ __forceinline__ void bn_share(int64_t nv, int nblk, int b, int64_t& lo, int64_t& hi) {
+    const int64_t per = (nv + nblk - 1) / nblk;
+    lo = per * b;
+    hi = lo + per < nv ? lo + per : nv;
+    if (lo > hi) lo = hi;
+}
+#endif
+
+}
diff --git a/molkgnn_amd/csrc/kgnn_capi.hip b/molkgnn_amd/csrc/kgnn_capi.hip
--- a/molkgnn_amd/csrc/kgnn_capi.hip
+++ b/molkgnn_amd/csrc/kgnn_capi.hip
@@ -5,6 +5,7 @@
 #include <mutex>
 
 #include "kgnn_launch.h"
+#include "kgnn_bn_reduce.h"
 #include "kgnn_split.h"
 
 using namespace mkgnn;
@@ -425,6 +426,23 @@
     g_grad_blocks_hint = gb;
     return 0;
 }
+
+struct BnSumsHint { BnSums bn; void* ws; size_t ws_bytes; };
+static thread_local BnSumsHint g_bn_sums_hint;
+static thread_local int g_bn_sums_taken = 0;
+static std::atomic<long long> g_bn_sums_launches;
+
+int mkgnn_backward_bn_sums(const float* x_raw, int64_t x_raw_stride, const float* save_mean, const float* save_invstd,
+                           const int64_t* n_valid_rows, void* workspace, size_t workspace_bytes) {
+    g_bn_sums_hint = BnSumsHint{};
+    if (!x_raw) return 0;
+    if (!save_mean || !save_invstd || !workspace) return api_fail("mkgnn_backward_bn_sums: null pointer");
+    g_bn_sums_hint.bn = BnSums{x_raw, x_raw_stride, save_mean, save_invstd, n_valid_rows, nullptr, nullptr};
+    g_bn_sums_hint.ws = workspace; g_bn_sums_hint.ws_bytes = workspace_bytes;
+    return 0;
+}
+int mkgnn_backward_bn_sums_taken(void) { return g_bn_sums_taken; }
+int64_t mkgnn_debug_bn_sums_launches(void) { return g_bn_sums_launches.load(); }
 
 int64_t mkgnn_debug_grad_blocks_launches(void) { return g_grad_blocks_launches.load(); }
 int mkgnn_debug_poison_backward(int32_t enable) { g_poison_bwd.store(enable ? 1 : 0); return 0; }
@@ -633,6 +651,9 @@
     const char* who = "mkgnn_kernelsetconv_backward";
     GradBlocks gb;
     const bool gb_hint = take_grad_blocks_hint(gb);
+    BnSumsHint bh = g_bn_sums_hint;
+    g_bn_sums_hint = BnSumsHint{};
+    g_bn_sums_taken = 0;
     const bool defer_bank = (variant & MKGNN_BACKWARD_DEFER_BANK) != 0;
     const bool through_nei = (variant & MKGNN_BACKWARD_THROUGH_NEIGHBOURS) != 0;
     const bool rows_split = (variant & MKGNN_BACKWARD_ROWS_SPLIT) != 0;
@@ -670,6 +691,14 @@
         int width = 0;
         for (int d = 1; d <= 4; ++d) width += (int)((gb.blk_len >> (8 * d)) & 0xFF);
         gb_gather = width == F;
+    }
+    bool bn_gather = bh.bn.x_raw && switches().bn_gather && variant != 1 && grad_x && n_edges > 0 && !gb_gather && rows_streamed && streamed &&
+                     F > 0 && bh.ws_bytes >= (size_t)2 * BN_MAIN_BLOCKS * F * sizeof(float) &&
+                     backward_gather_aligned_supported((const float*)((char*)workspace + w.contrib), (F + 3) / 4 * 4, scatter_rows, x, x_stride,
+                                                       n_atoms, F, grad_x, grad_x_stride);
+    if (bn_gather) {
+        bh.bn.part1 = (float*)bh.ws; bh.bn.part2 = bh.bn.part1 + (size_t)BN_MAIN_BLOCKS * F;
+        bn_gather = backward_gather_bn_sums_supported(bh.bn, F);
     }
     hipStream_t st = (hipStream_t)stream; char* ws = (char*)workspace;
     BwdArgs bank_a[4];
@@ -849,6 +878,10 @@
             e = launch_backward_gather_grad_blocks((const float*)(ws + w.contrib), (F + 3) / 4 * 4, scatter_rowptr, scatter_rows, x, x_stride,
                                                    inv_norm, n_atoms, F, grad_x, grad_x_stride, st, rows_split, gb);
             if (e == hipSuccess) g_grad_blocks_launches.fetch_add(1);
+        } else if (bn_gather) {
+            e = launch_backward_gather_bn_sums((const float*)(ws + w.contrib), (F + 3) / 4 * 4, scatter_rowptr, scatter_rows, x, x_stride,
+                                               inv_norm, n_atoms, F, st, rows_split, bh.bn);
+            if (e == hipSuccess) { g_bn_sums_launches.fetch_add(1); g_bn_sums_taken = 1; }
         } else
         e = launch_backward_gather((const float*)(ws + w.contrib), (F + 3) / 4 * 4, base, scatter_rowptr, scatter_rows, x,
                                    x_stride, inv_norm, n_atoms, F, grad_x, grad_x_stride, variant != 1, st, rows_split);
diff --git a/molkgnn_amd/csrc/kgnn_csr.hip b/molkgnn_amd/csrc/kgnn_csr.hip
--- a/molkgnn_amd/csrc/kgnn_csr.hip
+++ b/molkgnn_amd/csrc/kgnn_csr.hip
@@ -3,6 +3,7 @@
 #include <cstdlib>
 #include "kgnn_common.h"
 #include "kgnn_launch.h"
+#include "kgnn_bn_reduce.h"
 #include "kgnn_split.h"
 
 #include <atomic>
@@ -25,6 +26,7 @@
     int split_out;
     int x_split;
     const int8_t* present8;
+    BnSums bn;
 };
 
 template <int LPR>
@@ -47,10 +49,11 @@
     return v;
 }
 
-template <int LPR, bool GATHER, int BLK = 0, int CPL = 1, bool PM = false>
+template <int LPR, bool GATHER, int BLK = 0, int CPL = 1, bool PM = false, bool BNS = false>
 __global__ void __launch_bounds__(256) csr_rows_kernel(CsrArgs a) {
     static_assert(!(GATHER && BLK), "block rows: segment sums only");
     static_assert(!PM || GATHER, "present blocks: the gather only");
+    static_assert(!BNS || (GATHER && !PM && CPL == 1), "column sums: the plain one-chunk gather only");
     static_assert(CPL == 1 || CPL == 2, "one or two chunks per lane");
     constexpr int RPW = 64 / LPR, SEG = 4;
     static_assert(LPR >= SEG, "one index per lane of a row group");
@@ -65,21 +68,30 @@
         colc[q] = active[q] ? col[q] : 0;
     }
     const int n = (int)a.n;
-    const int wave0 = (int)((blockIdx.x * blockDim.x + threadIdx.x) >> 6);
-    const int nwaves = (int)((gridDim.x * blockDim.x) >> 6);
-    const int ngroups = (n + RPW - 1) / RPW;
+    int wave0 = (int)((blockIdx.x * blockDim.x + threadIdx.x) >> 6);
+    int nwaves = (int)((gridDim.x * blockDim.x) >> 6);
+    int ngroups = (n + RPW - 1) / RPW;
+    int row0 = 0, nend = n;
+    if constexpr (BNS) {
+        int64_t nv = n, lo, hi;
+        if (a.bn.nvalid) { const int64_t v = *a.bn.nvalid; nv = v < 1 ? 1 : (v < nv ? v : nv); }
+        bn_share(nv, (int)gridDim.x, (int)blockIdx.x, lo, hi);
+        row0 = (int)lo; nend = (int)hi;
+        wave0 = (int)(threadIdx.x >> 6); nwaves = (int)(blockDim.x >> 6);
+        ngroups = (nend - row0 + RPW - 1) / RPW;
+    }
     int last = a.rowptr[n] - 1;
     const int32_t* idxp = last >= 0 ? a.idx : a.rowptr;
     last = last >= 0 ? last : 0;
 
     auto segment = [&](int g, int& lo, int& hi, int& dg) -> int {
-        const int j = g * RPW + sub;
-        const int jc = (j < n && g < ngroups) ? j : n - 1;
+        const int j = row0 + g * RPW + sub;
+        const int jc = (j < nend && g < ngroups) ? j : nend - 1;
         lo = a.rowptr[(uint32_t)jc];
         hi = a.rowptr[(uint32_t)jc + 1];
         if constexpr (BLK == 2) dg = a.deg8[(uint32_t)jc];
         if constexpr (PM) dg = a.present8[(uint32_t)jc];
-        if (j >= n || g >= ngroups) hi = lo;
+        if (j >= nend || g >= ngroups) hi = lo;
         return jc;
     };
     auto block_of = [&](int d, int& b0, int& b1) {
@@ -195,6 +207,11 @@
     int mine_c = idx_issue(lo_c, hi_c, lo_c);
     int j_n = segment(g + nwaves, lo_n, hi_n, dg_n);
     int mine_n, lo_nn, hi_nn, dg_nn, j_nn;
+    f32x4 bn_s0 = {0.f, 0.f, 0.f, 0.f}, bn_s1 = {0.f, 0.f, 0.f, 0.f}, bn_mu = bn_s0, bn_is = bn_s0;
+    if constexpr (BNS) {
+#pragma unroll
+        for (int c = 0; c < 4; ++c) { bn_mu[c] = a.bn.save_mean[colc[0] + c]; bn_is[c] = a.bn.save_invstd[colc[0] + c]; }
+    }
     auto body = [&](auto kc) {
         constexpr int K = decltype(kc)::value;
         dg_nn = 0;
@@ -214,6 +231,8 @@
             for (int q = 0; q < CPL; ++q) xv[q] = *(const f32x4*)(xrow + (PM ? pm_c[q] : colc[q]));
             iv = a.inv[j_c];
         }
+        f32x4 xr = {0.f, 0.f, 0.f, 0.f};
+        if constexpr (BNS) xr = *(const f32x4*)(a.bn.x_raw + (uint64_t)(uint32_t)j_c * (uint64_t)a.bn.xrs + (uint32_t)colc[0]);
         mine_n = idx_issue(lo_n, hi_n, lo_n);
         j_nn = segment(g + 2 * nwaves, lo_nn, hi_nn, dg_nn);
         f32x4 acc[CPL];
@@ -233,7 +252,7 @@
         }
 #pragma unroll
         for (int q = 0; q < CPL; ++q) acc[q] = mask_cols(acc[q], active[q] ? col[q] : a.width, a.width);
-        const bool row_ok = g * RPW + sub < n;
+        const bool row_ok = row0 + g * RPW + sub < nend;
         if constexpr (GATHER) {
             const float xscale = a.x_split ? split_row_inv(iv) : iv;
             f32x4 xh[CPL];
@@ -255,6 +274,18 @@
                 f32x4 r;
 #pragma unroll
                 for (int c = 0; c < 4; ++c) r[c] = clamped ? acc[q][c] * iv : (acc[q][c] - dotp * xh[q][c]) * iv;
+                if constexpr (BNS) {
+#pragma unroll
+                    for (int c = 0; c < 4; ++c) asm("" : "+v"(r[c]));
+                    if (row_ok) {
+#pragma unroll
+                        for (int c = 0; c < 4; ++c) {
+                            bn_s0[c] += r[c];
+                            bn_s1[c] = fmaf(r[c], (xr[c] - bn_mu[c]) * bn_is[c], bn_s1[c]);
+                        }
+                    }
+                    continue;
+                }
                 if (row_ok && active[q] && (!PM || pm_keep[q])) *(f32x4*)(dst + col[q]) = r;
             }
         } else if constexpr (BLK == 2) {
@@ -308,6 +339,17 @@
         }
         lo_c = lo_n; hi_c = hi_n; j_c = j_n; dg_c = dg_n; mine_c = mine_n;
         lo_n = lo_nn; hi_n = hi_nn; j_n = j_nn; dg_n = dg_nn;
+    }
+    if constexpr (BNS) {
+        __shared__ f32x4 shv[256];
+        const f32x4 t0 = bn_reduce_rows(bn_s0, LPR, shv);
+        const f32x4 t1 = bn_reduce_rows(bn_s1, LPR, shv);
+        if ((int)threadIdx.x < LPR && active[0]) {
+            float* const p1 = a.bn.part1 + (int64_t)blockIdx.x * a.width;
+            float* const p2 = a.bn.part2 + (int64_t)blockIdx.x * a.width;
+#pragma unroll
+            for (int c = 0; c < 4; ++c) { p1[col[0] + c] = t0[c]; p2[col[0] + c] = t1[c]; }
+        }
     }
 }
 
@@ -506,12 +548,40 @@
     return launch_csr_rows<true, 0, true>(a, st);
 }
 
+bool backward_gather_bn_sums_supported(const BnSums& bn, int F) {
+    return bn.x_raw && F % 4 == 0 && F > 16 && F <= 32 && aligned_rows(bn.x_raw, bn.xrs, F) && bn.save_mean && bn.save_invstd &&
+           bn.part1 && bn.part2;
+}
+
+hipError_t launch_backward_gather_bn_sums(const float* contrib, int64_t cs, const int32_t* rowptr, const int32_t* rows, const float* x,
+                                          int64_t xs, const float* inv, int64_t n, int F, hipStream_t st, bool x_split, const BnSums& bn) {
+    CsrArgs a{};
+    a.src = contrib; a.ss = cs; a.rowptr = rowptr; a.idx = rows; a.n = n; a.width = F;
+    a.x = x; a.xs = xs; a.inv = inv; a.x_split = x_split ? 1 : 0;
+    a.fixed4 = switches().csr_fixed4;
+    a.bn = bn;
+    static_assert(BN_MAIN_BLOCKS >= 1, "the batch norm's grid");
+    csr_rows_kernel<8, true, 0, 1, false, true><<<BN_MAIN_BLOCKS, 256, 0, st>>>(a);
+    return hipGetLastError();
+}
+
 extern "C" int mkgnn_debug_backward_gather(const float* contrib, int64_t cs, const int32_t* rowptr, const int32_t* rows, const float* x,
                                            int64_t xs, const float* inv, int64_t n, int32_t F, float* gx, int64_t gxs, int32_t x_split,
                                            void* stream) {
     hipError_t e = hipSuccess;
     if (!try_backward_gather_aligned(contrib, cs, rowptr, rows, x, xs, inv, n, F, gx, gxs, (hipStream_t)stream, &e, x_split != 0)) return -1;
     return e == hipSuccess ? 0 : 1;
+}
+
+extern "C" int mkgnn_debug_backward_gather_bn_sums(const float* contrib, int64_t cs, const int32_t* rowptr, const int32_t* rows,
+                                                   const float* x, int64_t xs, const float* inv, int64_t n, int32_t F, int32_t x_split,
+                                                   const float* x_raw, int64_t x_raw_stride, const float* save_mean,
+                                                   const float* save_invstd, const int64_t* n_valid_rows, void* workspace,
+                                                   size_t workspace_bytes, void* stream) {
+    if (F < 1 || !workspace || workspace_bytes < (size_t)2 * BN_MAIN_BLOCKS * F * sizeof(float)) return -1;
+    BnSums bn{x_raw, x_raw_stride, save_mean, save_invstd, n_valid_rows, (float*)workspace, (float*)workspace + (size_t)BN_MAIN_BLOCKS * F};
+    if (!backward_gather_aligned_supported(contrib, cs, rows, x, xs, n, F, contrib, cs) || !backward_gather_bn_sums_supported(bn, F)) return -1;
+    return launch_backward_gather_bn_sums(contrib, cs, rowptr, rows, x, xs, inv, n, F, (hipStream_t)stream, x_split != 0, bn) == hipSuccess ? 0 : 1;
 }
 
 bool try_row_inv_norm_aligned(const float* x, int64_t xs, int64_t n, int width, float* inv, hipStream_t st, hipError_t* err) {
diff --git a/molkgnn_amd/csrc/kgnn_launch.h b/molkgnn_amd/csrc/kgnn_launch.h
--- a/molkgnn_amd/csrc/kgnn_launch.h
+++ b/molkgnn_amd/csrc/kgnn_launch.h
@@ -262,6 +262,10 @@
 hipError_t launch_backward_gather_grad_blocks(const float* contrib, int64_t cs, const int32_t* rowptr, const int32_t* rows,
                                               const float* x, int64_t xs, const float* inv, int64_t n, int F, float* gx, int64_t gxs,
                                               hipStream_t st, bool x_split, const GradBlocks& gb);
+struct BnSums;
+bool backward_gather_bn_sums_supported(const BnSums& bn, int F);
+hipError_t launch_backward_gather_bn_sums(const float* contrib, int64_t cs, const int32_t* rowptr, const int32_t* rows, const float* x,
+                                          int64_t xs, const float* inv, int64_t n, int F, hipStream_t st, bool x_split, const BnSums& bn);
 bool segment_sum_blocks_supported(const float* in, int64_t is, int64_t n, int width, const float* out, int64_t os);
 hipError_t launch_segment_sum_blocks(const float* in, int64_t is, const int32_t* rowptr, const int32_t* col, const int8_t* deg8,
                                      int64_t n, int width, const int32_t L[4], int mode, float* out, int64_t os,
diff --git a/molkgnn_amd/csrc/kgnn_switches.h b/molkgnn_amd/csrc/kgnn_switches.h
--- a/molkgnn_amd/csrc/kgnn_switches.h
+++ b/molkgnn_amd/csrc/kgnn_switches.h
@@ -32,6 +32,7 @@
     int tail_project_in_prepass;
     bool bn_one_launch;
     bool bn_merge;
+    bool bn_gather;
     char helper_priority;
     int fwd_pp;
     bool fwd_pp_env;
@@ -59,7 +60,7 @@
         s.bank_stream = not_0("MKGNN_BANK_STREAM"); s.fwd_stream = not_0("MKGNN_FWD_STREAM"); s.bf16_stream = not_0("MKGNN_BF16_STREAM");
         s.rows_split = not_0("MKGNN_ROWS_SPLIT"); s.grad_blocks = not_0("MKGNN_GRAD_BLOCKS"); s.tail_project_in_prepass = number("MKGNN_TAIL_PROJECT_IN_PREPASS", 2);
         if (const char* e = getenv("MKGNN_BN_ONE_LAUNCH")) s.bn_one_launch = e[0] == '1';
-        s.bn_merge = not_0("MKGNN_BN_MERGE");
+        s.bn_merge = not_0("MKGNN_BN_MERGE"); s.bn_gather = not_0("MKGNN_BN_GATHER");
         if (const char* e = getenv("MKGNN_HELPER_PRIORITY")) s.helper_priority = e[0];
         s.fwd_pp = number("MKGNN_FWD_PP", MKGNN_FWD_PP_DEFAULT); s.fwd_pp_env = number("MKGNN_FWD_PP", 0) != 0;
         s.fwd_split = number("MKGNN_FWD_SPLIT", MKGNN_FWD_SPLIT_DEFAULT); s.bwd_split = number("MKGNN_BWD_SPLIT", MKGNN_BWD_SPLIT_DEFAULT);
diff --git a/molkgnn_amd/functional.py b/molkgnn_amd/functional.py
--- a/molkgnn_amd/functional.py
+++ b/molkgnn_amd/functional.py
@@ -1,6 +1,7 @@
 from __future__ import annotations
 
 import threading
+import weakref
 from typing import List, Optional, Sequence, Tuple
 
 import os
@@ -146,6 +147,62 @@
     if getattr(x, "_backward_hooks", None) or x.retains_grad or torch.is_anomaly_enabled():
         return None
     return blocks
+
+
+_BN_GATHER_ATTR = "_mkgnn_bn_gather"
+BN_GATHER = os.environ.get("MKGNN_BN_GATHER", "0")[:1] == "1"
+
+
+class BnGatherTicket:
+    __slots__ = ("x_raw", "save_mean", "save_invstd", "n_valid", "partials", "out_ref", "__weakref__")
+
+    def __init__(self, x_raw, save_mean, save_invstd, n_valid=None):
+        self.x_raw, self.save_mean, self.save_invstd, self.n_valid = x_raw, save_mean, save_invstd, n_valid
+        self.partials = None
+        self.out_ref = None
+
+    def take_partials(self):
+        part, self.partials = self.partials, None
+        return part
+
+
+def bn_gather_width(C: int) -> bool:
+    return C % 4 == 0 and 16 < C <= 32
+
+
+def _gradient_watched(x: torch.Tensor) -> bool:
+    return bool(getattr(x, "_backward_hooks", None)) or x.retains_grad or torch.is_anomaly_enabled()
+
+
+def mark_bn_gather(out: torch.Tensor, ticket: BnGatherTicket, training: bool = True) -> torch.Tensor:
+    x_raw = ticket.x_raw
+    if not (BN_GATHER and training and out.requires_grad and not x_raw.requires_grad and out.dim() == 2 and x_raw.shape == out.shape
+            and bn_gather_width(out.shape[1]) and x_raw.stride(1) == 1 and x_raw.stride(0) % 4 == 0 and x_raw.data_ptr() % 16 == 0):
+        return out
+    ticket.out_ref = weakref.ref(out)
+    setattr(out, _BN_GATHER_ATTR, (out._version, ticket))
+    return out
+
+
+def bn_gather_of(x: torch.Tensor) -> Optional[BnGatherTicket]:
+    tag = getattr(x, _BN_GATHER_ATTR, None)
+    if tag is None or not BN_GATHER:
+        return None
+    version, ticket = tag
+    if version != x._version or ticket.out_ref is None or ticket.out_ref() is not x or _gradient_watched(x):
+        return None
+    return ticket
+
+
+def bn_gather_still_alone(ticket: BnGatherTicket) -> bool:
+    out = ticket.out_ref() if ticket.out_ref is not None else None
+    if torch.is_anomaly_enabled():
+        return False
+    return out is None or not (bool(getattr(out, "_backward_hooks", None)) or out.retains_grad)
+
+
+def debug_bn_sums_launches() -> int:
+    return int(_lib.load().mkgnn_debug_bn_sums_launches())
 
 
 def debug_grad_blocks_launches() -> int:
@@ -440,6 +497,8 @@
         need_grad = any(ctx.needs_input_grad) and getattr(_CALL, "grad_enabled", True)
         ctx.bwd_variant = int(bwd_variant)
         ctx.grad_blocks = grad_blocks_of(x, plan) if (need_grad and bwd_variant != BACKWARD_VARIANTS["generic"]) else None
+        ctx.bn_gather = bn_gather_of(x) if (need_grad and ctx.needs_input_grad[0]
+                                            and bwd_variant != BACKWARD_VARIANTS["generic"]) else None
         x, out_full, inv, saved_t, Ls, ws, x_split = _forward_impl(x, plan, is_last_layer, variant, out_pad, E, params, need_grad,
                                                                    inv, prepared)
         ctx.x_split = x_split
@@ -526,12 +585,22 @@
                                                                                  all(t is not q for q in gparams)]))
             hinted = ctx.grad_blocks is not None and gx is not None
             present = plan.present8 if hinted else None
+            ticket = ctx.bn_gather
+            summed = ticket is not None and gx is not None and not hinted and bn_gather_still_alone(ticket)
+            part = None
+            if summed:
+                part_bytes = int(lib.mkgnn_batchnorm_workspace_bytes(F))
+                part = torch.empty(part_bytes, dtype=torch.uint8, device=dev)
             if _USE_TORCH_OPS:
                 ps, bkl, counts, sv = _op_lists(plan, params, E, False, ctx.saved_t, dev)
             try:
                 if hinted:
                     _lib.check(lib.mkgnn_backward_grad_blocks(present.data_ptr(), _lib.Int32x4(*ctx.grad_blocks)),
                                "mkgnn_backward_grad_blocks")
+                if summed:
+                    _lib.check(lib.mkgnn_backward_bn_sums(ticket.x_raw.data_ptr(), _stride0(ticket.x_raw), ticket.save_mean.data_ptr(),
+                                                          ticket.save_invstd.data_ptr(), _lib.ptr(ticket.n_valid), part.data_ptr(),
+                                                          part_bytes), "mkgnn_backward_bn_sums")
                 if _USE_TORCH_OPS:
                     _lib.load_torch_ops().kernelsetconv_backward(x, inv, ps, bkl, counts, E, bool(ctx.is_last), g, sv, rowptr, rows, gx,
                                                                  list(alive), ws, bool(reuse), bwd_variant)
@@ -541,9 +610,13 @@
                         g.data_ptr(), _stride0(g), saved, rowptr.data_ptr(), rows.data_ptr(),
                         _lib.ptr(gx), F4, grads, ws.data_ptr(), ws_bytes, int(reuse), bwd_variant, _lib.stream_ptr(dev)),
                         "mkgnn_kernelsetconv_backward")
+                if summed and lib.mkgnn_backward_bn_sums_taken() == 1:
+                    ticket.partials = part
             finally:
                 if hinted:
                     lib.mkgnn_backward_grad_blocks(None, None)
+                if summed:
+                    lib.mkgnn_backward_bn_sums(None, 0, None, None, None, None, 0)
         del alive
         return (gx, None, None, None, None, None, None, None, None, None, *gparams)
 
diff --git a/molkgnn_amd/readout.py b/molkgnn_amd/readout.py
--- a/molkgnn_amd/readout.py
+++ b/molkgnn_amd/readout.py
@@ -253,7 +253,8 @@
 
 class _BatchNormFn(torch.autograd.Function):
     @staticmethod
-    def forward(ctx, x, weight, bias, bn: torch.nn.BatchNorm1d, use_batch_stats: bool, n_valid=None, companion=None, split_out=False):
+    def forward(ctx, x, weight, bias, bn: torch.nn.BatchNorm1d, use_batch_stats: bool, n_valid=None, companion=None, split_out=False,
+                ticket=None):
         lib = _lib.load()
         ctx.n_valid = n_valid
         x = _row_major(x if x.dtype == torch.float32 else x.float())
@@ -289,6 +290,10 @@
         ctx.use_batch_stats = use_batch_stats
         ctx.save_for_backward(x, weight, save_mean, save_invstd)
         ctx.wrote_split = bool(split_out and inv is not None)
+        ctx.ticket = None
+        if ticket is not None and ctx.wrote_split:
+            ticket.x_raw, ticket.save_mean, ticket.save_invstd, ticket.n_valid = x, save_mean, save_invstd, n_valid
+            ctx.ticket = ticket
         if inv is None:
             inv = torch.empty(0, dtype=torch.float32, device=dev)
         ctx.mark_non_differentiable(inv)
@@ -299,10 +304,18 @@
     def backward(ctx, grad_out, _g_inv=None):
         lib = _lib.load()
         if grad_out is None:
-            return None, None, None, None, None, None, None, None
+            return None, None, None, None, None, None, None, None, None
         x, weight, save_mean, save_invstd = ctx.saved_tensors
         n, C = x.shape
         dev = x.device
+        part = ctx.ticket.take_partials() if ctx.ticket is not None else None
+        if part is not None and not ctx.needs_input_grad[0]:
+            gw = torch.empty(C, dtype=torch.float32, device=dev) if (weight is not None and ctx.needs_input_grad[1]) else None
+            gb = torch.empty(C, dtype=torch.float32, device=dev) if ctx.needs_input_grad[2] else None
+            with torch.cuda.device(dev):
+                _lib.check(lib.mkgnn_batchnorm_backward_from_partials(C, _lib.ptr(gw), _lib.ptr(gb), part.data_ptr(), part.numel(),
+                                                                      _lib.stream_ptr(dev)), "mkgnn_batchnorm_backward_from_partials")
+            return None, gw, gb, None, None, None, None, None, None
         g = _row_major(grad_out if grad_out.dtype == torch.float32 else grad_out.float())
         gx = torch.empty((n, C), dtype=torch.float32, device=dev) if ctx.needs_input_grad[0] else None
         gw = torch.empty(C, dtype=torch.float32, device=dev) if (weight is not None and ctx.needs_input_grad[1]) else None
@@ -314,7 +327,7 @@
                 g.data_ptr(), _stride0(g), x.data_ptr(), _stride0(x), n, C, _lib.ptr(weight), save_mean.data_ptr(),
                 save_invstd.data_ptr(), int(ctx.use_batch_stats), _lib.ptr(gx), C, _lib.ptr(gw), _lib.ptr(gb),
                 _lib.ptr(ctx.n_valid), ws.data_ptr(), ws_bytes, _lib.stream_ptr(dev)), "mkgnn_batchnorm_backward")
-        return gx, gw, gb, None, None, None, None, None
+        return gx, gw, gb, None, None, None, None, None, None
 
 
 def _stats_supported(x: torch.Tensor, bn: torch.nn.BatchNorm1d) -> bool:
@@ -386,12 +399,18 @@
         return bn(x)
     if use_batch_stats and bn.training and x.shape[0] == 1:
         raise ValueError(f"Expected more than 1 value per channel when training, got input size {tuple(x.shape)}")
-    out, inv = _BatchNormFn.apply(x, bn.weight, bn.bias, bn, use_batch_stats, n_valid, companion, split_out)
+    from . import functional as _Fn
+    want_ticket = bool(split_out and _Fn.BN_GATHER and bn.training and use_batch_stats and torch.is_grad_enabled()
+                       and not x.requires_grad and _Fn.bn_gather_width(x.shape[1]))
+    ticket = _Fn.BnGatherTicket(None, None, None) if want_ticket else None
+    out, inv = _BatchNormFn.apply(x, bn.weight, bn.bias, bn, use_batch_stats, n_valid, companion, split_out, ticket)
     if inv.numel():
         from .functional import _INV_ATTR, mark_rows_split
         setattr(out, _INV_ATTR, (inv, out._version))
         if split_out:
             mark_rows_split(out)
+            if ticket is not None and ticket.x_raw is not None:
+                _Fn.mark_bn_gather(out, ticket, bn.training)
     return out
 
 
```
